# mahdi-slh/DeformContact

Hardware: AMD Instinct MI355X
Metric: M edges/sec fwd+bwd, everyday-deform batch=32 per GPU (encoder hot path) (higher is better)
Workload: dtype f32 (hops, storage, accumulate); wide dense blocks fp16x2-split operands (3 fp16 MFMA products, fp32 accumulate), narrow ones bf16x3-split (6 products); 1 GPU; everyday-deform synthetic, B=32 sample pairs per GPU: soft 32x(1024 v, 6132 e) + rigid 32x(762 v, 4560 e); TAGConv encoder 2 layers/branch, hidden 256, K=3 (configs[1]); edges_per_gpu_step=342144, global_batch=32, settle_steps=150, hipgraph=True, two_stream_branches=True, merged_branches=False, segmented_adjacency_build=True, parallelism=dp1

## Files before the change

deformcontact_amd/_lib.py:

```python
from __future__ import annotations

import ctypes
import os
from ctypes import POINTER, c_char_p, c_float, c_int, c_int32, c_int64, c_void_p

_HERE = os.path.dirname(os.path.abspath(__file__))
SO_PATH = os.path.join(_HERE, "libdeformcontact_hip.so")

_lib = None

_vp = c_void_p
_SIGNATURES = {
    "dc_version": (c_int, []),
    "dc_last_error": (c_char_p, []),
    "dc_stream_capture_id": (c_int64, [_vp]),
    "dc_csr_workspace_bytes": (c_int64, [c_int64, c_int64]),
    "dc_csr_build": (c_int, [_vp, c_int64, c_int64, c_int, c_int, _vp, _vp, _vp, _vp, _vp, _vp,
                             _vp, c_int64, _vp]),
    "dc_graph_workspace_bytes": (c_int64, [c_int64, c_int64]),
    "dc_graph_build": (c_int, [_vp, c_int64, c_int64, c_int, _vp, _vp, _vp, _vp, _vp, _vp, _vp, _vp,
                               _vp, _vp, c_int64, _vp]),
    "dc_graph_build_parts": (c_int, [POINTER(_vp), POINTER(c_int64), POINTER(c_int64), POINTER(c_int64), c_int,
                                     c_int64, c_int, _vp, _vp, _vp, _vp, _vp, _vp, _vp, _vp, _vp, _vp, c_int64,
                                     _vp]),
# ... 38 lines not shown
                                         _vp, _vp]),
    "dc_tag_grouped_bwd_dw_workspace_bytes": (c_int64, [POINTER(c_int64), c_int, c_int64, c_int64, c_int]),
    "dc_tag_grouped_bwd_dw_h2": (c_int, [_vp, c_int64, POINTER(_vp), POINTER(c_int64), c_int, c_int,
                                         POINTER(c_int64), POINTER(c_int64), c_int64, POINTER(_vp),
                                         POINTER(_vp), c_int, _vp, c_int64, c_int64, c_int64, _vp, _vp, _vp]),
    "dc_generic_dense_launches": (c_int64, [c_int]),
    "dc_kernel_trace": (None, [c_int]),
    "dc_kernel_trace_dump": (c_int64, [c_char_p, c_int64]),
    "dc_hash_i64": (c_int, [_vp, c_int64, _vp, _vp]),
    "dc_morton_codes": (c_int, [_vp, c_int64, c_int64, POINTER(c_float), POINTER(c_float), _vp, _vp]),
    "dc_morton_order_workspace_bytes": (c_int64, [c_int64]),
    "dc_morton_order": (c_int, [_vp, c_int64, c_int64, _vp, _vp, _vp, c_int64, _vp]),
    "dc_relabel_edges": (c_int, [_vp, c_int64, _vp, c_int64, _vp, _vp]),
    "dc_gather_rows": (c_int, [_vp, c_int64, _vp, _vp, c_int64, c_int64, c_int64, _vp]),
    "dc_invert_perm": (c_int, [_vp, _vp, _vp, c_int64, _vp]),
    "dc_neighbors_workspace_bytes": (c_int64, [c_int64, c_int64]),
    "dc_neighbors_fill": (c_int, [_vp, c_int64, c_int64, _vp, _vp, c_int64, c_int64, _vp, c_int, c_float, c_int, c_int,
                                  _vp, _vp, _vp, c_int64, _vp]),
    "dc_neighbors_compact_workspace_bytes": (c_int64, [c_int64]),
    "dc_neighbors_compact": (c_int, [_vp, c_int, _vp, c_int64, c_int, _vp, c_int64, _vp, c_int64, _vp]),
    "dc_spmm_f32": (c_int, [_vp, _vp, _vp, _vp, c_int64, _vp, c_int64, _vp, c_int64, c_int64,
                            c_int64, _vp]),
    "dc_spmm_bf16": (c_int, [_vp, _vp, _vp, _vp, c_int64, _vp, c_int64, _vp, c_int64, c_int64,
                             c_int64, c_int, _vp]),
    "dc_tag_linear_fwd_bf16": (c_int, [_vp, c_int64, _vp, _vp, c_int, _vp, c_int64, c_int, c_int64, c_int64,
                                       c_int64, _vp]),
    "dc_tag_mask_grad_bf16": (c_int, [_vp, c_int64, c_int, _vp, c_int64, c_int, _vp, c_int64, c_int64, c_int64, _vp]),
    "dc_tag_linear_bwd_dw_bf16_workspace_bytes": (c_int64, [c_int64, c_int64, c_int64, c_int]),
    "dc_tag_linear_bwd_dw_bf16": (c_int, [_vp, c_int64, _vp, c_int64, c_int, POINTER(_vp), _vp, c_int, _vp, c_int64,
                                          c_int64, c_int64, c_int64, _vp]),
    "dc_to_bf16": (c_int, [POINTER(_vp), c_int, c_int64, c_int64, c_int64, _vp, c_int64, _vp]),
    "dc_contact_loss_workspace_bytes": (c_int64, [c_int64]),
    "dc_contact_loss": (c_int, [_vp, _vp, _vp, _vp, _vp, c_int64, _vp, c_int64, c_int64, c_int64, _vp, _vp,
                                _vp, _vp, c_int64, _vp]),
    "dc_tag_linear_fwd": (c_int, [POINTER(_vp), POINTER(c_int64), POINTER(_vp), c_int, _vp, c_int,
                                  _vp, c_int64, c_int64, c_int64, c_int64, _vp]),
    "dc_tag_linear_bwd_dx": (c_int, [_vp, c_int64, _vp, c_int64, POINTER(_vp), c_int,
                                     POINTER(_vp), POINTER(c_int64), c_int64, c_int64, c_int64,
                                     _vp]),
    "dc_tag_linear_fwd_split": (c_int, [POINTER(_vp), POINTER(c_int64), POINTER(_vp), c_int, _vp,
                                        c_int, _vp, c_int64, c_int64, c_int64, c_int64, c_int, _vp]),
    "dc_tag_linear_bwd_dx_split_workspace_bytes": (c_int64, [c_int64, c_int64, c_int]),
    "dc_tag_linear_bwd_dx_split": (c_int, [_vp, c_int64, _vp, c_int64, POINTER(_vp), c_int,
                                           POINTER(_vp), POINTER(c_int64), _vp, c_int64, c_int64,
                                           c_int64, c_int64, c_int, _vp]),
    "dc_tag_linear_bwd_dw_workspace_bytes": (c_int64, [c_int64, c_int64, c_int64, c_int]),
    "dc_tag_linear_bwd_dw": (c_int, [_vp, c_int64, _vp, c_int64, POINTER(_vp), POINTER(c_int64),
                                     c_int, POINTER(_vp), c_int, c_int64, _vp, c_int, _vp, c_int64,
                                     c_int64, c_int64, c_int64, _vp]),
    "dc_tag_linear_bwd_dw_split": (c_int, [_vp, c_int64, _vp, c_int64, POINTER(_vp),
                                           POINTER(c_int64), c_int, POINTER(_vp), c_int, c_int64,
                                           _vp, c_int, _vp, c_int64, c_int64, c_int64, c_int64,
                                           c_int, _vp]),
    "dc_tag_linear_fwd_h2": (c_int, [POINTER(_vp), POINTER(c_int64), POINTER(_vp), c_int, _vp,
                                     c_int, _vp, c_int64, c_int64, c_int64, c_int64, _vp, _vp, _vp]),
    "dc_tag_linear_bwd_dx_h2": (c_int, [_vp, c_int64, _vp, c_int64, POINTER(_vp), c_int,
                                        POINTER(_vp), POINTER(c_int64), _vp, c_int64, c_int64,
                                        c_int64, c_int64, _vp, _vp, _vp]),
    "dc_tag_linear_bwd_dw_h2": (c_int, [_vp, c_int64, _vp, c_int64, POINTER(_vp),
                                        POINTER(c_int64), c_int, POINTER(_vp), c_int, c_int64,
                                        _vp, c_int, _vp, c_int64, c_int64, c_int64, c_int64,
                                        _vp, _vp, _vp]),
    "dc_tag_mask_grad": (c_int, [_vp, c_int64, _vp, c_int64, _vp, c_int64, c_int64, c_int64, _vp, _vp, _vp]),
    "dc_tag_transpose_weights": (c_int, [POINTER(_vp), c_int, c_int64, c_int64, _vp, _vp]),
    "dc_tag_linear_fwd_h2p_workspace_bytes": (c_int64, [c_int64, c_int64, c_int64]),
    "dc_tag_linear_fwd_h2p": (c_int, [_vp, c_int64, _vp, _vp, c_int, _vp, c_int64, c_int64, c_int64, c_int64,
                                      _vp, _vp, _vp, c_int64, _vp]),
    "dc_tag_linear_fwd_h2p_exp": (c_int, [_vp, c_int64, _vp, _vp, c_int64, c_int64, c_int64, c_int64, _vp, _vp, _vp,
                                          c_int64, _vp]),
    "dc_tag_weight_prep": (c_int, [POINTER(_vp), c_int, c_int64, c_int64, _vp, _vp, _vp, _vp, _vp]),
    "dc_tag_weight_prep_zero": (c_int, [POINTER(_vp), c_int, c_int64, c_int64, _vp, _vp, _vp, _vp, _vp, c_int64, _vp]),
    "dc_rowabsmax_f32": (c_int, [_vp, c_int64, c_int64, c_int64, _vp, _vp]),
    "dc_tag_weight_rowmax": (c_int, [POINTER(_vp), c_int, c_int64, c_int64, _vp, _vp]),
    "dc_spmm_f32_rowmax": (c_int, [_vp, _vp, _vp, _vp, c_int64, _vp, c_int64, _vp, c_int64, c_int64,
                                   c_int64, _vp, c_int, _vp]),
    "dc_tag_pack_input": (c_int, [_vp, c_int64, _vp, c_int64, c_int64, c_int64, c_int64, c_int64, _vp]),
    "dc_tag_pack_weights": (c_int, [POINTER(_vp), c_int, _vp, c_int64, c_int64, c_int64, _vp]),
    "dc_tag_linear_fwd_narrow_ok": (c_int, [c_int64, c_int, c_int64, c_int64]),
    "dc_tag_linear_fwd_narrow": (c_int, [_vp, c_int64, POINTER(_vp), c_int, c_int64, _vp, c_int, _vp, c_int64, c_int64,
                                         c_int64, c_int64, _vp]),
    "dc_attn_softmax_rows": (c_int, [_vp, c_int64, c_int64, c_int64, c_int64, _vp, _vp]),
    "dc_attn_exp_rows": (c_int, [_vp, c_int64, c_int64, c_int64, c_int64, _vp, _vp]),
    "dc_attn_ds_rows": (c_int, [_vp, _vp, c_int64, c_int64, c_int64, _vp, _vp, _vp]),
    "dc_adam_flat": (c_int, [_vp, _vp, _vp, _vp, c_int64, _vp, c_float, c_float, c_float, c_float,
                             c_int, _vp]),
    "dc_compose_perm": (c_int, [_vp, _vp, _vp, _vp, c_int64, _vp]),
    "dc_gat_edge_softmax_fwd": (c_int, [_vp, _vp, _vp, _vp, c_float, _vp, c_int64, _vp]),
    "dc_gat_edge_softmax_bwd": (c_int, [_vp, _vp, _vp, _vp, c_float, _vp, _vp, _vp, _vp, c_int64,
                                        _vp]),
    "dc_sddmm_f32": (c_int, [_vp, _vp, _vp, c_int64, _vp, c_int64, _vp, c_int64, c_int64, _vp]),
    "dc_segment_sum_f32": (c_int, [_vp, _vp, _vp, _vp, c_int64, _vp]),
    "dc_gather_f32": (c_int, [_vp, _vp, _vp, _vp, c_int64, _vp]),
    "dc_gat_alpha_heads_fwd": (c_int, [_vp, c_int64, _vp, _vp, _vp, _vp, c_int64, c_int64, c_int64, _vp]),
    "dc_gat_edge_softmax_heads_fwd": (c_int, [_vp, _vp, _vp, _vp, c_float, _vp, c_int64, c_int64, _vp]),
    "dc_spmm_f32_heads_bias_act": (c_int, [_vp, _vp, _vp, _vp, c_int64, _vp, c_int, c_int, _vp, c_int64, c_int64,
                                           c_int64, c_int64, _vp]),
    "dc_sddmm_f32_heads": (c_int, [_vp, _vp, _vp, c_int64, _vp, c_int64, _vp, c_int64, c_int64, c_int64, _vp]),
    "dc_gat_edge_softmax_heads_bwd": (c_int, [_vp, _vp, _vp, _vp, c_float, _vp, _vp, _vp, _vp, c_int64, c_int64,
                                              _vp]),
    "dc_segment_sum_f32_heads": (c_int, [_vp, _vp, _vp, _vp, c_int64, c_int64, _vp]),
    "dc_gather_f32_heads": (c_int, [_vp, _vp, _vp, _vp, c_int64, c_int64, _vp]),
    "dc_spread_heads_f32": (c_int, [_vp, c_int64, _vp, c_int64, c_int64, c_int64, c_int64, _vp]),
    "dc_gat_alpha_heads_bwd": (c_int, [_vp, c_int64, _vp, _vp, _vp, _vp, _vp, c_int64, c_int64, c_int64, c_int64, _vp,
                                       c_int64, _vp, _vp, c_int, _vp]),
    "dc_gat_edge_attr_fwd": (c_int, [_vp, _vp, _vp, c_int64, _vp, c_int, c_float, _vp, _vp, c_int64, c_int64, c_int64,
                                     c_int64, _vp]),
# ... 60 lines not shown
```

deformcontact_amd/csrc/dc_dense.h:

```cpp
#pragma once
#include "dc_common.h"

namespace dc {

constexpr int BK = 16;
constexpr int LDK = BK + 4;
constexpr int BN = 128;
constexpr int kMaxSeg = DC_MAX_SEG;

using f32x16 = __attribute__((ext_vector_type(16))) float;

struct Mat {
    const float *p;
    int64_t ld;
};

template <int MB>
struct Frag {
    float a[MB][4];
    float b[2][4];
};

template <int MB, bool A_KC, bool B_KC>
__device__ __forceinline__ void load_frag(Frag<MB> &f, const float *As, const float *Bs, int c,
// ... 38 lines not shown

template <int MB>
__device__ __forceinline__ void zero_acc(f32x16 (&acc)[MB][2]) {
#pragma unroll
    for (int mb = 0; mb < MB; ++mb)
#pragma unroll
        for (int i = 0; i < 16; ++i) acc[mb][0][i] = 0.f, acc[mb][1][i] = 0.f;
}

template <int MB> struct Tile {
    static constexpr int BM = 64 * MB;
    static constexpr int A_KC = BM * LDK, B_KC = BN * LDK, A_RC = BK * BM, B_RC = BK * BN;
};

template <int MB, typename F>
__device__ __forceinline__ void for_each_acc(const f32x16 (&acc)[MB][2], int wm, int wn, F &&f) {
    const int lane = threadIdx.x & 63, c = lane & 31, h = lane >> 5;
#pragma unroll
    for (int mb = 0; mb < MB; ++mb)
#pragma unroll
        for (int nb = 0; nb < 2; ++nb)
#pragma unroll
            for (int reg = 0; reg < 16; ++reg) {
                const int row = wm * 32 * MB + mb * 32 + (reg & 3) + 8 * (reg >> 2) + 4 * h;
                const int col = wn * 64 + nb * 32 + c;
                f(row, col, acc[mb][nb][reg]);
            }
}

struct H2Scales {
    const float *a_rowmax;
    const float *b_rowmax;
    int b_presplit;
};

__device__ __forceinline__ unsigned h2_exp(float m) {
    unsigned e = (__float_as_uint(m) >> 23) & 0xffu;
    e = e < 15u ? 15u : e;
    return e > 254u ? 254u : e;
}
__device__ __forceinline__ float h2_scale(float m) { return __uint_as_float((268u - h2_exp(m)) << 23); }
__device__ __forceinline__ float h2_unscale(float m) { return __uint_as_float((h2_exp(m) - 14u) << 23); }

__device__ __forceinline__ float h2_block_max(const float *v, int64_t beg, int64_t end, float *red) {
    float m = 0.f;
    for (int64_t i = beg + threadIdx.x; i < end; i += 256) m = fmaxf(m, v[i]);
#pragma unroll
    for (int o = 32; o >= 1; o >>= 1) m = fmaxf(m, __shfl_xor(m, o));
    if ((threadIdx.x & 63) == 0) red[threadIdx.x >> 6] = m;
    __syncthreads();
    m = fmaxf(fmaxf(red[0], red[1]), fmaxf(red[2], red[3]));
    __syncthreads();
    return m;
}

constexpr int kMaxGroups = DC_MAX_GROUPS;
constexpr int kGroupAlign = DC_GROUP_ALIGN;
struct FwdGroups {
    int n;
    int64_t row_beg[kMaxGroups];
    int64_t row_end[kMaxGroups];
    const float *w[kMaxGroups];
    const float *bias[kMaxGroups];
    const float *b_rowmax[kMaxGroups];
};
__device__ __forceinline__ int group_of_row(const int64_t (&row_beg)[kMaxGroups], int n, int64_t row) {
    int g = 0;
#pragma unroll
    for (int q = 1; q < kMaxGroups; ++q)
        if (q < n && row >= row_beg[q]) g = q;
    return g;
}

struct FwdParams {
    Mat x[kMaxSeg];
    Mat w[kMaxSeg];
    const float *bias;
    float *out;
    int64_t ldo, N, Fi, Fo;
    int nseg, relu;
    H2Scales h2;
    int ksplit;
    float *kpartial;
    const float *exp_lse;
    int64_t exp_ncols;
    FwdGroups grp;
    const float *x2, *x2_coef;
};

struct DxParams {
    Mat g, mask;
    int has_mask;
    Mat w[kMaxSeg];
    float *gx[kMaxSeg];
    int64_t ldgx[kMaxSeg];
    int64_t N, Fi, Fo;
    int nseg;
    H2Scales h2;
};

struct DwGroups {
    int n;
    int chunk_beg[kMaxGroups + 1];
    int64_t row_beg[kMaxGroups], row_end[kMaxGroups], chunk_rows[kMaxGroups];
};

struct DwParams {
    Mat g, mask;
    int has_mask;
    Mat x[kMaxSeg];
    float *partial;
    float *bias_partial;
    int64_t N, Fi, Fo, chunk_rows;
    int nseg, nchunks;
    H2Scales h2;
    DwGroups grp;
    const float *g2, *g2_coef;
};


struct DwBf16Params {
    const uint16_t *g, *x;
    int64_t ldg, ldx;
    float *partial;
    float *bias_partial;
    int64_t N, Fi, Fo, chunk_rows;
    int nseg, nchunks;
};
bool dw_bf16_launch(const DwBf16Params &p, hipStream_t hs);

bool fwd_fast_launch(const FwdParams &p, int mb, hipStream_t hs);
bool dx_fast_launch(const DxParams &p, int mb, hipStream_t hs);
bool dw_fast_launch(const DwParams &p, int mb, hipStream_t hs);
bool fwd_split_launch(const FwdParams &p, int mb, int products, hipStream_t hs);
bool dx_split_launch(DxParams p, float *wt, int mb, int products, hipStream_t hs);
bool dw_split_launch(const DwParams &p, int mb, int products, hipStream_t hs);
bool dw_h2w_launch(const DwParams &p, hipStream_t hs);
bool fwd_h2_launch(const FwdParams &p, int mb, hipStream_t hs);
bool fwd_h2w_launch(const FwdParams &p, hipStream_t hs);
bool fwd_h2d_launch(const FwdParams &p, hipStream_t hs);
void transpose_weights_launch(const float *const *ws, int nseg, int64_t Fo, int64_t Fi, float *wt,
                              hipStream_t hs);

}
```

deformcontact_amd/csrc/dc_dense.hip:

```cpp
#include <stdlib.h>

#include "dc_dense.h"

#include <atomic>
static std::atomic<long long> g_generic_dense_launches{0};

namespace dc {

template <bool VEC>
__device__ __forceinline__ float4 ld4(const float *row_ptr, int64_t k, int64_t kmax) {
    if (VEC) {
        const int64_t kc = (k + 4 <= kmax) ? k : 0;
        return *reinterpret_cast<const float4 *>(row_ptr + kc);
    } else {
        const int64_t last = kmax - 1;
        return make_float4(row_ptr[k + 0 <= last ? k + 0 : last], row_ptr[k + 1 <= last ? k + 1 : last],
                           row_ptr[k + 2 <= last ? k + 2 : last], row_ptr[k + 3 <= last ? k + 3 : last]);
    }
}

__device__ __forceinline__ float4 zero_invalid(float4 v, bool row_ok, int64_t k, int64_t kmax) {
    return make_float4((row_ok && k + 0 < kmax) ? v.x : 0.f, (row_ok && k + 1 < kmax) ? v.y : 0.f,
                       (row_ok && k + 2 < kmax) ? v.z : 0.f, (row_ok && k + 3 < kmax) ? v.w : 0.f);
}

__device__ __forceinline__ float4 relu_mask(float4 v, float4 m) {
    return make_float4(m.x > 0.f ? v.x : 0.f, m.y > 0.f ? v.y : 0.f, m.z > 0.f ? v.z : 0.f,
                       m.w > 0.f ? v.w : 0.f);
}

struct TileArgs {
    int64_t r0, rmax;
    int64_t c0, cmax;
};

template <int ROWS, bool VEC, bool MASK>
struct StageKC {
    float4 v[ROWS / 64];
    float4 m[MASK ? ROWS / 64 : 1];
    __device__ __forceinline__ void load(const Mat &mat, const Mat &mask, const TileArgs &t) {
        const int k4 = threadIdx.x & 3, r = threadIdx.x >> 2;
        const int64_t k = t.c0 + 4 * k4;
#pragma unroll
        for (int j = 0; j < ROWS / 64; ++j) {
            const int64_t row = t.r0 + r + 64 * j;
            const int64_t rc = row < t.rmax ? row : t.rmax - 1;
            v[j] = ld4<VEC>(mat.p + rc * mat.ld, k, t.cmax);
            if (MASK) m[j] = ld4<VEC>(mask.p + rc * mask.ld, k, t.cmax);
        }
    }
    __device__ __forceinline__ float4 value(int j, const TileArgs &t) const {
        const int k4 = threadIdx.x & 3, r = threadIdx.x >> 2;
        float4 x = zero_invalid(v[j], t.r0 + r + 64 * j < t.rmax, t.c0 + 4 * k4, t.cmax);
        if (MASK) x = relu_mask(x, m[j]);
        return x;
    }
    __device__ __forceinline__ void store(float *lds, const TileArgs &t) const {
        const int k4 = threadIdx.x & 3, r = threadIdx.x >> 2;
#pragma unroll
        for (int j = 0; j < ROWS / 64; ++j)
            *reinterpret_cast<float4 *>(lds + (r + 64 * j) * LDK + 4 * k4) = value(j, t);
    }
};

template <int COLS, bool VEC, bool MASK>
struct StageRC {
    static constexpr int PER = COLS / 4;
    static constexpr int KPER = 256 / PER;
    static constexpr int NLD = BK / KPER;
    float4 v[NLD];
    float4 m[MASK ? NLD : 1];
    __device__ __forceinline__ void load(const Mat &mat, const Mat &mask, const TileArgs &t) {
        const int c4 = threadIdx.x % PER, kr = threadIdx.x / PER;
        const int64_t col = t.c0 + 4 * c4;
#pragma unroll
        for (int j = 0; j < NLD; ++j) {
            const int64_t k = t.r0 + kr + KPER * j;
            const int64_t kc = k < t.rmax ? k : t.rmax - 1;
            v[j] = ld4<VEC>(mat.p + kc * mat.ld, col, t.cmax);
            if (MASK) m[j] = ld4<VEC>(mask.p + kc * mask.ld, col, t.cmax);
        }
    }
    __device__ __forceinline__ float4 value(int j, const TileArgs &t) const {
        const int c4 = threadIdx.x % PER, kr = threadIdx.x / PER;
        float4 x = zero_invalid(v[j], t.r0 + kr + KPER * j < t.rmax, t.c0 + 4 * c4, t.cmax);
        if (MASK) x = relu_mask(x, m[j]);
        return x;
    }
    __device__ __forceinline__ void store(float *lds, const TileArgs &t) const {
        const int c4 = threadIdx.x % PER, kr = threadIdx.x / PER;
#pragma unroll
        for (int j = 0; j < NLD; ++j)
            *reinterpret_cast<float4 *>(lds + (kr + KPER * j) * COLS + 4 * c4) = value(j, t);
    }
};

constexpr int kRing = 3;
static_assert(BK == 16, "the pipeline below is written for two 8-wide chunks per stage");

struct NoHook {
    template <typename S>
    __device__ __forceinline__ void operator()(const S &, const TileArgs &) const {}
};

template <int MB, bool A_KC, bool B_KC, int STAGE, int OFFB, typename SA, typename SB,
          typename TileFn, typename LdA, typename LdB, typename Hook = NoHook>
__device__ __forceinline__ void gemm_pipeline(float *lds, int nst, TileFn &&tile, LdA &&ldA,
                                              LdB &&ldB, f32x16 (&acc)[MB][2], int wm, int wn,
                                              Hook &&on_store_a = NoHook{}) {
    SA a0, a1;
    SB b0, b1;
    auto gload = [&](int st, SA &ra, SB &rb) {
        TileArgs ta, tb;
        tile(st, ta, tb);
        ldA(ra, ta);
        ldB(rb, tb);
    };
    auto lstore = [&](int st, const SA &ra, const SB &rb) {
        TileArgs ta, tb;
        tile(st, ta, tb);
        ra.store(lds + (st % kRing) * STAGE, ta);
        rb.store(lds + (st % kRing) * STAGE + OFFB, tb);
        on_store_a(ra, ta);
    };
    if (nst > 0) gload(0, a0, b0);
    if (nst > 1) gload(1, a1, b1);
    if (nst > 0) lstore(0, a0, b0);
    if (nst > 2) gload(2, a0, b0);
    if (nst > 1) lstore(1, a1, b1);
    if (nst > 3) gload(3, a1, b1);
    __syncthreads();
    Frag<MB> f0, f1;
    if (nst > 0) load_frag<MB, A_KC, B_KC>(f0, lds, lds + OFFB, 0, wm, wn);
// ... 76 lines not shown
    const int64_t col0 = (int64_t)(lb % ntn) * BN;
    const int wid = threadIdx.x >> 6, wm = wid >> 1, wn = wid & 1;

    f32x16 acc[MB][2];
    zero_acc<MB>(acc);

    const int nst = (int)((p.Fo + BK - 1) / BK);
    using SA = StageKC<BM, VEC, MASK>;
    using SB = StageRC<BN, VEC, false>;
    auto tile = [&](int st, TileArgs &ta, TileArgs &tb) {
        ta = TileArgs{row0, p.N, (int64_t)st * BK, p.Fo};
        tb = TileArgs{(int64_t)st * BK, p.Fo, col0, p.Fi};
    };
    auto ldA = [&](SA &ra, const TileArgs &t) { ra.load(p.g, p.mask, t); };
    auto ldB = [&](SB &rb, const TileArgs &t) { rb.load(p.w[s], p.w[s], t); };
    gemm_pipeline<MB, true, false, kStage, kOffB, SA, SB>(lds, nst, tile, ldA, ldB, acc, wm, wn);
    float *out = p.gx[s];
    const int64_t ldo = p.ldgx[s];
    for_each_acc<MB>(acc, wm, wn, [&](int r, int c, float v) {
        const int64_t row = row0 + r, col = col0 + c;
        if (row < p.N && col < p.Fi) out[row * ldo + col] = v;
    });
}


template <int MB, bool VEC, bool MASK>
__global__ void __launch_bounds__(256)
k_tag_linear_bwd_dw(DwParams p) {
    using T = Tile<MB>;
    constexpr int BM = T::BM, kStage = T::A_RC + T::B_RC, kOffB = T::A_RC;
    __shared__ __attribute__((aligned(16))) float lds[kRing * kStage];
    const unsigned ntm = (unsigned)((p.Fo + BM - 1) / BM), ntn = (unsigned)((p.Fi + BN - 1) / BN);
    const unsigned tiles = ntm * ntn, per_chunk = tiles * p.nseg;
    const unsigned lb = blockIdx.x;
    const unsigned chunk = lb / per_chunk, rem = lb % per_chunk;
    const int s = (int)(rem / tiles);
    const int64_t o0 = (int64_t)((rem % tiles) / ntn) * BM, f0 = (int64_t)((rem % tiles) % ntn) * BN;
    const int64_t n_beg = (int64_t)chunk * p.chunk_rows;
    const int64_t n_end = (n_beg + p.chunk_rows < p.N) ? n_beg + p.chunk_rows : p.N;
    const int wid = threadIdx.x >> 6, wm = wid >> 1, wn = wid & 1;
    const bool do_bias = p.bias_partial && s == 0 && f0 == 0;

    f32x16 acc[MB][2];
    zero_acc<MB>(acc);
    float4 bsum4 = make_float4(0.f, 0.f, 0.f, 0.f);

    const int nst = (int)((n_end - n_beg + BK - 1) / BK);
    using SA = StageRC<BM, VEC, MASK>;
    using SB = StageRC<BN, VEC, false>;
    auto tile = [&](int st, TileArgs &ta, TileArgs &tb) {
        ta = TileArgs{n_beg + (int64_t)st * BK, n_end, o0, p.Fo};
        tb = TileArgs{n_beg + (int64_t)st * BK, n_end, f0, p.Fi};
    };
    auto ldA = [&](SA &ra, const TileArgs &t) { ra.load(p.g, p.mask, t); };
    auto ldB = [&](SB &rb, const TileArgs &t) { rb.load(p.x[s], p.x[s], t); };
    auto bias_hook = [&](const SA &ra, const TileArgs &t) {
        if (do_bias) {
#pragma unroll
            for (int j = 0; j < SA::NLD; ++j) {
                const float4 x = ra.value(j, t);
                bsum4.x += x.x, bsum4.y += x.y, bsum4.z += x.z, bsum4.w += x.w;
            }
        }
    };
    gemm_pipeline<MB, false, false, kStage, kOffB, SA, SB>(lds, nst, tile, ldA, ldB, acc, wm, wn,
                                                          bias_hook);
    float *out = p.partial + ((int64_t)chunk * p.nseg + s) * p.Fo * p.Fi;
    for_each_acc<MB>(acc, wm, wn, [&](int r, int c, float v) {
        const int64_t o = o0 + r, f = f0 + c;
        if (o < p.Fo && f < p.Fi) out[o * p.Fi + f] = v;
    });
    if (do_bias) {
        __syncthreads();
        float4 *red = reinterpret_cast<float4 *>(lds);
        red[threadIdx.x] = bsum4;
        __syncthreads();
        if (threadIdx.x < SA::PER) {
            float4 t = make_float4(0.f, 0.f, 0.f, 0.f);
            for (int g = 0; g < 256 / SA::PER; ++g) {
                const float4 v = red[g * SA::PER + threadIdx.x];
                t.x += v.x, t.y += v.y, t.z += v.z, t.w += v.w;
            }
            float *bp = p.bias_partial + (int64_t)chunk * p.Fo;
            const int64_t o = o0 + 4 * threadIdx.x;
            if (o + 0 < p.Fo) bp[o + 0] = t.x;
            if (o + 1 < p.Fo) bp[o + 1] = t.y;
            if (o + 2 < p.Fo) bp[o + 2] = t.z;
            if (o + 3 < p.Fo) bp[o + 3] = t.w;
        }
    }
}

struct ReduceParams {
    const float *partial, *bias_partial;
    float *gw[2 * kMaxSeg];
    float *gbias;
    int64_t Fi, Fo, cols;
    int nseg, nchunks, ngw, bps, accumulate;
};

constexpr int kReduceOutputs = 64;
__device__ __forceinline__ void dw_reduce_body(const ReduceParams &p) {
    __shared__ float red[4][kReduceOutputs];
    const int64_t per_out = p.Fo * p.cols, total = per_out * p.ngw;
    const int64_t seg_elems = p.Fo * p.Fi, slab = seg_elems * p.nseg;
    const int el = threadIdx.x & 63, q = threadIdx.x >> 6;
    const int64_t i = (int64_t)blockIdx.x * kReduceOutputs + el;
// ... 93 lines not shown
static inline int env_int(const char *name, int dflt) {
    const char *v = getenv(name);
    return v ? atoi(v) : dflt;
}

static inline int pick_mb(int64_t rows, int64_t col_tiles) {
    return (((rows + 127) / 128) * col_tiles >= 512) ? 2 : 1;
}

static inline int split_mb(int64_t rows, int64_t col_tiles) {
    const int64_t nb2 = ((rows + 127) / 128) * col_tiles, nb1 = ((rows + 63) / 64) * col_tiles;
    const double t2 = (double)((nb2 + 255) / 256);
    const double t1 = (double)((nb1 + 255) / 256) * 0.5 * 1.12;
    return t1 < t2 ? 1 : 2;
}

static inline int dw_mb(int64_t Fo) {
    return Fo >= 128 ? 2 : 1;
}

static void dw_plan(int64_t N, int64_t Fi, int64_t Fo, int nseg, int64_t *chunk_rows,
                    int *nchunks) {
    const int64_t BM = 64 * dw_mb(Fo);
    const int64_t tiles = ((Fo + BM - 1) / BM) * ((Fi + BN - 1) / BN) * nseg;
    constexpr int target = 512, maxchunks = 128;
    int64_t want = target / (tiles > 0 ? tiles : 1);
    if (want < 1) want = 1;
    if (want > maxchunks) want = maxchunks;
    if (want == 1 && N >= 8192) {
        const int64_t t2 = ((Fo + 127) / 128) * ((Fi + 255) / 256) * nseg;
        double best = 0.0;
        for (int64_t c = 1; c <= 8 && N / c >= 2048; ++c) {
            const int64_t w = (t2 * c + 255) / 256;
            const double eff = (double)(t2 * c) / (double)(w * 256);
            if (eff > best + 0.02) best = eff, want = c;
        }
    }
    int64_t rows = (N + want - 1) / want;
    if (rows < 256) rows = 256;
    rows = (rows + 2 * BK - 1) / (2 * BK) * (2 * BK);
    *chunk_rows = rows;
    *nchunks = (int)((N + rows - 1) / rows);
    if (*nchunks < 1) *nchunks = 1;
}

}

using namespace dc;

static int fwd_impl(const float *const *xs, const int64_t *ldxs, const float *const *ws, int nseg,
                    const float *bias, int relu, float *out, int64_t ldo, int64_t N, int64_t Fi,
                    int64_t Fo, dc_stream_t stream, int products, H2Scales h2 = H2Scales{},
                    float *ksplit_ws = nullptr, int64_t ksplit_ws_bytes = 0, const float *exp_lse = nullptr,
                    int64_t exp_ncols = 0) {
    DC_REQUIRE(nseg >= 1 && nseg <= kMaxSeg, "dc_tag_linear_fwd: nseg must be 1..%d", kMaxSeg);
    DC_REQUIRE(N >= 0 && Fi >= 1 && Fo >= 1, "dc_tag_linear_fwd: bad sizes");
    if (N == 0) return DC_OK;
    DC_REQUIRE(xs && ldxs && ws && out && ldo >= Fo, "dc_tag_linear_fwd: null pointer / ldo < Fo");
    FwdParams p{};
    bool vec = (Fi % 4 == 0);
    for (int s = 0; s < nseg; ++s) {
        DC_REQUIRE(xs[s] && ws[s] && ldxs[s] >= Fi, "dc_tag_linear_fwd: bad segment %d", s);
        p.x[s] = make_mat(xs[s], ldxs[s], &vec);
        p.w[s] = make_mat(ws[s], Fi, &vec);
    }
    p.bias = bias, p.out = out, p.ldo = ldo, p.N = N, p.Fi = Fi, p.Fo = Fo;
    p.nseg = nseg, p.relu = relu;
    p.h2 = h2;
    p.exp_lse = exp_lse, p.exp_ncols = exp_ncols;
    DC_REQUIRE(!exp_lse || h2.b_presplit, "dc_tag_linear_fwd: the exp epilogue exists on the pre-split h2 kernels only");
    const int64_t ntn = (Fo + BN - 1) / BN;
    const int mb = pick_mb(N, ntn);
    const int64_t grid = ((N + 64 * mb - 1) / (64 * mb)) * ntn;
    DC_REQUIRE(grid < (int64_t)INT32_MAX, "dc_tag_linear_fwd: grid too large");
    const dim3 gd((unsigned)grid), bd(256);
    hipStream_t hs = (hipStream_t)stream;
    if (products == 2 && vec) {
        int smb = split_mb(N, ntn);
        const int64_t nst = Fi / BK;
        if (ksplit_ws && !bias && !relu && ldo == Fo && nseg == 1) {
            smb = 2;
            int64_t tiles = ((N + 127) / 128) * ntn;
            if (tiles < 128) smb = 1, tiles = ((N + 63) / 64) * ntn;
            int64_t ks = tiles < 256 ? (512 + tiles - 1) / tiles : 1;
            if (ks > nst / 8) ks = nst / 8;
            if (ks > 32) ks = 32;
            while (ks > 1 && ks * N * Fo * (int64_t)sizeof(float) > ksplit_ws_bytes) --ks;
            if (ks > 1) p.ksplit = (int)ks, p.kpartial = ksplit_ws;
        }
        if (fwd_h2_launch(p, smb, hs)) {
            if (p.ksplit > 1) {
                ReduceParams r{};
                r.partial = p.kpartial, r.gw[0] = out, r.Fi = Fo, r.Fo = N, r.cols = Fo;
                r.nseg = 1, r.nchunks = p.ksplit, r.ngw = 1, r.bps = 1, r.accumulate = 0;
                const int64_t total = N * Fo;
                launch_reduce(r, total, hs);
            }
            return check_launch("dc_tag_linear_fwd_h2");
        }
        p.ksplit = 0, p.kpartial = nullptr;
    }
    DC_REQUIRE(!h2.b_presplit, "dc_tag_linear_fwd_h2p: shape not eligible for the pre-split kernel");
    if (products && vec && fwd_split_launch(p, split_mb(N, ntn), products, hs))
        return check_launch("dc_tag_linear_fwd_split");
    DC_REQUIRE(products != 2, "dc_tag_linear_fwd_h2: needs Fi %% 16 == 0, 16-byte aligned operands, "
                              "equal leading dimensions (Fi=%lld)", (long long)Fi);
    if (vec && fwd_fast_launch(p, mb, hs)) return check_launch("dc_tag_linear_fwd");
    static const int trace = env_int("DC_DENSE_TRACE", 0);
    ++g_generic_dense_launches;
    if (trace)
        fprintf(stderr, "[dc] generic fwd dense kernel: N=%lld Fi=%lld Fo=%lld nseg=%d vec=%d ldx=%lld ldo=%lld products=%d\n",
                (long long)N, (long long)Fi, (long long)Fo, nseg, (int)vec, (long long)ldxs[0], (long long)ldo, products);
    if (mb == 2 && vec)
        DC_LAUNCH((k_tag_linear_fwd<2, true>), gd, bd, 0, hs, p);
    else if (mb == 2)
        DC_LAUNCH((k_tag_linear_fwd<2, false>), gd, bd, 0, hs, p);
    else if (vec)
        DC_LAUNCH((k_tag_linear_fwd<1, true>), gd, bd, 0, hs, p);
    else
        DC_LAUNCH((k_tag_linear_fwd<1, false>), gd, bd, 0, hs, p);
    return check_launch("dc_tag_linear_fwd");
}

static int dx_impl(const float *g, int64_t ldg, const float *out_for_mask, int64_t ldo,
                   const float *const *ws, int nseg, float *const *gxs, const int64_t *ldgxs,
                   int64_t N, int64_t Fi, int64_t Fo, dc_stream_t stream, float *split_ws,
                   int products, H2Scales h2 = H2Scales{}) {
    DC_REQUIRE(nseg >= 1 && nseg <= kMaxSeg, "dc_tag_linear_bwd_dx: nseg must be 1..%d", kMaxSeg);
    DC_REQUIRE(N >= 0 && Fi >= 1 && Fo >= 1, "dc_tag_linear_bwd_dx: bad sizes");
    if (N == 0) return DC_OK;
    DC_REQUIRE(g && ws && gxs && ldgxs && ldg >= Fo, "dc_tag_linear_bwd_dx: null pointer / ldg < Fo");
    DC_REQUIRE(!out_for_mask || ldo >= Fo, "dc_tag_linear_bwd_dx: ldo < Fo");
    DxParams p{};
    bool vec = (Fi % 4 == 0) && (Fo % 4 == 0);
    p.g = make_mat(g, ldg, &vec);
    p.has_mask = out_for_mask != nullptr;
    if (out_for_mask) p.mask = make_mat(out_for_mask, ldo, &vec);
    for (int s = 0; s < nseg; ++s) {
        DC_REQUIRE(ws[s] && gxs[s] && ldgxs[s] >= Fi, "dc_tag_linear_bwd_dx: bad segment %d", s);
        p.w[s] = make_mat(ws[s], Fi, &vec);
        p.gx[s] = gxs[s];
        p.ldgx[s] = ldgxs[s];
    }
// ... 47 lines not shown
extern "C" int dc_tag_linear_bwd_dx(const float *g, int64_t ldg, const float *out_for_mask,
                                    int64_t ldo, const float *const *ws, int nseg,
                                    float *const *gxs, const int64_t *ldgxs, int64_t N, int64_t Fi,
                                    int64_t Fo, dc_stream_t stream) {
    return dx_impl(g, ldg, out_for_mask, ldo, ws, nseg, gxs, ldgxs, N, Fi, Fo, stream, nullptr, 0);
}

extern "C" int dc_tag_linear_bwd_dw(const float *g, int64_t ldg, const float *out_for_mask,
                                    int64_t ldo, const float *const *xs, const int64_t *ldxs,
                                    int nseg, float *const *gws, int ngw, int64_t gw_cols,
                                    float *gbias, int accumulate, void *partials,
                                    int64_t partials_bytes, int64_t N, int64_t Fi, int64_t Fo,
                                    dc_stream_t stream);
extern "C" int dc_tag_linear_bwd_dw_split(const float *g, int64_t ldg, const float *out_for_mask,
                                          int64_t ldo, const float *const *xs, const int64_t *ldxs,
                                          int nseg, float *const *gws, int ngw, int64_t gw_cols,
                                          float *gbias, int accumulate, void *partials,
                                          int64_t partials_bytes, int64_t N, int64_t Fi, int64_t Fo,
                                          int products, dc_stream_t stream);

extern "C" int64_t dc_tag_linear_bwd_dx_split_workspace_bytes(int64_t Fi, int64_t Fo, int nseg) {
    if (Fi < 1 || Fo < 1 || nseg < 1 || nseg > kMaxSeg) return DC_EINVAL;
    return (int64_t)sizeof(float) * nseg * Fi * Fo + 16;
}

extern "C" int dc_tag_linear_bwd_dx_split(const float *g, int64_t ldg, const float *out_for_mask,
                                          int64_t ldo, const float *const *ws, int nseg,
                                          float *const *gxs, const int64_t *ldgxs, void *workspace,
                                          int64_t workspace_bytes, int64_t N, int64_t Fi,
                                          int64_t Fo, int products, dc_stream_t stream) {
    DC_REQUIRE(products == 6 || products == 3 || products == 1,
               "dc_tag_linear_bwd_dx_split: products must be 6, 3 or 1");
    DC_REQUIRE(workspace && ((uintptr_t)workspace & 15) == 0 &&
                   workspace_bytes >= dc_tag_linear_bwd_dx_split_workspace_bytes(Fi, Fo, nseg),
               "dc_tag_linear_bwd_dx_split: workspace missing, misaligned or too small");
    return dx_impl(g, ldg, out_for_mask, ldo, ws, nseg, gxs, ldgxs, N, Fi, Fo, stream,
                   (float *)workspace, products);
}

extern "C" int64_t dc_tag_linear_bwd_dw_workspace_bytes(int64_t N, int64_t Fi, int64_t Fo,
                                                        int nseg) {
    if (N < 0 || Fi < 1 || Fo < 1 || nseg < 1 || nseg > kMaxSeg) return DC_EINVAL;
    int64_t rows;
    int nchunks;
    dw_plan(N, Fi, Fo, nseg, &rows, &nchunks);
    return (int64_t)sizeof(float) * (nchunks + 1) * (nseg * Fo * Fi + Fo) + 16;
}

static int dw_impl(const float *g, int64_t ldg, const float *out_for_mask, int64_t ldo,
                   const float *const *xs, const int64_t *ldxs, int nseg, float *const *gws, int ngw,
                   int64_t gw_cols, float *gbias, int accumulate, void *partials,
                   int64_t partials_bytes, int64_t N, int64_t Fi, int64_t Fo, dc_stream_t stream,
                   int products, H2Scales h2 = H2Scales{}, const float *g2 = nullptr,
                   const float *g2_coef = nullptr) {
    DC_REQUIRE(nseg >= 1 && nseg <= kMaxSeg, "dc_tag_linear_bwd_dw: nseg must be 1..%d", kMaxSeg);
    DC_REQUIRE(N >= 0 && Fi >= 1 && Fo >= 1, "dc_tag_linear_bwd_dw: bad sizes");
    DC_REQUIRE(g && xs && ldxs && gws && partials && ldg >= Fo,
               "dc_tag_linear_bwd_dw: null pointer / ldg < Fo");
    DC_REQUIRE(!out_for_mask || ldo >= Fo, "dc_tag_linear_bwd_dw: ldo < Fo");
    DC_REQUIRE(partials_bytes >= dc_tag_linear_bwd_dw_workspace_bytes(N, Fi, Fo, nseg),
               "dc_tag_linear_bwd_dw: workspace too small");
    DC_REQUIRE(((uintptr_t)partials & 15) == 0, "dc_tag_linear_bwd_dw: workspace not 16-byte aligned");
    DwParams p{};
    bool vec = (Fi % 4 == 0) && (Fo % 4 == 0);
    p.g = make_mat(g, ldg, &vec);
    p.has_mask = out_for_mask != nullptr;
    if (out_for_mask) p.mask = make_mat(out_for_mask, ldo, &vec);
    ReduceParams r{};
    for (int s = 0; s < nseg; ++s) {
        DC_REQUIRE(xs[s] && ldxs[s] >= Fi, "dc_tag_linear_bwd_dw: bad segment %d", s);
        p.x[s] = make_mat(xs[s], ldxs[s], &vec);
    }
    DC_REQUIRE(ngw >= nseg && ngw <= 2 * kMaxSeg && ngw % nseg == 0 && gw_cols >= 1 &&
                   (ngw / nseg) * gw_cols <= Fi,
               "dc_tag_linear_bwd_dw: %d output blocks of %lld columns do not tile %d segments of %lld",
               ngw, (long long)gw_cols, nseg, (long long)Fi);
    for (int j = 0; j < ngw; ++j) {
        DC_REQUIRE(gws[j], "dc_tag_linear_bwd_dw: null output block %d", j);
        r.gw[j] = gws[j];
    }
    dw_plan(N, Fi, Fo, nseg, &p.chunk_rows, &p.nchunks);
    p.N = N, p.Fi = Fi, p.Fo = Fo, p.nseg = nseg;
    p.h2 = h2;
    p.partial = (float *)partials;
    const int64_t tail = vec ? N % BK : 0;
    const bool ragged = tail != 0 && N > tail;
    const int nslots = p.nchunks + (ragged ? 1 : 0);
    p.bias_partial = gbias ? p.partial + (int64_t)nslots * nseg * Fo * Fi : nullptr;
    const int mb = dw_mb(Fo);
    const int64_t tiles = ((Fo + 64 * mb - 1) / (64 * mb)) * ((Fi + BN - 1) / BN);
    const int64_t grid = tiles * nseg * p.nchunks;
    if (!p.has_mask) p.mask = p.g;
    const dim3 gd((unsigned)grid), bd(256);
    hipStream_t hs = (hipStream_t)stream;
    if (g2) {
        DC_REQUIRE(g2_coef && products == 2 && vec && !ragged && (((uintptr_t)g2) & 15) == 0,
                   "dc_tag_linear_bwd_dw_h2_corr: needs the coefficient vector, aligned operands and N %% 16 == 0");
        p.g2 = g2, p.g2_coef = g2_coef;
        DC_REQUIRE(dw_h2w_launch(p, hs), "dc_tag_linear_bwd_dw_h2_corr: shape not eligible for the 128 x 256 tile kernel "
                   "(needs Fo %% 128 == 0, Fi == 256, N %% 32 == 0; N=%lld Fi=%lld Fo=%lld)", (long long)N,
                   (long long)Fi, (long long)Fo);
        r.partial = p.partial, r.bias_partial = p.bias_partial, r.gbias = gbias;
        r.Fi = Fi, r.Fo = Fo, r.nseg = nseg, r.nchunks = nslots;
        r.cols = gw_cols, r.ngw = ngw, r.bps = ngw / nseg, r.accumulate = accumulate;
        const int64_t total_c = (int64_t)ngw * Fo * gw_cols + (gbias ? Fo : 0);
        launch_reduce(r, total_c, hs);
        return check_launch("dc_tag_linear_bwd_dw_h2_corr");
    }
    if (ragged) {
        DwParams t = p;
        const int64_t n0 = N - tail;
        t.g.p += n0 * t.g.ld;
        t.mask.p += n0 * t.mask.ld;
        for (int s = 0; s < nseg; ++s) t.x[s].p += n0 * t.x[s].ld;
        t.N = tail, t.chunk_rows = BK, t.nchunks = 1;
        t.partial = p.partial + (int64_t)p.nchunks * nseg * Fo * Fi;
        t.bias_partial = p.bias_partial ? p.bias_partial + (int64_t)p.nchunks * Fo : nullptr;
        t.h2 = H2Scales{};
        const dim3 gt((unsigned)(tiles * nseg));
        if (mb == 2) {
            if (p.has_mask) DC_LAUNCH((k_tag_linear_bwd_dw<2, true, true>), gt, bd, 0, hs, t);
            else DC_LAUNCH((k_tag_linear_bwd_dw<2, true, false>), gt, bd, 0, hs, t);
        } else {
            if (p.has_mask) DC_LAUNCH((k_tag_linear_bwd_dw<1, true, true>), gt, bd, 0, hs, t);
            else DC_LAUNCH((k_tag_linear_bwd_dw<1, true, false>), gt, bd, 0, hs, t);
        }
        p.N = n0;
    }
    bool fast_done = products && vec && dw_split_launch(p, mb, products, hs);
    DC_REQUIRE(fast_done || products != 2, "dc_tag_linear_bwd_dw_h2: needs N %% 16 == 0, Fi %% 4 == 0, "
               "Fo %% 4 == 0 and 16-byte aligned operands (N=%lld)", (long long)N);
    fast_done = fast_done || (vec && dw_fast_launch(p, mb, hs));
#define DC_DW(MB_, V_, M_) DC_LAUNCH((k_tag_linear_bwd_dw<MB_, V_, M_>), gd, bd, 0, hs, p)
    if (!fast_done) ++g_generic_dense_launches;
    if (fast_done) {
    } else
    if (mb == 2) {
        if (vec && p.has_mask) DC_DW(2, true, true);
        else if (vec) DC_DW(2, true, false);
        else if (p.has_mask) DC_DW(2, false, true);
        else DC_DW(2, false, false);
    } else {
        if (vec && p.has_mask) DC_DW(1, true, true);
        else if (vec) DC_DW(1, true, false);
        else if (p.has_mask) DC_DW(1, false, true);
        else DC_DW(1, false, false);
    }
#undef DC_DW
    r.partial = p.partial, r.bias_partial = p.bias_partial, r.gbias = gbias;
    r.Fi = Fi, r.Fo = Fo, r.nseg = nseg, r.nchunks = nslots;
    r.cols = gw_cols, r.ngw = ngw, r.bps = ngw / nseg, r.accumulate = accumulate;
    const int64_t total = (int64_t)ngw * Fo * gw_cols + (gbias ? Fo : 0);
    launch_reduce(r, total, (hipStream_t)stream);
    return check_launch("dc_tag_linear_bwd_dw");
}

extern "C" int dc_tag_linear_bwd_dw(const float *g, int64_t ldg, const float *out_for_mask,
                                    int64_t ldo, const float *const *xs, const int64_t *ldxs,
                                    int nseg, float *const *gws, int ngw, int64_t gw_cols,
                                    float *gbias, int accumulate, void *partials,
                                    int64_t partials_bytes, int64_t N, int64_t Fi, int64_t Fo,
                                    dc_stream_t stream) {
    return dw_impl(g, ldg, out_for_mask, ldo, xs, ldxs, nseg, gws, ngw, gw_cols, gbias, accumulate,
                   partials, partials_bytes, N, Fi, Fo, stream, 0);
}

extern "C" int dc_tag_linear_bwd_dw_split(const float *g, int64_t ldg, const float *out_for_mask,
                                          int64_t ldo, const float *const *xs, const int64_t *ldxs,
                                          int nseg, float *const *gws, int ngw, int64_t gw_cols,
                                          float *gbias, int accumulate, void *partials,
                                          int64_t partials_bytes, int64_t N, int64_t Fi, int64_t Fo,
                                          int products, dc_stream_t stream) {
    DC_REQUIRE(products == 6 || products == 3 || products == 1,
               "dc_tag_linear_bwd_dw_split: products must be 6, 3 or 1");
    return dw_impl(g, ldg, out_for_mask, ldo, xs, ldxs, nseg, gws, ngw, gw_cols, gbias, accumulate,
                   partials, partials_bytes, N, Fi, Fo, stream, products);
}


extern "C" int dc_tag_linear_fwd_h2(const float *const *xs, const int64_t *ldxs,
                                    const float *const *ws, int nseg, const float *bias, int relu,
                                    float *out, int64_t ldo, int64_t N, int64_t Fi, int64_t Fo,
                                    const float *x_rowmax, const float *w_rowmax,
                                    dc_stream_t stream) {
    DC_REQUIRE(x_rowmax && w_rowmax, "dc_tag_linear_fwd_h2: x_rowmax / w_rowmax missing");
    H2Scales h{};
    h.a_rowmax = x_rowmax, h.b_rowmax = w_rowmax;
    return fwd_impl(xs, ldxs, ws, nseg, bias, relu, out, ldo, N, Fi, Fo, stream, 2, h);
}

extern "C" int64_t dc_tag_linear_fwd_h2p_workspace_bytes(int64_t N, int64_t K, int64_t Fo) {
    if (N < 0 || K < 1 || Fo < 1) return DC_EINVAL;
    const int64_t tiles = ((N + 63) / 64) * ((Fo + BN - 1) / BN);
    if (tiles >= 256 || K / BK < 16) return 0;
    return 32 * N * Fo * (int64_t)sizeof(float);
}

extern "C" int dc_tag_linear_fwd_h2p(const float *x, int64_t ldx, const void *w_image,
                                     const float *bias, int relu, float *out, int64_t ldo, int64_t N,
                                     int64_t K, int64_t Fo, const float *x_rowmax,
                                     const float *w_rowmax, void *workspace,
                                     int64_t workspace_bytes, dc_stream_t stream) {
    DC_REQUIRE(x && w_image && x_rowmax && w_rowmax, "dc_tag_linear_fwd_h2p: null pointer");
    DC_REQUIRE(K >= 16 && K % 16 == 0 && ldx >= K && ldx % 4 == 0 && (((uintptr_t)x) & 15) == 0 &&
                   (((uintptr_t)w_image) & 15) == 0,
               "dc_tag_linear_fwd_h2p: K %% 16 == 0 and 16-byte aligned operands required (K=%lld)",
               (long long)K);
    H2Scales h{};
    h.a_rowmax = x_rowmax, h.b_rowmax = w_rowmax, h.b_presplit = 1;
    const float *xs[1] = {x};
    const float *ws[1] = {(const float *)w_image};
    const int64_t ld[1] = {ldx};
    DC_REQUIRE(!workspace || (((uintptr_t)workspace) & 15) == 0, "dc_tag_linear_fwd_h2p: workspace misaligned");
    return fwd_impl(xs, ld, ws, 1, bias, relu, out, ldo, N, K, Fo, stream, 2, h, (float *)workspace,
                    workspace ? workspace_bytes : 0);
}

extern "C" int dc_tag_linear_fwd_h2p_corr(const float *x, int64_t ldx, const float *x2, const float *x2_coef,
                                          const void *w_image, float *out, int64_t ldo, int64_t N, int64_t K,
                                          int64_t Fo, const float *x_rowmax, const float *w_rowmax,
                                          dc_stream_t stream) {
    DC_REQUIRE(N >= 0 && K >= 32 && K % 32 == 0 && Fo >= 1, "dc_tag_linear_fwd_h2p_corr: K must be a multiple of 32");
    if (N == 0) return DC_OK;
    DC_REQUIRE(x && x2 && x2_coef && w_image && out && x_rowmax && w_rowmax && ldx >= K && ldo >= Fo &&
                   (((uintptr_t)x2) & 15) == 0, "dc_tag_linear_fwd_h2p_corr: null / short / misaligned operand");
    FwdParams p{};
    bool vec = true;
    p.x[0] = make_mat(x, ldx, &vec);
    p.w[0] = make_mat((const float *)w_image, K, &vec);
    p.out = out, p.ldo = ldo, p.N = N, p.Fi = K, p.Fo = Fo, p.nseg = 1;
    p.h2.a_rowmax = x_rowmax, p.h2.b_rowmax = w_rowmax, p.h2.b_presplit = 1;
    p.x2 = x2, p.x2_coef = x2_coef;
    DC_REQUIRE(vec && fwd_h2w_launch(p, (hipStream_t)stream),
               "dc_tag_linear_fwd_h2p_corr: shape not eligible for the 128 x 256 tile kernel (N=%lld K=%lld Fo=%lld: "
               "needs 16-byte aligned rows)", (long long)N, (long long)K, (long long)Fo);
    return check_launch("dc_tag_linear_fwd_h2p_corr");
}

extern "C" int dc_tag_linear_fwd_h2p_exp(const float *x, int64_t ldx, const void *w_image, float *out,
                                         int64_t ldo, int64_t N, int64_t K, int64_t Fo, const float *x_rowmax,
                                         const float *w_rowmax, const float *row_lse, int64_t ncols_valid,
                                         dc_stream_t stream) {
    DC_REQUIRE(x && w_image && x_rowmax && w_rowmax && row_lse, "dc_tag_linear_fwd_h2p_exp: null pointer");
    DC_REQUIRE(K >= 16 && K % 16 == 0 && ldx >= K && ldx % 4 == 0 && (((uintptr_t)x) & 15) == 0 &&
                   (((uintptr_t)w_image) & 15) == 0 && ncols_valid >= 0 && ncols_valid <= Fo,
               "dc_tag_linear_fwd_h2p_exp: K %% 16 == 0, 16-byte aligned operands, 0 <= ncols_valid <= Fo required");
    H2Scales h{};
    h.a_rowmax = x_rowmax, h.b_rowmax = w_rowmax, h.b_presplit = 1;
    const float *xs[1] = {x};
    const float *ws[1] = {(const float *)w_image};
    const int64_t ld[1] = {ldx};
    return fwd_impl(xs, ld, ws, 1, nullptr, 0, out, ldo, N, K, Fo, stream, 2, h, nullptr, 0, row_lse, ncols_valid);
}

extern "C" int dc_tag_linear_bwd_dx_h2(const float *g, int64_t ldg, const float *out_for_mask,
                                       int64_t ldo, const float *const *ws, int nseg,
                                       float *const *gxs, const int64_t *ldgxs, void *workspace,
                                       int64_t workspace_bytes, int64_t N, int64_t Fi, int64_t Fo,
                                       const float *g_rowmax, const float *w_rowmax,
                                       dc_stream_t stream) {
    DC_REQUIRE(w_rowmax && g_rowmax, "dc_tag_linear_bwd_dx_h2: g_rowmax / w_rowmax missing");
    DC_REQUIRE(workspace && ((uintptr_t)workspace & 15) == 0 &&
                   workspace_bytes >= dc_tag_linear_bwd_dx_split_workspace_bytes(Fi, Fo, nseg),
               "dc_tag_linear_bwd_dx_h2: workspace missing, misaligned or too small");
    H2Scales h{};
    h.a_rowmax = g_rowmax, h.b_rowmax = w_rowmax;
    return dx_impl(g, ldg, out_for_mask, ldo, ws, nseg, gxs, ldgxs, N, Fi, Fo, stream,
                   (float *)workspace, 2, h);
// ... 23 lines not shown
    H2Scales h2{};
    h2.a_rowmax = g_rowmax, h2.b_rowmax = x_rowmax;
    return dw_impl(g, ldg, nullptr, 0, xs, ldxs, nseg, gws, ngw, gw_cols, nullptr, accumulate, partials,
                   partials_bytes, N, Fi, Fo, stream, 2, h2, g2, g2_coef);
}

namespace dc {
__global__ void __launch_bounds__(256)
k_rowabsmax(const float *__restrict__ x, int64_t ld, int64_t N, int F, float *__restrict__ rowmax,
            bool vec4) {
    const int64_t row = (int64_t)blockIdx.x * 4 + (threadIdx.x >> 6);
    if (row >= N) return;
    const int lane = threadIdx.x & 63;
    const float *xr = x + row * ld;
    float m = 0.f;
    if (vec4) {
        for (int c = lane * 4; c < F; c += 256) {
            const float4 v = *reinterpret_cast<const float4 *>(xr + c);
            m = fmaxf(m, fmaxf(fmaxf(fabsf(v.x), fabsf(v.y)), fmaxf(fabsf(v.z), fabsf(v.w))));
        }
    } else {
        for (int c = lane; c < F; c += 64) m = fmaxf(m, fabsf(xr[c]));
    }
#pragma unroll
    for (int o = 32; o >= 1; o >>= 1) m = fmaxf(m, __shfl_xor(m, o));
    if (lane == 0) rowmax[row] = m;
}

struct WRowmaxParams {
    const float *w[kMaxSeg];
    int nseg;
    int64_t Fo, Fi;
    float *out;
};
__global__ void __launch_bounds__(256) k_w_rowmax(WRowmaxParams p) {
    const int64_t o = (int64_t)blockIdx.x * 4 + (threadIdx.x >> 6);
    if (o >= p.Fo) return;
    const int lane = threadIdx.x & 63;
    float m = 0.f;
    for (int s = 0; s < p.nseg; ++s) {
        const float *wr = p.w[s] + o * p.Fi;
        for (int64_t c = lane; c < p.Fi; c += 64) m = fmaxf(m, fabsf(wr[c]));
    }
#pragma unroll
    for (int q = 32; q >= 1; q >>= 1) m = fmaxf(m, __shfl_xor(m, q));
    if (lane == 0) p.out[o] = m;
}
}

namespace dc {
__global__ void __launch_bounds__(256)
k_mask_grad(const float *__restrict__ g, int64_t ldg, const float *__restrict__ mask, int64_t ldm,
            float *__restrict__ gm, int64_t ldgm, int64_t N, int F, float *__restrict__ rowmax_a,
            float *__restrict__ rowmax_b, bool vec4) {
    const int64_t row = (int64_t)blockIdx.x * 4 + (threadIdx.x >> 6);
    if (row >= N) return;
    const int lane = threadIdx.x & 63;
    const float *gr = g + row * ldg, *mr = mask ? mask + row * ldm : nullptr;
    float *o = gm + row * ldgm;
    float m = 0.f;
    if (vec4) {
        for (int c = lane * 4; c < F; c += 256) {
            float4 v = *reinterpret_cast<const float4 *>(gr + c);
            if (mr) {
                const float4 k = *reinterpret_cast<const float4 *>(mr + c);
                v = make_float4(k.x > 0.f ? v.x : 0.f, k.y > 0.f ? v.y : 0.f, k.z > 0.f ? v.z : 0.f,
                                k.w > 0.f ? v.w : 0.f);
            }
            *reinterpret_cast<float4 *>(o + c) = v;
            m = fmaxf(m, fmaxf(fmaxf(fabsf(v.x), fabsf(v.y)), fmaxf(fabsf(v.z), fabsf(v.w))));
        }
    } else {
        for (int c = lane; c < F; c += 64) {
            float v = gr[c];
            if (mr && !(mr[c] > 0.f)) v = 0.f;
            o[c] = v;
            m = fmaxf(m, fabsf(v));
        }
    }
#pragma unroll
    for (int q = 32; q >= 1; q >>= 1) m = fmaxf(m, __shfl_xor(m, q));
    if (lane == 0) {
        rowmax_a[row] = m;
        if (rowmax_b) rowmax_b[row] = m;
    }
}
}

extern "C" int dc_tag_mask_grad(const float *g, int64_t ldg, const float *out_for_mask, int64_t ldo,
                                float *gm, int64_t ldgm, int64_t N, int64_t F, float *rowmax_a,
                                float *rowmax_b, dc_stream_t stream) {
    DC_REQUIRE(N >= 0 && F >= 1 && F < (1 << 24) && ldg >= F && ldgm >= F && (!out_for_mask || ldo >= F),
               "dc_tag_mask_grad: bad sizes");
    if (N == 0) return DC_OK;
    DC_REQUIRE(g && gm && rowmax_a, "dc_tag_mask_grad: null pointer");
    const bool vec4 = (F % 4 == 0) && (ldg % 4 == 0) && (ldgm % 4 == 0) && (((uintptr_t)g) & 15) == 0 &&
                      (((uintptr_t)gm) & 15) == 0 &&
                      (!out_for_mask || ((ldo % 4 == 0) && (((uintptr_t)out_for_mask) & 15) == 0));
    DC_LAUNCH(k_mask_grad, dim3((unsigned)((N + 3) / 4)), dim3(256), 0, (hipStream_t)stream, g,
                       ldg, out_for_mask, ldo, gm, ldgm, N, (int)F, rowmax_a, rowmax_b, vec4);
    return check_launch("dc_tag_mask_grad");
}

namespace dc {
struct WPrepParams {
    const float *w[kMaxSeg];
    int nseg;
    int64_t Fo, Fi;
    float *w_rowmax, *wt_rowmax;
    _Float16 *wimg, *wtimg;
    float *zero;
    int64_t zero_n;
    int tall;
};
__device__ __forceinline__ void wprep_put(_Float16 *img_row, int64_t k, float v, float scale) {
    const float x = v * scale;
    const _Float16 h = (_Float16)x;
    _Float16 *rec = img_row + (k >> 4) * 32 + (k & 15);
    rec[0] = h;
    rec[16] = (_Float16)(x - (float)h);
}
__device__ __forceinline__ void weight_prep_body(const WPrepParams &p) {
    const int lane = threadIdx.x & 63;
    for (int64_t i = (int64_t)blockIdx.x * blockDim.x + threadIdx.x; i < p.zero_n; i += (int64_t)gridDim.x * blockDim.x)
        p.zero[i] = 0.f;
    if (p.tall)
        for (int64_t i = (int64_t)blockIdx.x * blockDim.x + threadIdx.x; i < p.Fi; i += (int64_t)gridDim.x * blockDim.x)
            p.wt_rowmax[i] = 0.f;
    const int64_t rb = (p.Fo + 3) / 4;
    float m = 0.f;
    const bool small = p.Fi <= 256 && p.Fo <= 256;
    if ((int64_t)blockIdx.x < rb) {
        const int64_t o = (int64_t)blockIdx.x * 4 + (threadIdx.x >> 6);
        if (o >= p.Fo) return;
        float v[kMaxSeg][4];
        if (small) {
#pragma unroll
            for (int s = 0; s < kMaxSeg; ++s)
#pragma unroll
                for (int j = 0; j < 4; ++j) {
                    const int64_t c = lane + 64 * j;
                    v[s][j] = (s < p.nseg && c < p.Fi) ? p.w[s][o * p.Fi + c] : 0.f;
                    m = fmaxf(m, fabsf(v[s][j]));
                }
        } else {
            for (int s = 0; s < p.nseg; ++s) {
                const float *wr = p.w[s] + o * p.Fi;
                for (int64_t c = lane; c < p.Fi; c += 64) m = fmaxf(m, fabsf(wr[c]));
            }
        }
#pragma unroll
        for (int q = 32; q >= 1; q >>= 1) m = fmaxf(m, __shfl_xor(m, q));
        if (lane == 0) p.w_rowmax[o] = m;
        if (p.wimg) {
// ... 472 lines not shown
```

deformcontact_amd/csrc/dc_dense_fast.hip:

```cpp
#include "dc_dense.h"

namespace dc {

template <int ROWS, bool KC, bool MASK>
struct FastOp {
    static constexpr int NV = ROWS / 64;
    static constexpr int PER = ROWS / 4;
    static constexpr int KPER = 256 / PER;
    const float *p[NV];
    const float *pm[MASK ? NV : 1];
    float4 v[NV];
    float4 m[MASK ? NV : 1];
    int off[NV];
    int64_t step;

    __device__ __forceinline__ void init_kc(const float *base, const float *mbase, int64_t ld,
                                            int64_t row0, int64_t nrows, int64_t k0) {
        const int k4 = threadIdx.x & 3, r = threadIdx.x >> 2;
#pragma unroll
        for (int j = 0; j < NV; ++j) {
            int64_t row = row0 + r + 64 * j;
            row = row < nrows ? row : nrows - 1;
            p[j] = base + row * ld + k0 + 4 * k4;
            if (MASK) pm[j] = mbase + row * ld + k0 + 4 * k4;
// ... 204 lines not shown
        __syncthreads();
        float4 *red = reinterpret_cast<float4 *>(lds);
        red[threadIdx.x] = bsum4;
        __syncthreads();
        if (threadIdx.x < OA::PER) {
            float4 t = make_float4(0.f, 0.f, 0.f, 0.f);
            for (int g = 0; g < 256 / OA::PER; ++g) {
                const float4 v = red[g * OA::PER + threadIdx.x];
                t.x += v.x, t.y += v.y, t.z += v.z, t.w += v.w;
            }
            float *bp = p.bias_partial + (int64_t)chunk * p.Fo;
            const int64_t o = o0 + 4 * threadIdx.x;
            if (o + 4 <= p.Fo) {
                bp[o + 0] = t.x, bp[o + 1] = t.y, bp[o + 2] = t.z, bp[o + 3] = t.w;
            }
        }
    }
}

static inline bool al16(const void *q) { return ((uintptr_t)q & 15) == 0; }

bool fwd_fast_launch(const FwdParams &p, int mb, hipStream_t hs) {
    if (p.Fi % BK != 0 || p.Fi < BK) return false;
    for (int s = 0; s < p.nseg; ++s)
        if (!al16(p.x[s].p) || !al16(p.w[s].p) || p.x[s].ld % 4 != 0 || p.x[s].ld != p.x[0].ld)
            return false;
    const int64_t grid = ((p.N + 64 * mb - 1) / (64 * mb)) * ((p.Fo + BN - 1) / BN);
    const dim3 gd((unsigned)grid), bd(256);
    if (mb == 2)
        DC_LAUNCH((k_fwd_fast<2>), gd, bd, 0, hs, p);
    else
        DC_LAUNCH((k_fwd_fast<1>), gd, bd, 0, hs, p);
    return true;
}

bool dx_fast_launch(const DxParams &p, int mb, hipStream_t hs) {
    if (p.Fo % BK != 0 || p.Fi % 4 != 0 || p.Fi < 4 || !al16(p.g.p) || p.g.ld % 4 != 0) return false;
    if (p.has_mask && (!al16(p.mask.p) || p.mask.ld != p.g.ld)) return false;
    for (int s = 0; s < p.nseg; ++s)
        if (!al16(p.w[s].p)) return false;
    const int64_t grid = ((p.N + 64 * mb - 1) / (64 * mb)) * ((p.Fi + BN - 1) / BN) * p.nseg;
    const dim3 gd((unsigned)grid), bd(256);
#define DC_L(MB_, M_) DC_LAUNCH((k_dx_fast<MB_, M_>), gd, bd, 0, hs, p)
    if (mb == 2) { if (p.has_mask) DC_L(2, true); else DC_L(2, false); }
    else { if (p.has_mask) DC_L(1, true); else DC_L(1, false); }
#undef DC_L
    return true;
}

bool dw_fast_launch(const DwParams &p, int mb, hipStream_t hs) {
    if (p.N % BK != 0 || p.chunk_rows % BK != 0 || p.Fi % 4 != 0 || p.Fo % 4 != 0 || p.Fi < 4 ||
        p.Fo < 4 || !al16(p.g.p) || p.g.ld % 4 != 0)
        return false;
    if (p.has_mask && (!al16(p.mask.p) || p.mask.ld != p.g.ld)) return false;
    for (int s = 0; s < p.nseg; ++s)
        if (!al16(p.x[s].p) || p.x[s].ld % 4 != 0) return false;
    const int64_t tiles = ((p.Fo + 64 * mb - 1) / (64 * mb)) * ((p.Fi + BN - 1) / BN);
    const dim3 gd((unsigned)(tiles * p.nseg * p.nchunks)), bd(256);
#define DC_L(MB_, M_) DC_LAUNCH((k_dw_fast<MB_, M_>), gd, bd, 0, hs, p)
    if (mb == 2) { if (p.has_mask) DC_L(2, true); else DC_L(2, false); }
    else { if (p.has_mask) DC_L(1, true); else DC_L(1, false); }
#undef DC_L
    return true;
}

}
```

deformcontact_amd/csrc/dc_dense_h2.hip:

```cpp
#include "dc_dense.h"

namespace dc {

using h2_f16x4 = __attribute__((ext_vector_type(4))) _Float16;
using h2_f16x8 = __attribute__((ext_vector_type(8))) _Float16;

constexpr int kH2Plane = 32;
constexpr int kH2Row = 2 * kH2Plane + 16;

__device__ __forceinline__ void h2_split_store(char *dst, float4 x, float s) {
    x = make_float4(x.x * s, x.y * s, x.z * s, x.w * s);
    h2_f16x4 h, l;
    const float v[4] = {x.x, x.y, x.z, x.w};
#pragma unroll
    for (int i = 0; i < 4; ++i) {
        const _Float16 a = (_Float16)v[i];
        h[i] = a;
        l[i] = (_Float16)(v[i] - (float)a);
    }
    *reinterpret_cast<h2_f16x4 *>(dst) = h;
    *reinterpret_cast<h2_f16x4 *>(dst + kH2Plane) = l;
}

template <int MB, bool BDMA>
// ... 133 lines not shown
            frags(cur);
            if (BDMA) dma_b(nxt);
            store(nxt);
            load();
            mma();
            if (BDMA) __builtin_amdgcn_s_waitcnt(0xF70 | 0);
            __syncthreads();
        }
        for (; it < nst; ++it) {
            const int cur = it & 1, nxt = cur ^ 1;
            frags(cur);
            if (it + 1 < nst) {
                if (BDMA) dma_b(nxt);
                store(nxt);
            }
            mma();
            if (BDMA) __builtin_amdgcn_s_waitcnt(0xF70 | 0);
            __syncthreads();
        }
    }

    float bcol[2], icol[2];
#pragma unroll
    for (int nb = 0; nb < 2; ++nb) {
        const int64_t col = col0 + wn * 64 + nb * 32 + (threadIdx.x & 31);
        bcol[nb] = (p.bias && col < p.Fo) ? p.bias[col] : 0.f;
        icol[nb] = h2_unscale(p.h2.b_rowmax[col < p.Fo ? col : p.Fo - 1]);
    }
    const bool relu = p.relu != 0;
    if (ks > 1) {
        float *part = p.kpartial + (int64_t)kz * p.N * p.Fo;
        for_each_acc<MB>(acc, wm, wn, [&](int rr, int c, float v) {
            const int64_t row = row0 + rr, col = col0 + c;
            if (row < p.N && col < p.Fo) part[row * p.Fo + col] = (v * s_inv[rr]) * icol[(c >> 5) & 1];
        });
        return;
    }
    for_each_acc<MB>(acc, wm, wn, [&](int rr, int c, float v) {
        const int64_t row = row0 + rr, col = col0 + c;
        if (row < p.N && col < p.Fo) {
            v = (v * s_inv[rr]) * icol[(c >> 5) & 1];
            v += bcol[(c >> 5) & 1];
            if (relu) v = fmaxf(v, 0.f);
            if (p.exp_lse) v = col < p.exp_ncols ? expf(v - p.exp_lse[row]) : 0.f;
            p.out[row * p.ldo + col] = v;
        }
    });
}



static inline bool h2_al16(const void *q) { return ((uintptr_t)q & 15) == 0; }

bool fwd_h2_launch(const FwdParams &p, int mb, hipStream_t hs) {
    if (!p.h2.a_rowmax || !p.h2.b_rowmax || p.nseg != 1) return false;
    if (fwd_h2w_launch(p, hs)) return true;
    if (p.Fi % BK != 0 || p.Fi < BK) return false;
    if (p.x[0].ld * 128 >= ((int64_t)1 << 30) || p.Fi * 128 >= ((int64_t)1 << 30)) return false;
    for (int s = 0; s < p.nseg; ++s)
        if (!h2_al16(p.x[s].p) || !h2_al16(p.w[s].p) || p.x[s].ld % 4 != 0 || p.x[s].ld != p.x[0].ld)
            return false;
    const int64_t grid = ((p.N + 64 * mb - 1) / (64 * mb)) * ((p.Fo + BN - 1) / BN) *
                         (p.ksplit > 1 ? p.ksplit : 1);
    const dim3 gd((unsigned)grid), bd(256);
    if (p.h2.b_presplit) {
        if (mb == 2) DC_LAUNCH((k_fwd_h2<2, true>), gd, bd, 0, hs, p);
        else DC_LAUNCH((k_fwd_h2<1, true>), gd, bd, 0, hs, p);
    } else {
        if (mb == 2) DC_LAUNCH((k_fwd_h2<2, false>), gd, bd, 0, hs, p);
        else DC_LAUNCH((k_fwd_h2<1, false>), gd, bd, 0, hs, p);
    }
    return true;
}

}
```

deformcontact_amd/csrc/dc_dense_h2d.hip:

```cpp
#include "dc_dense.h"

namespace dc {

using hd_f16x8 = __attribute__((ext_vector_type(8))) _Float16;
using hd_f32x4 = __attribute__((ext_vector_type(4))) float;

constexpr int kDBM = 128, kDBN = 256, kDBK = 32;
constexpr int kDRow = 128;
constexpr int kDSzA = kDBM * kDRow, kDSzB = kDBN * kDRow;
constexpr int kDRX = 4, kDRW = 3;
constexpr int kDLds = kDRW * kDSzB + kDRX * kDSzA;
constexpr int kDOffRowF = kDBM * 1024, kDOffColF = kDOffRowF + kDBM * 4, kDOffBias = kDOffColF + kDBN * 4;
static_assert(kDLds <= 160 * 1024 && kDOffBias + kDBN * 4 <= kDLds, "LDS budget");

__device__ __forceinline__ int hd_swz(int row) { return ((row >> 1) & 7) ^ ((row & 1) << 1); }
#define DC_HD_WAITVM(n) __builtin_amdgcn_s_waitcnt(0x0F70 | ((n) & 15) | (((n) >> 4) << 14))

template <bool FULL>
__global__ void __launch_bounds__(512)
k_fwd_h2d(FwdParams p) {
    __shared__ __attribute__((aligned(1024))) char lds[kDLds];
    char *const sB = lds, *const sA = lds + kDRW * kDSzB;
    const unsigned ntn = (unsigned)((p.Fo + kDBN - 1) / kDBN);
    const unsigned lb = xcd_remap(blockIdx.x, gridDim.x);
    const int64_t row0 = (int64_t)(lb / ntn) * kDBM, col0 = (int64_t)(lb % ntn) * kDBN;
    const int wid = __builtin_amdgcn_readfirstlane((int)(threadIdx.x >> 6)), lane = threadIdx.x & 63;
    const int nst = (int)(p.Fi / kDBK);
    const int64_t lda = p.x[0].ld;
    const float *wimg = p.w[0].p, *bias = p.bias, *brm = p.h2.b_rowmax;
    int64_t data_end = p.N;
    if (p.grp.n >= 1) {
        const int g = group_of_row(p.grp.row_beg, p.grp.n, row0);
        wimg = p.grp.w[g], bias = p.grp.bias[g], brm = p.grp.b_rowmax[g];
        data_end = p.grp.row_end[g];
    }

    auto store_rows = [&]() {
        __syncthreads();
        const bool relu = p.relu != 0;
        const hd_f32x4 icol = *reinterpret_cast<const hd_f32x4 *>(lds + kDOffColF + 16 * lane);
        const hd_f32x4 bcol = *reinterpret_cast<const hd_f32x4 *>(lds + kDOffBias + 16 * lane);
        const int64_t col = col0 + 4 * lane;
#pragma unroll 4
        for (int j = 0; j < 16; ++j) {
            const int rl = wid * 16 + j;
            const int64_t row = row0 + rl;
            const float sv = *reinterpret_cast<const float *>(lds + kDOffRowF + 4 * rl);
            hd_f32x4 v = *reinterpret_cast<const hd_f32x4 *>(lds + rl * 1024 + 16 * lane);
#pragma unroll
            for (int i = 0; i < 4; ++i) {
                float t = (v[i] * sv) * icol[i];
                t += bcol[i];
                if (relu) t = fmaxf(t, 0.f);
                v[i] = row >= data_end ? 0.f : t;
            }
            if (FULL || (row < p.N && col < p.Fo)) *reinterpret_cast<hd_f32x4 *>(p.out + row * p.ldo + col) = v;
        }
    };

    if (wid >= 4) {
        const bool isx = wid >= 6;
        const int w = wid & 1;
        const int64_t ld = isx ? lda : p.Fi;
        const int64_t trows = isx ? (p.N - row0 < kDBM ? p.N - row0 : kDBM) : (p.Fo - col0 < kDBN ? p.Fo - col0 : kDBN);
        const float *base = isx ? p.x[0].p + row0 * lda : wimg + col0 * p.Fi;
        const __amdgpu_buffer_rsrc_t rs = __builtin_amdgcn_make_buffer_rsrc(
            const_cast<float *>(base), 0, (int)(((trows - 1) * ld + p.Fi) * 4), 0x00020000);
        int voff[2];
#pragma unroll
        for (int e = 0; e < 2; ++e)
            voff[e] = (int)(((int64_t)(lane >> 3) * ld) * 4 + 16 * ((lane & 7) ^ hd_swz(8 * e + (lane >> 3))));
        const int cstep = (int)(8 * ld * 4);
        if (isx) {
            float rowf[2] = {0.f, 0.f};
            hd_f32x4 colf = {0.f, 0.f, 0.f, 0.f}, biasv = {0.f, 0.f, 0.f, 0.f};
            if (w == 0) {
#pragma unroll
                for (int i = 0; i < 2; ++i) {
                    const int64_t row = row0 + 2 * lane + i;
                    rowf[i] = h2_unscale(p.h2.a_rowmax[(FULL || row < p.N) ? row : p.N - 1]);
                }
#pragma unroll
                for (int i = 0; i < 4; ++i) {
                    const int64_t col = col0 + 4 * lane + i;
                    const int64_t colc = (FULL || col < p.Fo) ? col : p.Fo - 1;
                    colf[i] = h2_unscale(brm[colc]);
                    biasv[i] = bias ? bias[colc] : 0.f;
                }
            }
            auto stage = [&](int s) {
                char *dst = sA + (s % kDRX) * kDSzA;
#pragma unroll
                for (int j = 0; j < 8; ++j) {
                    const int c = 8 * w + j;
                    __builtin_amdgcn_raw_ptr_buffer_load_lds(rs, (void __attribute__((address_space(3))) *)(dst + c * 1024), 16,
                                                             voff[j & 1], c * cstep + s * (kDBK * 4), 0, 0);
                }
            };
#pragma unroll
            for (int s = 0; s < kDRX - 1; ++s)
                if (s < nst) stage(s);
            if (nst > kDRX - 1) DC_HD_WAITVM(8 * (kDRX - 3)); else DC_HD_WAITVM(0);
            __builtin_amdgcn_s_barrier();
            int it = 0;
            for (; it + kDRX - 1 < nst; ++it) {
                stage(it + kDRX - 1);
                DC_HD_WAITVM(8 * (kDRX - 3));
                __builtin_amdgcn_s_barrier();
            }
// ... 124 lines not shown
        mma_nb(FA_CUR, 0);                                                                            \
        fragB(0, SW_NEXT, KS_NEXT);                                                                   \
        __builtin_amdgcn_sched_group_barrier(0x100, 4, 0);                                            \
        __builtin_amdgcn_sched_group_barrier(0x008, 6, 0);                                            \
        __builtin_amdgcn_sched_group_barrier(0x100, 2, 0);                                            \
        __builtin_amdgcn_sched_barrier(0);                                                            \
        mma_nb(FA_CUR, 1);                                                                            \
        fragB(1, SW_NEXT, KS_NEXT);                                                                   \
        __builtin_amdgcn_sched_group_barrier(0x008, 6, 0);                                            \
        __builtin_amdgcn_sched_group_barrier(0x100, 2, 0);                                            \
        __builtin_amdgcn_sched_barrier(0);                                                            \
        mma_nb(FA_CUR, 2);                                                                            \
        split(FA_NEXT, 0);                                                                            \
        fragB(2, SW_NEXT, KS_NEXT);                                                                   \
        sgb_mfma_valu();                                                                              \
        __builtin_amdgcn_sched_barrier(0);                                                            \
        mma_nb(FA_CUR, 3);                                                                            \
        split(FA_NEXT, 1);                                                                            \
        fragB(3, SW_NEXT, KS_NEXT);                                                                   \
        sgb_mfma_valu();                                                                              \
        __builtin_amdgcn_sched_barrier(0);                                                            \
    }
    for (int it = 0; it + 1 < nst; ++it) {
        const int sx1 = sx + 1 == kDRX ? 0 : sx + 1, sw1 = sw + 1 == kDRW ? 0 : sw + 1;
        DC_H2D_KSTEP(fa0, fa1, sx, sw, 1)
        DC_H2D_KSTEP(fa1, fa0, sx1, sw1, 0)
        __syncthreads();
        sx = sx1, sw = sw1;
    }
    DC_H2D_KSTEP(fa0, fa1, sx, sw, 1)
#pragma unroll
    for (int nb = 0; nb < 4; ++nb) mma_nb(fa1, nb);
    __syncthreads();
#undef DC_H2D_KSTEP

    const int c = lane & 31, h = lane >> 5;
    float *const so = reinterpret_cast<float *>(lds);
#pragma unroll
    for (int mb = 0; mb < 2; ++mb)
#pragma unroll
        for (int nb = 0; nb < 4; ++nb)
#pragma unroll
            for (int r = 0; r < 16; ++r)
#ifdef DC_H2D_ABL_MFMA16
                so[(wm * 64 + mb * 32 + (r & 3) + 8 * (r >> 2) + 4 * h) * 256 + wn * 128 + nb * 32 + c] = acc4[mb][nb][r >> 2][r & 3];
#else
                so[(wm * 64 + mb * 32 + (r & 3) + 8 * (r >> 2) + 4 * h) * 256 + wn * 128 + nb * 32 + c] = acc[mb][nb][r];
#endif
    store_rows();
}

static inline bool hd_al16(const void *q) { return ((uintptr_t)q & 15) == 0; }

bool fwd_h2d_launch(const FwdParams &p, hipStream_t hs) {
    static const int on = [] {
        const char *v = getenv("DC_H2_DMA");
        return (v && *v) ? atoi(v) : 1;
    }();
    if (!on || p.ksplit > 1 || p.exp_lse || p.x2) return false;
    if (!p.h2.a_rowmax || !p.h2.b_rowmax || !p.h2.b_presplit || p.nseg != 1) return false;
    static const int min_k = [] {
        const char *v = getenv("DC_H2_DMA_MIN_K");
        return (v && *v) ? atoi(v) : 8 * kDBK;
    }();
    if (p.Fi % kDBK != 0 || p.Fi < kDBK || p.Fi < min_k || p.Fo % 4 != 0 || p.ldo % 4 != 0 || p.x[0].ld % 4 != 0) return false;
    if (!hd_al16(p.x[0].p) || !hd_al16(p.w[0].p) || !hd_al16(p.out)) return false;
    for (int g = 0; g < p.grp.n; ++g)
        if (!hd_al16(p.grp.w[g])) return false;
    if (p.x[0].ld * kDBM >= ((int64_t)1 << 28) || p.Fi * kDBN >= ((int64_t)1 << 28)) return false;
    const int64_t tiles = ((p.N + kDBM - 1) / kDBM) * ((p.Fo + kDBN - 1) / kDBN);
    if (tiles >= (int64_t)INT32_MAX) return false;
    const dim3 gd((unsigned)tiles), bd(512);
    if (p.N % kDBM == 0 && p.Fo % kDBN == 0)
        DC_LAUNCH((k_fwd_h2d<true>), gd, bd, 0, hs, p);
    else
        DC_LAUNCH((k_fwd_h2d<false>), gd, bd, 0, hs, p);
    return true;
}

}
```

deformcontact_amd/csrc/dc_dense_h2w.hip:

```cpp
#include "dc_dense.h"

namespace dc {

using hw_f16x4 = __attribute__((ext_vector_type(4))) _Float16;
using hw_f16x8 = __attribute__((ext_vector_type(8))) _Float16;
using hw_f32x4 = __attribute__((ext_vector_type(4))) float;
using hw_u32x4 = __attribute__((ext_vector_type(4))) unsigned;

constexpr int kWBM = 128, kWBN = 256, kWBK = 32;
constexpr int kWRow = 128;
constexpr int kWSzA = kWBM * kWRow, kWSzB = kWBN * kWRow;

__device__ __forceinline__ int hw_swz(int row) { return ((row >> 1) & 7) ^ ((row & 1) << 1); }

template <bool FULL, bool CORR = false>
__global__ void __launch_bounds__(512)
k_fwd_h2w(FwdParams p) {
    __shared__ __attribute__((aligned(16))) char sA[3 * kWSzA];
    __shared__ __attribute__((aligned(16))) char sB[3 * kWSzB];
    __shared__ __attribute__((aligned(16))) float s_inv[kWBM];
    const unsigned ntn = (unsigned)((p.Fo + kWBN - 1) / kWBN);
    const unsigned ks = p.ksplit > 1 ? (unsigned)p.ksplit : 1u, ntiles = gridDim.x / ks;
    const unsigned lbb = xcd_remap(blockIdx.x, gridDim.x);
    const unsigned lb = lbb % ntiles, kz = lbb / ntiles;
// ... 179 lines not shown
            const int64_t col = col0 + wn * 64 + nb * 32 + c;
            const bool cok = FULL || col < p.Fo;
            const float icol = h2_unscale(brm[cok ? col : p.Fo - 1]);
#pragma unroll
            for (int mb = 0; mb < 2; ++mb)
#pragma unroll
                for (int g = 0; g < 4; ++g) {
                    const int rl = wm * 64 + mb * 32 + 8 * g + 4 * h;
#pragma unroll
                    for (int i = 0; i < 4; ++i) {
                        const int64_t row = row0 + rl + i;
                        if (FULL || (cok && row < p.N))
                            part[row * p.Fo + col] = (acc[mb][nb][4 * g + i] * s_inv[rl + i]) * icol;
                    }
                }
        }
        return;
    }
#pragma unroll
    for (int nb = 0; nb < 2; ++nb) {
        const int64_t col = col0 + wn * 64 + nb * 32 + c;
        const bool cok = FULL || col < p.Fo;
        const int64_t colc = cok ? col : p.Fo - 1;
        const float bcol = bias ? bias[colc] : 0.f;
        const float icol = h2_unscale(brm[colc]);
#pragma unroll
        for (int mb = 0; mb < 2; ++mb)
#pragma unroll
            for (int g = 0; g < 4; ++g) {
                const int rl = wm * 64 + mb * 32 + 8 * g + 4 * h;
                const float4 si = *reinterpret_cast<const float4 *>(&s_inv[rl]);
                const float sv[4] = {si.x, si.y, si.z, si.w};
#pragma unroll
                for (int i = 0; i < 4; ++i) {
                    const int64_t row = row0 + rl + i;
                    float v = (acc[mb][nb][4 * g + i] * sv[i]) * icol;
                    v += bcol;
                    if (relu) v = fmaxf(v, 0.f);
                    if (p.exp_lse)
                        v = col < p.exp_ncols ? expf(v - p.exp_lse[(FULL || row < p.N) ? row : p.N - 1]) : 0.f;
                    if (row >= data_end) v = 0.f;
                    if (FULL || (cok && row < p.N)) p.out[row * p.ldo + col] = v;
                }
            }
    }
}

static inline bool hw_al16(const void *q) { return ((uintptr_t)q & 15) == 0; }
static inline int hw_env_int(const char *name, int dflt) {
    const char *v = getenv(name);
    return (v && *v) ? atoi(v) : dflt;
}

bool fwd_h2w_launch(const FwdParams &p, hipStream_t hs) {
    static const int wide = hw_env_int("DC_H2_WIDE", 1);
    if (!p.h2.a_rowmax || !p.h2.b_rowmax || !p.h2.b_presplit || p.nseg != 1) return false;
    if (!wide && p.grp.n < 1 && !p.x2) return false;
    const int64_t ks = p.ksplit > 1 ? p.ksplit : 1;
    if (ks > 1 && (!p.kpartial || p.bias || p.relu || p.exp_lse)) return false;
    if (p.Fi % kWBK != 0 || p.Fi < kWBK) return false;
    if (p.x[0].ld * kWBM >= ((int64_t)1 << 30) || p.Fi * kWBN >= ((int64_t)1 << 30)) return false;
    if (!hw_al16(p.x[0].p) || !hw_al16(p.w[0].p) || p.x[0].ld % 4 != 0) return false;
    const int64_t tiles = ((p.N + kWBM - 1) / kWBM) * ((p.Fo + kWBN - 1) / kWBN);
    static const int min_tiles = hw_env_int("DC_H2_WIDE_MIN_TILES", 128);
    if ((tiles * ks < min_tiles && p.grp.n < 1 && !p.x2) || tiles * ks >= (int64_t)INT32_MAX) return false;
    if (fwd_h2d_launch(p, hs)) return true;
    const dim3 gd((unsigned)(tiles * ks)), bd(512);
    if (p.x2) {
        if (!p.x2_coef || ks > 1 || !hw_al16(p.x2)) return false;
        if (p.N % kWBM == 0 && p.Fo % kWBN == 0)
            DC_LAUNCH((k_fwd_h2w<true, true>), gd, bd, 0, hs, p);
        else
            DC_LAUNCH((k_fwd_h2w<false, true>), gd, bd, 0, hs, p);
        return true;
    }
    if (p.N % kWBM == 0 && p.Fo % kWBN == 0)
        DC_LAUNCH((k_fwd_h2w<true>), gd, bd, 0, hs, p);
    else
        DC_LAUNCH((k_fwd_h2w<false>), gd, bd, 0, hs, p);
    return true;
}

}
```

deformcontact_amd/csrc/dc_dense_narrow.hip:

```cpp
#include "dc_dense.h"

#ifndef DC_NARROW_ABL
#define DC_NARROW_ABL 0
#endif

namespace dc {

using nb_bf16x4 = __attribute__((ext_vector_type(4))) __bf16;
using nb_bf16x8 = __attribute__((ext_vector_type(8))) __bf16;
using nb_f32x4 = __attribute__((ext_vector_type(4))) float;

struct NarrowParams {
    const float *x;
    int64_t ld;
    const float *w[kMaxSeg];
    int nseg, fi;
    const float *bias;
    float *out;
    int64_t ldo, N;
    int relu, ntiles;
};

constexpr int kNarrowFo = 256;

__device__ __forceinline__ void nb_lds_barrier() {
    asm volatile("s_waitcnt lgkmcnt(0)\n\ts_barrier" ::: "memory");
}

__device__ __forceinline__ void nb_split1(float x, __bf16 &hi, __bf16 &mid, __bf16 &lo) {
    hi = (__bf16)x;
    const float r = x - (float)hi;
    mid = (__bf16)r;
    const float r2 = r - (float)mid;
    lo = (__bf16)r2;
}

template <int KS, int MB>
__global__ void __launch_bounds__(256)
k_fwd_narrow(NarrowParams p) {
    constexpr int TR = 32 * MB;
    constexpr int SROWA = KS * 96 + 16;
    constexpr int PPR = 4 * KS;
    constexpr int TP = TR * PPR, NV = (TP + 255) / 256;
    constexpr int KP = 16 * KS;
    constexpr int kOffStage = ((TR * SROWA + 1023) / 1024) * 1024;
    constexpr int kLdsTiles = kOffStage + TR * 1024, kLdsW = kNarrowFo * (KP + 4) * 4;
    __shared__ __attribute__((aligned(1024))) char lds[kLdsTiles > kLdsW ? kLdsTiles : kLdsW];
    char *const sA = lds;
    float *const so = reinterpret_cast<float *>(lds + kOffStage);
    const int wid = __builtin_amdgcn_readfirstlane((int)(threadIdx.x >> 6)), lane = threadIdx.x & 63;
    const int c = lane & 31, h = lane >> 5;

    nb_f32x4 xv[NV];
    auto load_tile = [&](int t) {
        const int64_t row0 = (int64_t)t * TR;
#pragma unroll
        for (int j = 0; j < NV; ++j) {
            const int q = (int)threadIdx.x + 256 * j;
            if (TP % 256 != 0 && q >= TP) continue;
            const int r = q / PPR, c4 = q - r * PPR;
            int64_t row = row0 + r;
            row = row < p.N ? row : p.N - 1;
            if (DC_NARROW_ABL & 8) xv[j] = nb_f32x4{(float)row, 1.f, 2.f, 3.f};
            else xv[j] = *reinterpret_cast<const nb_f32x4 *>(p.x + row * p.ld + 4 * c4);
        }
    };
    int t = blockIdx.x;
    if (t < p.ntiles) load_tile(t);

    constexpr int WROW = KP + 4;
    {
        float *wi = reinterpret_cast<float *>(lds);
        const int width = p.nseg * p.fi, per4 = kNarrowFo * p.fi / 4;
// ... 21 lines not shown
                }
            }
        const int padw = KP - width;
        for (int e = threadIdx.x; e < kNarrowFo * padw; e += 256) {
            const int o = e / padw, f = e - o * padw;
            wi[o * WROW + width + f] = 0.f;
        }
    }
    __syncthreads();
    nb_bf16x8 fb[2][KS][3];
#pragma unroll
    for (int nb = 0; nb < 2; ++nb) {
        const float *wr = reinterpret_cast<const float *>(lds) + (64 * wid + 32 * nb + c) * WROW + 8 * h;
#pragma unroll
        for (int ks = 0; ks < KS; ++ks) {
            const nb_f32x4 v0 = *reinterpret_cast<const nb_f32x4 *>(wr + 16 * ks);
            const nb_f32x4 v1 = *reinterpret_cast<const nb_f32x4 *>(wr + 16 * ks + 4);
#pragma unroll
            for (int j = 0; j < 8; ++j) {
                __bf16 hi, mid, lo;
                nb_split1(j < 4 ? v0[j] : v1[j - 4], hi, mid, lo);
                fb[nb][ks][0][j] = hi, fb[nb][ks][1][j] = mid, fb[nb][ks][2][j] = lo;
            }
        }
    }
    __syncthreads();
    float bcol[2];
#pragma unroll
    for (int nb = 0; nb < 2; ++nb) bcol[nb] = p.bias ? p.bias[64 * wid + 32 * nb + c] : 0.f;
    const bool relu = p.relu != 0;

    auto store_tile = [&]() {
#pragma unroll
        for (int j = 0; j < NV; ++j) {
            const int q = (int)threadIdx.x + 256 * j;
            if (TP % 256 != 0 && q >= TP) continue;
            const int r = q / PPR, c4 = q - r * PPR;
            nb_bf16x4 hi, mid, lo;
#pragma unroll
            for (int i = 0; i < 4; ++i) {
                __bf16 a, b, d;
                nb_split1(xv[j][i], a, b, d);
                hi[i] = a, mid[i] = b, lo[i] = d;
            }
            char *dst = sA + r * SROWA + (c4 >> 2) * 96 + ((c4 >> 1) & 1) * 16 + (c4 & 1) * 8;
            *reinterpret_cast<nb_bf16x4 *>(dst) = hi;
            *reinterpret_cast<nb_bf16x4 *>(dst + 32) = mid;
            *reinterpret_cast<nb_bf16x4 *>(dst + 64) = lo;
        }
    };

    auto store_rows = [&](int64_t row0) {
#pragma unroll 4
        for (int r = wid; r < TR; r += 4) {
            const int64_t row = row0 + r;
            const nb_f32x4 v = *reinterpret_cast<const nb_f32x4 *>(so + r * 256 + 4 * lane);
            if (row < p.N && (!(DC_NARROW_ABL & 4) || v[0] == 12345.678f)) *reinterpret_cast<nb_f32x4 *>(p.out + row * p.ldo + 4 * lane) = v;
        }
    };
    int64_t prev_row0 = -1;
    for (; t < p.ntiles; t += gridDim.x) {
        const int64_t row0 = (int64_t)t * TR;
        if (!(DC_NARROW_ABL & 8)) store_tile();
        if (prev_row0 >= 0) store_rows(prev_row0);
        if (t + (int)gridDim.x < p.ntiles) load_tile(t + gridDim.x);
        nb_lds_barrier();
        f32x16 acc[MB][2];
#pragma unroll
        for (int mb = 0; mb < MB; ++mb)
#pragma unroll
            for (int nb = 0; nb < 2; ++nb)
#pragma unroll
                for (int i = 0; i < 16; ++i) acc[mb][nb][i] = 0.f;
        constexpr int HI = 0, MID = 1, LO = 2;
        constexpr int pa6[6] = {LO, HI, MID, MID, HI, HI}, pb6[6] = {HI, LO, MID, HI, MID, HI};
#pragma unroll
        for (int ks = 0; ks < KS; ++ks) {
            nb_bf16x8 fa[MB][3];
#pragma unroll
            for (int mb = 0; mb < MB; ++mb)
#pragma unroll
                for (int pl = 0; pl < 3; ++pl)
                    fa[mb][pl] = *reinterpret_cast<const nb_bf16x8 *>(sA + (mb * 32 + c) * SROWA + ks * 96 + pl * 32 + h * 16);
#pragma unroll
            for (int tt = 0; tt < 6; ++tt)
#pragma unroll
                for (int mb = 0; mb < MB; ++mb)
#pragma unroll
                    for (int nb = 0; nb < 2; ++nb)
                        if (!(DC_NARROW_ABL & 1))
                            acc[mb][nb] = __builtin_amdgcn_mfma_f32_32x32x16_bf16(fa[mb][pa6[tt]], fb[nb][ks][pb6[tt]], acc[mb][nb], 0, 0, 0);
                        else
                            acc[mb][nb][tt] += (float)fa[mb][pa6[tt]][0] * (float)fb[nb][ks][pb6[tt]][0];
        }
#pragma unroll
        for (int mb = 0; mb < MB; ++mb)
#pragma unroll
            for (int nb = 0; nb < 2; ++nb)
#pragma unroll
                for (int r = 0; r < 16; ++r) {
                    float v = acc[mb][nb][r] + bcol[nb];
                    if (relu) v = fmaxf(v, 0.f);
                    if (!(DC_NARROW_ABL & 16) || r == 0)
                        so[(mb * 32 + (r & 3) + 8 * (r >> 2) + 4 * h) * 256 + 64 * wid + 32 * nb + c] = v;
                }
        nb_lds_barrier();
        prev_row0 = row0;
    }
    if (prev_row0 >= 0) store_rows(prev_row0);
}

template <int KS>
static void narrow_launch(const NarrowParams &p0, hipStream_t hs) {
    NarrowParams p = p0;
    p.ntiles = (int)((p.N + 31) / 32);
    const unsigned grid = (unsigned)(p.ntiles < 256 ? p.ntiles : 256);
    DC_LAUNCH((k_fwd_narrow<KS, 1>), dim3(grid), dim3(256), 0, hs, p);
}

}

using namespace dc;

extern "C" int dc_tag_linear_fwd_narrow_ok(int64_t fi, int nseg, int64_t wpad, int64_t Fo) {
    return (Fo == kNarrowFo && nseg >= 1 && nseg <= kMaxSeg && fi >= 1 && fi <= 32 && nseg * fi <= wpad &&
            (wpad == 96 || wpad == 112 || wpad == 128)) ? 1 : 0;
}

extern "C" int dc_tag_linear_fwd_narrow(const float *slab, int64_t ld, const float *const *ws, int nseg, int64_t fi,
                                        const float *bias, int relu, float *out, int64_t ldo, int64_t N, int64_t wpad,
                                        int64_t Fo, dc_stream_t stream) {
    DC_REQUIRE(dc_tag_linear_fwd_narrow_ok(fi, nseg, wpad, Fo),
               "dc_tag_linear_fwd_narrow: needs Fo = 256, a padded reduction of 96 / 112 / 128 >= nseg * fi (got Fo=%lld wpad=%lld "
               "nseg=%d fi=%lld)", (long long)Fo, (long long)wpad, nseg, (long long)fi);
    DC_REQUIRE(N >= 0, "dc_tag_linear_fwd_narrow: negative N");
    if (N == 0) return DC_OK;
    DC_REQUIRE(slab && ws && out && ld >= wpad && ldo >= Fo, "dc_tag_linear_fwd_narrow: null pointer / short leading dimension");
    DC_REQUIRE(ld % 4 == 0 && ldo % 4 == 0 && ((uintptr_t)slab & 15) == 0 && ((uintptr_t)out & 15) == 0,
               "dc_tag_linear_fwd_narrow: rows of the slab and of the output must be 16-byte aligned");
    DC_REQUIRE(N < ((int64_t)1 << 31) - 64, "dc_tag_linear_fwd_narrow: too many rows");
    NarrowParams p{};
    p.x = slab, p.ld = ld, p.nseg = nseg, p.fi = (int)fi, p.bias = bias, p.out = out, p.ldo = ldo, p.N = N, p.relu = relu;
    for (int s = 0; s < nseg; ++s) {
        DC_REQUIRE(ws[s], "dc_tag_linear_fwd_narrow: null weight segment %d", s);
        p.w[s] = ws[s];
    }
    hipStream_t hs = (hipStream_t)stream;
    switch (wpad) {
    case 96: narrow_launch<6>(p, hs); break;
    case 112: narrow_launch<7>(p, hs); break;
    default: narrow_launch<8>(p, hs); break;
    }
    return check_launch("dc_tag_linear_fwd_narrow");
}
```

deformcontact_amd/csrc/dc_dense_split.hip:

```cpp
#include "dc_dense.h"

#ifndef DC_DWS_ABL
#define DC_DWS_ABL 0
#endif

namespace dc {

using bf16x4 = __attribute__((ext_vector_type(4))) __bf16;
using bf16x8 = __attribute__((ext_vector_type(8))) __bf16;

constexpr int kPlane = 32;

template <int NP> struct Planes {
    static_assert(NP == 6 || NP == 3 || NP == 1 || NP == 2, "products per tile: 6, 3, 1 or 2 (= fp16x2)");
    static constexpr bool F16 = NP == 2;
    static constexpr int P = NP == 6 ? 3 : ((NP == 3 || NP == 2) ? 2 : 1);
    static constexpr int NPROD = NP == 2 ? 3 : NP;
    static constexpr int SROW = P * kPlane + 16;
};

using f16x4 = __attribute__((ext_vector_type(4))) _Float16;
using f16x8 = __attribute__((ext_vector_type(8))) _Float16;

__device__ __forceinline__ void split4_h2(const float4 &v, f16x4 &h, f16x4 &l) {
// ... 240 lines not shown
}

template <int MB, bool MASK, int NP>
__global__ void __launch_bounds__(256)
k_dx_split(DxParams p) {
    constexpr int BM = 64 * MB, SROW = Planes<NP>::SROW;
    __shared__ __attribute__((aligned(16))) char lds[2 * (BM + BN) * SROW];
    const unsigned ntn = (unsigned)((p.Fi + BN - 1) / BN), per_row = ntn * p.nseg;
    const unsigned lb = xcd_remap(blockIdx.x, gridDim.x);
    const int64_t row0 = (int64_t)(lb / per_row) * BM;
    const int s = (int)((lb % per_row) / ntn);
    const int64_t col0 = (int64_t)(lb % ntn) * BN;
    const int wid = threadIdx.x >> 6, wm = wid >> 1, wn = wid & 1;

    f32x16 acc[MB][2];
    zero_acc<MB>(acc);
    SplitOp<BM, MASK, NP> A;
    SplitOp<BN, false, NP> B;
    A.init(p.g.p, p.mask.p, p.g.ld, row0, p.N, p.mask.ld);
    B.init(p.w[s].p, nullptr, p.Fo, col0, p.Fi);
    constexpr bool F16 = Planes<NP>::F16;
    __shared__ float s_inv[F16 ? BM : 1];
    float invb = 1.f;
    if (F16) {
        const int r = threadIdx.x >> 2;
#pragma unroll
        for (int j = 0; j < BM / 64; ++j) {
            int64_t row = row0 + r + 64 * j;
            row = row < p.N ? row : p.N - 1;
            const float m = p.h2.a_rowmax[row];
            A.sc[j] = h2_scale(m);
            if ((threadIdx.x & 3) == 0) s_inv[r + 64 * j] = h2_unscale(m);
        }
        const float bm = h2_block_max(p.h2.b_rowmax, 0, p.Fo, reinterpret_cast<float *>(lds));
        B.set_scale(h2_scale(bm));
        invb = h2_unscale(bm);
    }
    split_loop<MB, NP>(lds, (int)(p.Fo / BK), A, B, []() {}, acc, wm, wn);
    float *out = p.gx[s];
    const int64_t ldo = p.ldgx[s];
    for_each_acc<MB>(acc, wm, wn, [&](int r, int c, float v) {
        const int64_t row = row0 + r, col = col0 + c;
        if (F16) v = (v * s_inv[r]) * invb;
        if (row < p.N && col < p.Fi) out[row * ldo + col] = v;
    });
}

template <int COLS, int NP> struct TrImage {
    static constexpr int ROWB = COLS * 2 + 64;
    static constexpr int PLANE = BK * ROWB;
    static constexpr int BYTES = Planes<NP>::P * PLANE;
};

template <int COLS, bool MASK, int NP>
struct SplitOpRC {
    static constexpr int P = Planes<NP>::P;
    static constexpr int NV = COLS / 64;
    static constexpr int PER = COLS / 4, KPER = 256 / PER;
    using Img = TrImage<COLS, NP>;
    const float *p[NV];
    const float *pm[MASK ? NV : 1];
    float4 v[NV];
    float4 m[MASK ? NV : 1];
    int off[NV];
    int64_t step, mstep;
    float sc;

    __device__ __forceinline__ void init(const float *base, const float *mbase, int64_t ld,
                                         int64_t k0, int64_t col0, int64_t ncols, int64_t mld = 0) {
        const int c4 = threadIdx.x % PER, kr = threadIdx.x / PER;
        int64_t col = col0 + 4 * c4;
        col = col + 4 <= ncols ? col : ncols - 4;
        mld = mld ? mld : ld;
#pragma unroll
        for (int j = 0; j < NV; ++j) {
            const int64_t k = k0 + kr + KPER * j;
            p[j] = base + k * ld + col;
            if (MASK) pm[j] = mbase + k * mld + col;
            off[j] = (kr + KPER * j) * Img::ROWB + 8 * c4;
        }
        step = BK * ld;
        mstep = BK * mld;
    }
    __device__ __forceinline__ void load() {
#pragma unroll
        for (int j = 0; j < NV; ++j) {
            if ((DC_DWS_ABL & 8) && MASK) v[j] = make_float4(1.f, 2.f, 3.f, (float)j);
            else if ((DC_DWS_ABL & 16) && !MASK) v[j] = make_float4(1.f, 2.f, 3.f, (float)j);
            else v[j] = *reinterpret_cast<const float4 *>(p[j]);
            p[j] += step;
            if (MASK) {
                if (DC_DWS_ABL & 2) m[j] = make_float4(1.f, -1.f, 1.f, 1.f);
                else m[j] = *reinterpret_cast<const float4 *>(pm[j]);
                pm[j] += mstep;
            }
        }
    }
    __device__ __forceinline__ float4 value(int j) const {
        if (!MASK) return v[j];
        return make_float4(m[j].x > 0.f ? v[j].x : 0.f, m[j].y > 0.f ? v[j].y : 0.f,
                           m[j].z > 0.f ? v[j].z : 0.f, m[j].w > 0.f ? v[j].w : 0.f);
    }
    __device__ __forceinline__ void store(char *lds) const {
#pragma unroll
        for (int j = 0; j < NV; ++j) {
            if (Planes<NP>::F16) {
                float4 x = value(j);
                x = make_float4(x.x * sc, x.y * sc, x.z * sc, x.w * sc);
                f16x4 h, l;
                split4_h2(x, h, l);
                *reinterpret_cast<f16x4 *>(lds + off[j]) = h;
                *reinterpret_cast<f16x4 *>(lds + off[j] + Img::PLANE) = l;
                continue;
            }
            bf16x4 hi, mid, lo;
            split4(value(j), hi, mid, lo);
            *reinterpret_cast<bf16x4 *>(lds + off[j]) = hi;
            if (P > 1) *reinterpret_cast<bf16x4 *>(lds + off[j] + Img::PLANE) = mid;
            if (P > 2) *reinterpret_cast<bf16x4 *>(lds + off[j] + 2 * Img::PLANE) = lo;
        }
    }
};

using s16x4 = __attribute__((ext_vector_type(4))) short;
typedef __attribute__((address_space(3))) s16x4 lds_s16x4;

template <int ROWB>
__device__ __forceinline__ bf16x8 tr_operand(const char *plane, int m0) {
    const int lane = threadIdx.x & 63, g = lane >> 4, q = (lane >> 2) & 3, pp = lane & 3;
    const int h = g >> 1;
    const char *a = plane + (8 * h + q) * ROWB + (m0 + 16 * (g & 1) + 4 * pp) * 2;
    const s16x4 lo4 = __builtin_amdgcn_ds_read_tr16_b64_v4i16((lds_s16x4 *)(uintptr_t)(a));
    const s16x4 hi4 = __builtin_amdgcn_ds_read_tr16_b64_v4i16(
        (lds_s16x4 *)(uintptr_t)(a + 4 * ROWB));
    union { s16x4 s[2]; bf16x8 b; } u;
    u.s[0] = lo4, u.s[1] = hi4;
    return u.b;
}

template <int MB, bool MASK, int NP>
__global__ void __launch_bounds__(256)
k_dw_split(DwParams p) {
    constexpr int BM = 64 * MB, P = Planes<NP>::P;
    using IA = TrImage<BM, NP>;
    using IB = TrImage<BN, NP>;
    constexpr int kStage = IA::BYTES + IB::BYTES, kOffB = IA::BYTES;
    __shared__ __attribute__((aligned(16))) char lds[2 * kStage];
    const unsigned ntm = (unsigned)((p.Fo + BM - 1) / BM), ntn = (unsigned)((p.Fi + BN - 1) / BN);
    const unsigned tiles = ntm * ntn, per_chunk = tiles * p.nseg;
    const unsigned lb = xcd_remap(blockIdx.x, gridDim.x);
    const unsigned chunk = lb / per_chunk, rem = lb % per_chunk;
    const int s = (int)(rem / tiles);
    const int64_t o0 = (int64_t)((rem % tiles) / ntn) * BM, f0 = (int64_t)((rem % tiles) % ntn) * BN;
    const int64_t n_beg = (int64_t)chunk * p.chunk_rows;
    const int64_t n_end = (n_beg + p.chunk_rows < p.N) ? n_beg + p.chunk_rows : p.N;
    const int wid = threadIdx.x >> 6, wm = wid >> 1, wn = wid & 1;
    const bool do_bias = p.bias_partial && s == 0 && f0 == 0;

    f32x16 acc[MB][2];
    zero_acc<MB>(acc);
    float4 bsum4 = make_float4(0.f, 0.f, 0.f, 0.f);
    using OA = SplitOpRC<BM, MASK, NP>;
    OA A;
    SplitOpRC<BN, false, NP> B;
    A.init(p.g.p, p.mask.p, p.g.ld, n_beg, o0, p.Fo, p.mask.ld);
    B.init(p.x[s].p, nullptr, p.x[s].ld, n_beg, f0, p.Fi);
    float inva = 1.f, invb = 1.f;
    if (Planes<NP>::F16) {
        const float am = h2_block_max(p.h2.a_rowmax, n_beg, n_end, reinterpret_cast<float *>(lds));
        const float bm = h2_block_max(p.h2.b_rowmax, n_beg, n_end, reinterpret_cast<float *>(lds));
        A.sc = h2_scale(am), B.sc = h2_scale(bm);
        inva = h2_unscale(am), invb = h2_unscale(bm);
    }
    auto bias_acc = [&]() {
        if (do_bias) {
#pragma unroll
            for (int j = 0; j < OA::NV; ++j) {
                const float4 x = A.value(j);
                bsum4.x += x.x, bsum4.y += x.y, bsum4.z += x.z, bsum4.w += x.w;
            }
        }
    };
    const int nst = (int)((n_end - n_beg) / BK);
    if (nst > 0) {
        A.load();
        B.load();
        A.store(lds);
        B.store(lds + kOffB);
        bias_acc();
        if (nst > 1) {
            A.load();
            B.load();
        }
    }
    __syncthreads();
    for (int it = 0; it < nst; ++it) {
        const char *cur = lds + (it & 1) * kStage;
        char *nxt = lds + ((it + 1) & 1) * kStage;
        SplitFrag<MB, NP> f;
#pragma unroll
        for (int pl = 0; pl < P; ++pl) {
#pragma unroll
            for (int mb = 0; mb < MB; ++mb)
                f.a[mb][pl] = tr_operand<IA::ROWB>(cur + pl * IA::PLANE, wm * 32 * MB + mb * 32);
#pragma unroll
            for (int nb = 0; nb < 2; ++nb)
                f.b[nb][pl] = tr_operand<IB::ROWB>(cur + kOffB + pl * IB::PLANE, wn * 64 + nb * 32);
        }
        if (it + 1 < nst) {
            A.store(nxt);
            B.store(nxt + kOffB);
            bias_acc();
        }
        if (it + 2 < nst) {
            A.load();
            B.load();
        }
        if (!(DC_DWS_ABL & 1)) mma_split<MB, NP>(f, acc);
// ... 275 lines not shown

bool fwd_split_launch(const FwdParams &p, int mb, int np, hipStream_t hs) {
    if (np != 6 && np != 3 && np != 1 && np != 2) return false;
    if (np == 2 && (!p.h2.a_rowmax || !p.h2.b_rowmax)) return false;
    if (p.Fi % BK != 0 || p.Fi < BK) return false;
    for (int s = 0; s < p.nseg; ++s)
        if (!al16(p.x[s].p) || !al16(p.w[s].p) || p.x[s].ld % 4 != 0 || p.x[s].ld != p.x[0].ld)
            return false;
    const int64_t grid = ((p.N + 64 * mb - 1) / (64 * mb)) * ((p.Fo + BN - 1) / BN);
    const dim3 gd((unsigned)grid), bd(256);
#define DC_L(MB_, NP_) DC_LAUNCH((k_fwd_split<MB_, NP_>), gd, bd, 0, hs, p)
    if (mb == 2) { if (np == 6) DC_L(2, 6); else if (np == 3) DC_L(2, 3); else if (np == 2) DC_L(2, 2); else DC_L(2, 1); }
    else { if (np == 6) DC_L(1, 6); else if (np == 3) DC_L(1, 3); else if (np == 2) DC_L(1, 2); else DC_L(1, 1); }
#undef DC_L
    return true;
}

bool dx_split_eligible(const DxParams &p) {
    if (p.Fo % BK != 0 || p.Fo < BK || p.Fi % 4 != 0 || !al16(p.g.p) || p.g.ld % 4 != 0) return false;
    if (p.has_mask && (!al16(p.mask.p) || p.mask.ld % 4 != 0)) return false;
    return true;
}

bool dx_split_launch(DxParams p, float *wt, int mb, int np, hipStream_t hs) {
    if (!dx_split_eligible(p) || !al16(wt) || (np != 6 && np != 3 && np != 1 && np != 2)) return false;
    if (np == 2 && (!p.h2.b_rowmax || !p.h2.a_rowmax)) return false;
    TransposeParams t{};
    for (int s = 0; s < p.nseg; ++s) t.w[s] = p.w[s].p;
    t.wt = wt, t.Fi = p.Fi, t.Fo = p.Fo, t.nseg = p.nseg;
    const int64_t tiles = ((p.Fi + 31) / 32) * ((p.Fo + 31) / 32) * p.nseg;
    DC_LAUNCH(k_transpose_w, dim3((unsigned)tiles), dim3(256), 0, hs, t);
    for (int s = 0; s < p.nseg; ++s) p.w[s] = Mat{wt + (int64_t)s * p.Fi * p.Fo, p.Fo};
    const int64_t grid = ((p.N + 64 * mb - 1) / (64 * mb)) * ((p.Fi + BN - 1) / BN) * p.nseg;
    const dim3 gd((unsigned)grid), bd(256);
#define DC_L(MB_, M_)                                                                 \
    do {                                                                              \
        if (np == 6) DC_LAUNCH((k_dx_split<MB_, M_, 6>), gd, bd, 0, hs, p);       \
        else if (np == 3) DC_LAUNCH((k_dx_split<MB_, M_, 3>), gd, bd, 0, hs, p);  \
        else if (np == 2) DC_LAUNCH((k_dx_split<MB_, M_, 2>), gd, bd, 0, hs, p);  \
        else DC_LAUNCH((k_dx_split<MB_, M_, 1>), gd, bd, 0, hs, p);               \
    } while (0)
    if (mb == 2) { if (p.has_mask) DC_L(2, true); else DC_L(2, false); }
    else { if (p.has_mask) DC_L(1, true); else DC_L(1, false); }
#undef DC_L
    return true;
}

bool dw_split_launch(const DwParams &p, int mb, int np, hipStream_t hs) {
    if (np != 6 && np != 3 && np != 1 && np != 2) return false;
    if (np == 2 && (!p.h2.a_rowmax || !p.h2.b_rowmax)) return false;
    if (p.N % BK != 0 || p.chunk_rows % BK != 0 || p.Fi % 4 != 0 || p.Fo % 4 != 0 || p.Fi < 4 ||
        p.Fo < 4 || !al16(p.g.p) || p.g.ld % 4 != 0)
        return false;
    if (p.has_mask && (!al16(p.mask.p) || p.mask.ld % 4 != 0)) return false;
    for (int s = 0; s < p.nseg; ++s)
        if (!al16(p.x[s].p) || p.x[s].ld % 4 != 0) return false;
    if (np == 2 && dw_h2w_launch(p, hs)) return true;
    const int64_t tiles = ((p.Fo + 64 * mb - 1) / (64 * mb)) * ((p.Fi + BN - 1) / BN);
    const dim3 gd((unsigned)(tiles * p.nseg * p.nchunks)), bd(256);
#define DC_L(MB_, M_)                                                                 \
    do {                                                                              \
        if (np == 6) DC_LAUNCH((k_dw_split<MB_, M_, 6>), gd, bd, 0, hs, p);       \
        else if (np == 3) DC_LAUNCH((k_dw_split<MB_, M_, 3>), gd, bd, 0, hs, p);  \
        else if (np == 2) DC_LAUNCH((k_dw_split<MB_, M_, 2>), gd, bd, 0, hs, p);  \
        else DC_LAUNCH((k_dw_split<MB_, M_, 1>), gd, bd, 0, hs, p);               \
    } while (0)
    if (mb == 2) { if (p.has_mask) DC_L(2, true); else DC_L(2, false); }
    else { if (p.has_mask) DC_L(1, true); else DC_L(1, false); }
#undef DC_L
    return true;
}

}
```

deformcontact_amd/ops.py:

```python
from __future__ import annotations

import ctypes
import os
from typing import List, Optional

import torch

from . import _lib
from .deferred import resolve
from .graph import GraphIndex, SortedAdjacency, _require_cuda, capture_id, current_stream_ptr


def _rowmajor(t: torch.Tensor, what: str, dtypes=(torch.float32,)) -> int:
    if t.dim() != 2 or t.dtype not in dtypes:
        raise ValueError(f"{what}: expected a 2-D tensor of {dtypes}, got {tuple(t.shape)} {t.dtype}")
    if t.size(1) > 1 and t.stride(1) != 1:
        raise ValueError(f"{what}: innermost dimension must be contiguous")
    return t.stride(0) if t.size(0) > 1 else max(t.stride(0), t.size(1))


def _vp_array(ptrs):
    return (ctypes.c_void_p * len(ptrs))(*ptrs)


# ... 73 lines not shown
    n, f = x.shape
    if adj.ptr.numel() != n + 1:
        raise ValueError(f"hop_bf16: x has {n} rows but the graph has {adj.ptr.numel() - 1} nodes")
    if out is None:
        out = torch.empty((n, f), dtype=out_dtype, device=x.device)
    if out.shape != x.shape:
        raise ValueError("hop_bf16: out shape mismatch")
    ldy = _rowmajor(out, "out", (out_dtype,))
    lda = 0
    if addend is not None:
        if addend.shape != x.shape:
            raise ValueError("hop_bf16: addend shape mismatch")
        lda = _rowmajor(addend, "addend", (out_dtype,))
    rc = _lib.lib().dc_spmm_bf16(
        adj.ptr.data_ptr(), adj.other.data_ptr(), _ptr(adj.w if weighted else None), x.data_ptr(), ldx,
        _ptr(addend), lda, out.data_ptr(), ldy, n, f, 1 if out_dtype == torch.float32 else 0,
        current_stream_ptr(x.device))
    _lib.check(rc, "dc_spmm_bf16")
    return out


class _HopFn(torch.autograd.Function):

    @staticmethod
    def forward(ctx, g: GraphIndex, x: torch.Tensor, weighted: bool):
        ctx.g, ctx.weighted = g, weighted
        return hop(g.fwd, x.contiguous(), weighted=weighted)

    @staticmethod
    def backward(ctx, gy):
        return None, hop(ctx.g.bwd, _grad_layout(gy, 0), weighted=ctx.weighted), None


def propagate(g: GraphIndex, x: torch.Tensor, weighted: bool = True) -> torch.Tensor:
    return _HopFn.apply(g, resolve(x), weighted)


def _grad_layout(g: torch.Tensor, row_align: int) -> torch.Tensor:
    ok = row_align == 1 or (row_align == 4 and g.stride(0) % 4 == 0 and g.data_ptr() % 16 == 0)
    return g if (ok and g.stride(1) == 1) else g.contiguous()


MAX_SEG = 4

DIRECT_PARAM_GRAD = True


DENSE_SPLIT_BF16 = os.environ.get("DC_DENSE_SPLIT", "1") != "0"

DENSE_PRODUCTS = 6


NARROW_FWD = os.environ.get("DC_NARROW_FWD", "1") != "0"

DENSE_F16X2 = os.environ.get("DC_DENSE_F16X2", "1") != "0"


HOP_CHAIN = os.environ.get("DC_HOP_CHAIN", "1") != "0"
_CHAIN_MAX_NODES = None


def hop_chain_eligible(g, adj: SortedAdjacency, slab: torch.Tensor, f: int, k: int) -> bool:
    global _CHAIN_MAX_NODES
    seg = getattr(g, "_layout", None)
    if not HOP_CHAIN or seg is None or k < 1 or f % 32 != 0 or adj.row_offset:
        return False
    if _CHAIN_MAX_NODES is None:
        _CHAIN_MAX_NODES = int(_lib.lib().dc_hop_chain_max_nodes())
    return (0 < g._seg_max_nodes <= _CHAIN_MAX_NODES and slab.dtype == torch.float32 and slab.dim() == 2
            and slab.stride(1) == 1 and slab.stride(0) % 4 == 0 and slab.data_ptr() % 16 == 0
            and adj.ptr.numel() == slab.size(0) + 1)


HOP_CHAIN_GCN = True


def hop_chain(g, adj: SortedAdjacency, slab: torch.Tensor, f: int, k: int, weighted: bool = True,
              rowmax: Optional[torch.Tensor] = None, rowmax_mode: int = 0, src_block: int = 0, direction: int = 1) -> None:
    nptr, nseg = g._layout
    w = adj.w if weighted else None
    deg = g.fwd.ptr if (HOP_CHAIN_GCN and w is not None and g.normalize and not g.self_loops) else None
    rc = _lib.lib().dc_hop_chain_f32(
        adj.ptr.data_ptr(), adj.other.data_ptr(), _ptr(w), _ptr(deg), adj.other.numel(),
        nptr, nseg, slab.data_ptr(), slab.stride(0), slab.size(0), f, k, int(src_block), int(direction),
        _ptr(rowmax), int(rowmax_mode), current_stream_ptr(slab.device))
    _lib.check(rc, "dc_hop_chain_f32")


DEBUG_TAP = None
DEBUG_CHAIN = None
DEBUG_CHAIN_PRE = None


def chained_hops(g: GraphIndex, slab: torch.Tensor, f: int, k: int, backward: bool,
                 rowmax: Optional[torch.Tensor] = None, transposed: bool = False,
                 rowmax_has_block0: bool = False, rowmax_zeroed: bool = False) -> None:
    if k == 0:
        return
    adj = g.bwd if (backward or transposed) else g.fwd
    blocks = [slab[:, j * f:(j + 1) * f] for j in range(k + 1)]
    if backward:
        for j in range(k, 0, -1):
            hop(adj, blocks[j], out=blocks[j - 1], addend=blocks[j - 1], weighted=g.normalize)
    elif hop_chain_eligible(g, adj, slab, f, k):
        if DEBUG_CHAIN_PRE is not None:
            DEBUG_CHAIN_PRE(g, adj, slab, f, k, transposed)
# ... 181 lines not shown
        return [slab], [ld], slab.size(1), 1
    return [slab[:, j * fi:(j + 1) * fi] for j in range(k + 1)], [ld] * (k + 1), fi, k + 1


def _tag_slab(g, x: torch.Tensor, weights, h2: bool, need_x: bool):
    n, fi = x.shape
    k = len(weights) - 1
    dev = x.device
    wpad = tag_slab_geometry(fi, k)[2]
    slab = _as_slab_block0(x, n, fi, wpad)
    if slab is None and k == 0 and wpad == fi and x.is_contiguous() and x.data_ptr() % 16 == 0:
        slab = x
    rowmax = prepped = None
    if slab is None:
        key = None
        if HOP_CACHE and g is not None and k >= 1 and not need_x:
            key = _hop_cache_key(x, k, wpad, h2)
            hit = _hop_cache_get(g, key, x, dev)
            if hit is not None:
                slab, rowmax = hit
        if slab is None:
            slab, rowmax = _build_input_slab(g, x, k, h2)
            if key is not None:
                _hop_cache_put(g, key, x, slab, rowmax, dev)
    else:
        rowmax = torch.empty(n, dtype=torch.float32, device=dev) if h2 else None
        zeroed = False
        if h2 and g is not None and hop_chain_eligible(g, g.fwd, slab, fi, k):
            fo = weights[0].size(0)
            prepped = _h2_weight_prep(_lib.lib(), [w.contiguous() for w in weights], k, fo, fi,
                                      need_x and fo % 16 == 0, dev, current_stream_ptr(dev), zero=rowmax)
            zeroed = True
        chained_hops(g, slab, fi, k, backward=False, rowmax=rowmax, rowmax_zeroed=zeroed)
    if h2 and k == 0:
        rowmax = rowabsmax(slab)
    return slab, rowmax, prepped


def _tag_out_buffer(next_geom, n: int, fo: int, dev) -> torch.Tensor:
    if isinstance(next_geom, OutInto):
        out = next_geom.view
        if out.shape != (n, fo) or out.stride(1) != 1 or out.dtype != torch.float32 or out.device != dev:
            raise ValueError("tag_conv: out_into view has the wrong shape / layout")
        return out
    if next_geom is None:
        return torch.empty((n, fo), dtype=torch.float32, device=dev)
    next_width, next_wpad = next_geom
    nxt = _alloc_slab(n, next_wpad, dev, tag=(n, fo, next_wpad))
    if next_wpad > next_width:
        nxt[:, next_width:].zero_()
    return nxt[:, :fo]


def _tag_weight_gradients(ctx, slab, g: torch.Tensor, mask_ptr, ldm: int, g_rowmax=None, xrowmax=None):
    k, fi, fo = ctx.k, ctx.fi, ctx.fo
    need_ws, need_b = ctx.needs_input_grad[5:], ctx.has_bias and ctx.needs_input_grad[2]
    gws: List[Optional[torch.Tensor]] = [None] * (k + 1)
    if not (any(need_ws) or need_b):
        return gws, None
    L = _lib.lib()
    n, dev = slab.size(0), slab.device
    st = current_stream_ptr(dev)
    bucket = _direct_sink(list(ctx.params) + ([ctx.bias_param] if ctx.has_bias else []),
                          list(need_ws) + [need_b or not ctx.has_bias])
    if bucket is not None:
        outs = [p.grad for p in ctx.params]
        gb_out = ctx.bias_param.grad if ctx.has_bias else None
    else:
        outs = [torch.empty((fo, fi), dtype=torch.float32, device=dev) for _ in range(k + 1)]
        gb_out = torch.empty(fo, dtype=torch.float32, device=dev) if need_b else None
    xs, ldxs, fi_eff, nseg = _dense_operands(slab, fi, k, ctx.concat)
    nbytes = L.dc_tag_linear_bwd_dw_workspace_bytes(n, fi_eff, fo, nseg)
    scratch = torch.empty(nbytes, dtype=torch.uint8, device=dev)
    args = (g.data_ptr(), g.stride(0), mask_ptr, ldm, _ptr_array(xs), _i64_array(ldxs), nseg,
            _ptr_array(outs), k + 1, fi, _ptr(gb_out), int(bucket is not None), scratch.data_ptr(), nbytes,
            n, fi_eff, fo)
    if g_rowmax is not None and n % 16 == 0:
        rc = L.dc_tag_linear_bwd_dw_h2(*args, g_rowmax.data_ptr(), xrowmax.data_ptr(), st)
    elif ctx.path != "fp32":
        rc = L.dc_tag_linear_bwd_dw_split(*args, DENSE_PRODUCTS, st)
    else:
        rc = L.dc_tag_linear_bwd_dw(*args, st)
    _lib.check(rc, "dc_tag_linear_bwd_dw")
    if bucket is not None:
        bucket.note_direct_write(torch.cuda.current_stream(dev))
        return gws, None
    return [outs[j] if need_ws[j] else None for j in range(k + 1)], gb_out


def _tap_h2_backward(g, fi: int, fo: int, hop_rowmax, g_rowmax, gx, gslab) -> None:
    DEBUG_TAP(f"bwd{fi}x{fo}.hop_rowmax", hop_rowmax)
    DEBUG_TAP(f"bwd{fi}x{fo}.g_rowmax", g_rowmax)
    if os.environ.get("HUNT_TAP_ADJ") == "1":
        for nm, t in (("bwd.ptr", g.bwd.ptr), ("bwd.other", g.bwd.other), ("bwd.w", g.bwd.w), ("fwd.ptr", g.fwd.ptr)):
            DEBUG_TAP(f"bwd{fi}x{fo}.adj.{nm}", t)
    if os.environ.get("HUNT_TAP_BIG") == "1":
        DEBUG_TAP(f"bwd{fi}x{fo}.gx", gx)
        DEBUG_TAP(f"bwd{fi}x{fo}.gslab", gslab)


def _tag_backward_h2(ctx, gout: torch.Tensor):
    slab, out, xrowmax, wt, wt_rowmax, *ws = ctx.saved_tensors
    g, k, fi, fo = ctx.g, ctx.k, ctx.fi, ctx.fo
    L = _lib.lib()
    n, dev = slab.size(0), slab.device
    st = current_stream_ptr(dev)
    need_x = ctx.needs_input_grad[1]
    ldm = out.stride(0) if out is not None else fo
    gwid = (k + 1) * fo
    gslab = _alloc_slab(n, gwid, dev)
    gld = gslab.stride(0)
    g_rowmax = torch.empty(n, dtype=torch.float32, device=dev)
    hop_rowmax = torch.empty(n, dtype=torch.float32, device=dev) if need_x else None
    _lib.check(L.dc_tag_mask_grad(gout.data_ptr(), gout.stride(0), _ptr(out), ldm, gslab.data_ptr(), gld, n, fo,
                                  g_rowmax.data_ptr(), _ptr(hop_rowmax), st), "dc_tag_mask_grad")

    def weight_gradients():
        return _tag_weight_gradients(ctx, slab, gslab, None, ldm, g_rowmax, xrowmax)

    dw_pos = _dw_position(dev)
    if not need_x:
        return (None, *weight_gradients())
    grads = weight_gradients() if dw_pos == "first" else None
    chained_hops(g, gslab, fo, k, backward=False, rowmax=hop_rowmax, transposed=True, rowmax_has_block0=True)
    if dw_pos == "mid":
        grads = weight_gradients()
    if wt is None:
        wt = torch.empty((fi, gwid), dtype=torch.float32, device=dev)
        wt_rowmax = torch.empty(fi, dtype=torch.float32, device=dev)
        _lib.check(L.dc_tag_weight_prep(_ptr_array(ws), k + 1, fo, fi, torch.empty(fo, device=dev).data_ptr(), None,
                                        wt.data_ptr(), wt_rowmax.data_ptr(), st), "dc_tag_weight_prep")
    gx = torch.empty((n, fi), dtype=torch.float32, device=dev)
    rc = L.dc_tag_linear_fwd_h2p(gslab.data_ptr(), gld, wt.data_ptr(), None, 0, gx.data_ptr(), fi, n, gwid, fi,
                                 hop_rowmax.data_ptr(), wt_rowmax.data_ptr(), None, 0, st)
    _lib.check(rc, "dc_tag_linear_fwd_h2 (dX)")
    if DEBUG_TAP is not None:
        _tap_h2_backward(g, fi, fo, hop_rowmax, g_rowmax, gx, gslab)
    if grads is None:
        grads = weight_gradients()
    return (gx, *grads)


def _tag_backward_generic(ctx, gout: torch.Tensor):
    slab, out, _, _, _, *ws = ctx.saved_tensors
    k, fi, fo = ctx.k, ctx.fi, ctx.fo
    L = _lib.lib()
    n, dev = slab.size(0), slab.device
    st = current_stream_ptr(dev)
    mask_ptr, ldm = _ptr(out), (out.stride(0) if out is not None else fo)
    gws, gb = _tag_weight_gradients(ctx, slab, gout, mask_ptr, ldm)
    if not ctx.needs_input_grad[1]:
        return None, gws, gb
    wpad = slab.size(1)
    if ctx.path == "narrow":
        ws = [_pack_weights(ws, fo, fi, wpad, st)]
    gslab = _alloc_slab(n, wpad, dev)
    gxs, ldgs, fi_eff, nseg = _dense_operands(gslab, fi, k, ctx.concat)
    if ctx.path != "fp32":
        wsb = L.dc_tag_linear_bwd_dx_split_workspace_bytes(fi_eff, fo, nseg)
        wsx = torch.empty(wsb, dtype=torch.uint8, device=dev)
        rc = L.dc_tag_linear_bwd_dx_split(gout.data_ptr(), gout.stride(0), mask_ptr, ldm, _ptr_array(ws), nseg,
                                          _ptr_array(gxs), _i64_array(ldgs), wsx.data_ptr(), wsb, n, fi_eff, fo,
                                          DENSE_PRODUCTS, st)
    else:
        rc = L.dc_tag_linear_bwd_dx(gout.data_ptr(), gout.stride(0), mask_ptr, ldm, _ptr_array(ws), nseg,
                                    _ptr_array(gxs), _i64_array(ldgs), n, fi_eff, fo, st)
    _lib.check(rc, "dc_tag_linear_bwd_dx")
    chained_hops(ctx.g, gslab, fi, k, backward=True)
    return gslab[:, :fi], gws, gb


class _TagConvFn(torch.autograd.Function):

    @staticmethod
    def forward(ctx, g: GraphIndex, x: torch.Tensor, bias: Optional[torch.Tensor], relu: bool,
                next_geom, *weights):
        n, fi = x.shape
        k = len(weights) - 1
        fo = weights[0].size(0)
        if k + 1 > MAX_SEG:
            raise NotImplementedError(f"TAGConv K={k} > {MAX_SEG - 1} is not supported by the fused dense block")
        dev = x.device
        L = _lib.lib()
        st = current_stream_ptr(dev)
        six = next_geom is SIX_PRODUCTS
        if six:
            next_geom = None
        ctx.empty = n == 0
        if ctx.empty:
            ctx.fi, ctx.has_bias = fi, bias is not None
            ctx.save_for_backward(*weights)
            return _tag_out_buffer(next_geom, n, fo, dev)
        concat, width, wpad = tag_slab_geometry(fi, k)
        path = _dense_path(fi, k, fo, six, concat and bool(L.dc_tag_linear_fwd_narrow_ok(fi, k + 1, wpad, fo)))
        need_x = ctx.needs_input_grad[1]
        slab, rowmax, prepped = _tag_slab(g, x, weights, path == "h2", need_x)
        ws = [w.contiguous() for w in weights]
        if concat and path != "narrow":
            ws = [_pack_weights(ws, fo, fi, wpad, st)]
        out = _tag_out_buffer(next_geom, n, fo, dev)
        ldo = out.stride(0)
        b = bias.contiguous() if bias is not None else None
        wt = wt_rowmax = None
        if path == "h2":
            if prepped is None:
                prepped = _h2_weight_prep(L, ws, k, fo, fi, need_x and fo % 16 == 0, dev, st)
            wmax, wimg, wt, wt_rowmax = prepped
            rc = L.dc_tag_linear_fwd_h2p(slab.data_ptr(), slab.stride(0), wimg.data_ptr(), _ptr(b), int(relu),
                                         out.data_ptr(), ldo, n, width, fo, rowmax.data_ptr(), wmax.data_ptr(),
                                         None, 0, st)
        elif path == "narrow":
            rc = L.dc_tag_linear_fwd_narrow(slab.data_ptr(), slab.stride(0), _ptr_array(ws), k + 1, fi, _ptr(b),
                                            int(relu), out.data_ptr(), ldo, n, wpad, fo, st)
        else:
            xs, ldxs, fi_eff, nseg = _dense_operands(slab, fi, k, concat)
            args = (_ptr_array(xs), _i64_array(ldxs), _ptr_array(ws), nseg, _ptr(b), int(relu), out.data_ptr(), ldo,
                    n, fi_eff, fo)
            rc = L.dc_tag_linear_fwd(*args, st) if path == "fp32" else L.dc_tag_linear_fwd_split(*args, DENSE_PRODUCTS, st)
        _lib.check(rc, "dc_tag_linear_fwd")
        ctx.g, ctx.k, ctx.fi, ctx.fo, ctx.has_bias, ctx.relu, ctx.concat, ctx.path = \
            g, k, fi, fo, bias is not None, relu, concat, path
        ctx.params, ctx.bias_param = weights, bias
        ctx.save_for_backward(slab, out if relu else None, rowmax, wt, wt_rowmax, *ws)
        return out

    @staticmethod
    def backward(ctx, gout):
        if ctx.empty:
            need = ctx.needs_input_grad
            ws = ctx.saved_tensors
            gx = gout.new_zeros((0, ctx.fi)) if need[1] else None
            gb = gout.new_zeros(gout.size(1)) if (ctx.has_bias and need[2]) else None
            return (None, gx, gb, None, None, *[torch.zeros_like(w) if need[5 + j] else None for j, w in enumerate(ws)])
        gout = _grad_layout(gout, 4)
        if ctx.path == "h2" and ctx.fo % 16 == 0:
            gx, gws, gb = _tag_backward_h2(ctx, gout)
        else:
            gx, gws, gb = _tag_backward_generic(ctx, gout)
        return (None, gx, gb, None, None, *gws)


class OutInto:

    def __init__(self, view: torch.Tensor):
        self.view = view


_MERGED_TAG = "_dc_merged_slab"


def alloc_merged_slab(mg: GraphIndex, fi: int, k: int, dev) -> torch.Tensor:
    concat, width, wpad = tag_slab_geometry(fi, k)
    if concat:
        raise ValueError("alloc_merged_slab: wide layers only (Fi a multiple of 16, (K+1)*Fi > 128)")
    n = mg.num_nodes
    slab = _alloc_slab(n, wpad, dev, tag=("merged", n, fi, wpad, tuple(mg.row_beg), tuple(mg.rows)))
    ends = list(mg.row_beg[1:]) + [n]
    for r0, rows, r1 in zip(mg.row_beg, mg.rows, ends):
        if r0 + rows < r1:
            slab[r0 + rows:r1, :fi].zero_()
    return slab


def merged_slab_part(slab: torch.Tensor, mg: GraphIndex, g: int, fi: int) -> torch.Tensor:
    r0 = mg.row_beg[g]
    return slab[r0:r0 + mg.rows[g], :fi]


def _as_merged_slab(xs, mg: GraphIndex, fi: int, wpad: int):
    base = xs[0]._base
    tag = ("merged", mg.num_nodes, fi, wpad, tuple(mg.row_beg), tuple(mg.rows))
    if base is None or getattr(base, _SLAB_TAG, None) != tag or base.dim() != 2 or not base.is_contiguous():
        return None
    ld = base.size(1)
    for g, x in enumerate(xs):
        if (x._base is not base or x.shape != (mg.rows[g], fi) or x.stride() != (ld, 1)
# ... 870 lines not shown
```

include/deformcontact.h:

```cpp
#ifndef DEFORMCONTACT_H
#define DEFORMCONTACT_H

#include <stdint.h>

#ifdef __cplusplus
extern "C" {
#endif

#define DC_OK 0
#define DC_EINVAL (-1)
#define DC_ELAUNCH (-2)
#define DC_EWORKSPACE (-3)

typedef void *dc_stream_t;

#define DC_MAX_PARTS 4
#define DC_MAX_GROUPS 4
#define DC_GROUP_ALIGN 256

int dc_version(void);
const char *dc_last_error(void);
int64_t dc_stream_capture_id(dc_stream_t stream);

int64_t dc_csr_workspace_bytes(int64_t E, int64_t N);
// ... 73 lines not shown

int dc_spmm_bf16(const int32_t *ptr, const int32_t *other, const float *w, const uint16_t *x,
                 int64_t ldx, const void *addend, int64_t ldadd, void *y, int64_t ldy, int64_t N,
                 int64_t F, int y_is_f32, dc_stream_t stream);

int dc_spmm_f32_rowmax(const int32_t *ptr, const int32_t *other, const float *w, const float *x,
                       int64_t ldx, const float *addend, int64_t ldadd, float *y, int64_t ldy,
                       int64_t N, int64_t F, float *rowmax, int mode, dc_stream_t stream);

int64_t dc_hop_chain_max_nodes(void);
int64_t dc_hop_chain_lds_request(void);
int dc_hop_chain_f32(const int32_t *ptr, const int32_t *other, const float *w, const int32_t *deg_ptr,
                     int64_t cap, const int64_t *node_ptr_host, int nseg, float *slab, int64_t ld, int64_t N,
                     int64_t F, int K, int src_block, int dir, float *rowmax, int mode,
                     dc_stream_t stream);

int dc_tag_linear_fwd_bf16(const uint16_t *a, int64_t lda, const uint16_t *w, const float *bias,
                           int relu, void *out, int64_t ldo, int out_is_bf16, int64_t N, int64_t K,
                           int64_t Fo, dc_stream_t stream);
int dc_tag_mask_grad_bf16(const void *g, int64_t ldg, int g_is_bf16, const void *out_for_mask, int64_t ldo,
                          int mask_is_bf16, uint16_t *gm, int64_t ldgm, int64_t N, int64_t F,
                          dc_stream_t stream);
int64_t dc_tag_linear_bwd_dw_bf16_workspace_bytes(int64_t N, int64_t Fi, int64_t Fo, int nseg);
int dc_tag_linear_bwd_dw_bf16(const uint16_t *g, int64_t ldg, const uint16_t *x, int64_t ldx, int nseg,
                              float *const *gws, float *gbias, int accumulate, void *partials,
                              int64_t partials_bytes, int64_t N, int64_t Fi, int64_t Fo, dc_stream_t stream);
int dc_to_bf16(const float *const *srcs, int nseg, int64_t rows, int64_t cols, int64_t ld_src,
               uint16_t *dst, int64_t ld_dst, dc_stream_t stream);

int64_t dc_contact_loss_workspace_bytes(int64_t N);
int dc_contact_loss(const int32_t *ptr_f, const int32_t *other_f, const int32_t *ptr_b,
                    const int32_t *other_b, const float *pred, int64_t ld_pred, const float *target,
                    int64_t ld_target, int64_t N, int64_t E, float *grad_l1, float *grad_gcl,
                    float *losses , void *workspace, int64_t workspace_bytes,
                    dc_stream_t stream);

#define DC_MAX_SEG 4
int dc_tag_linear_fwd(const float *const *xs, const int64_t *ldxs, const float *const *ws,
                      int nseg, const float *bias, int relu, float *out, int64_t ldo,
                      int64_t N, int64_t Fi, int64_t Fo, dc_stream_t stream);

int dc_tag_linear_bwd_dx(const float *g, int64_t ldg, const float *out_for_mask, int64_t ldo,
                         const float *const *ws, int nseg, float *const *gxs,
                         const int64_t *ldgxs, int64_t N, int64_t Fi, int64_t Fo,
                         dc_stream_t stream);

int dc_tag_linear_fwd_split(const float *const *xs, const int64_t *ldxs, const float *const *ws,
                            int nseg, const float *bias, int relu, float *out, int64_t ldo,
                            int64_t N, int64_t Fi, int64_t Fo, int products, dc_stream_t stream);
int dc_tag_linear_fwd_narrow_ok(int64_t fi, int nseg, int64_t wpad, int64_t Fo);
int dc_tag_linear_fwd_narrow(const float *slab, int64_t ld, const float *const *ws, int nseg, int64_t fi,
                             const float *bias, int relu, float *out, int64_t ldo, int64_t N, int64_t wpad,
                             int64_t Fo, dc_stream_t stream);
int64_t dc_tag_linear_bwd_dx_split_workspace_bytes(int64_t Fi, int64_t Fo, int nseg);
int dc_tag_linear_bwd_dx_split(const float *g, int64_t ldg, const float *out_for_mask,
                               int64_t ldo, const float *const *ws, int nseg, float *const *gxs,
                               const int64_t *ldgxs, void *workspace, int64_t workspace_bytes,
                               int64_t N, int64_t Fi, int64_t Fo, int products, dc_stream_t stream);

int64_t dc_tag_linear_bwd_dw_workspace_bytes(int64_t N, int64_t Fi, int64_t Fo, int nseg);
int dc_tag_linear_bwd_dw(const float *g, int64_t ldg, const float *out_for_mask, int64_t ldo,
                         const float *const *xs, const int64_t *ldxs, int nseg,
                         float *const *gws, int ngw, int64_t gw_cols, float *gbias,
                         int accumulate, void *partials, int64_t partials_bytes, int64_t N,
                         int64_t Fi, int64_t Fo, dc_stream_t stream);
int dc_tag_linear_bwd_dw_split(const float *g, int64_t ldg, const float *out_for_mask,
                               int64_t ldo, const float *const *xs, const int64_t *ldxs, int nseg,
                               float *const *gws, int ngw, int64_t gw_cols, float *gbias,
                               int accumulate, void *partials, int64_t partials_bytes, int64_t N,
                               int64_t Fi, int64_t Fo, int products, dc_stream_t stream);

int dc_tag_linear_fwd_h2(const float *const *xs, const int64_t *ldxs, const float *const *ws,
                         int nseg, const float *bias, int relu, float *out, int64_t ldo, int64_t N,
                         int64_t Fi, int64_t Fo, const float *x_rowmax, const float *w_rowmax,
                         dc_stream_t stream);
int dc_tag_linear_bwd_dx_h2(const float *g, int64_t ldg, const float *out_for_mask, int64_t ldo,
                            const float *const *ws, int nseg, float *const *gxs,
                            const int64_t *ldgxs, void *workspace, int64_t workspace_bytes,
                            int64_t N, int64_t Fi, int64_t Fo, const float *g_rowmax,
                            const float *w_rowmax, dc_stream_t stream);
int dc_tag_linear_bwd_dw_h2(const float *g, int64_t ldg, const float *out_for_mask, int64_t ldo,
                            const float *const *xs, const int64_t *ldxs, int nseg,
                            float *const *gws, int ngw, int64_t gw_cols, float *gbias,
                            int accumulate, void *partials, int64_t partials_bytes, int64_t N,
                            int64_t Fi, int64_t Fo, const float *g_rowmax, const float *x_rowmax,
                            dc_stream_t stream);
int dc_tag_linear_bwd_dw_h2_corr(const float *g, int64_t ldg, const float *g2, const float *g2_coef,
                                 const float *const *xs, const int64_t *ldxs, int nseg, float *const *gws, int ngw,
                                 int64_t gw_cols, int accumulate, void *partials, int64_t partials_bytes, int64_t N,
                                 int64_t Fi, int64_t Fo, const float *g_rowmax, const float *x_rowmax,
                                 dc_stream_t stream);
int dc_tag_mask_grad(const float *g, int64_t ldg, const float *out_for_mask, int64_t ldo, float *gm,
                     int64_t ldgm, int64_t N, int64_t F, float *rowmax_a, float *rowmax_b,
                     dc_stream_t stream);
int dc_tag_transpose_weights(const float *const *ws, int nseg, int64_t Fo, int64_t Fi, float *wt,
                             dc_stream_t stream);
int dc_tag_weight_prep(const float *const *ws, int nseg, int64_t Fo, int64_t Fi, float *w_rowmax,
                       void *w_image, void *wt_image, float *wt_rowmax, dc_stream_t stream);
int dc_tag_weight_prep_zero(const float *const *ws, int nseg, int64_t Fo, int64_t Fi, float *w_rowmax,
                            void *w_image, void *wt_image, float *wt_rowmax, float *zero, int64_t zero_n,
                            dc_stream_t stream);
int64_t dc_tag_linear_fwd_h2p_workspace_bytes(int64_t N, int64_t K, int64_t Fo);
int dc_tag_linear_fwd_h2p(const float *x, int64_t ldx, const void *w_image, const float *bias, int relu,
                          float *out, int64_t ldo, int64_t N, int64_t K, int64_t Fo,
                          const float *x_rowmax, const float *w_rowmax, void *workspace,
                          int64_t workspace_bytes, dc_stream_t stream);
int dc_tag_linear_fwd_h2p_exp(const float *x, int64_t ldx, const void *w_image, float *out, int64_t ldo,
                              int64_t N, int64_t K, int64_t Fo, const float *x_rowmax, const float *w_rowmax,
                              const float *row_lse, int64_t ncols_valid, dc_stream_t stream);
int dc_tag_linear_fwd_h2p_corr(const float *x, int64_t ldx, const float *x2, const float *x2_coef, const void *w_image,
                               float *out, int64_t ldo, int64_t N, int64_t K, int64_t Fo, const float *x_rowmax,
                               const float *w_rowmax, dc_stream_t stream);
int dc_tag_grouped_weight_prep(const float *const *ws, int ngroups, int nseg, int64_t Fo, int64_t Fi,
                               float *const *w_rowmax, void *const *w_image, void *const *wt_image,
                               float *const *wt_rowmax, dc_stream_t stream);
int dc_tag_grouped_fwd_h2p(const float *x, int64_t ldx, int ngroups, const int64_t *row_beg,
                           const int64_t *rows, int64_t N_total, const void *const *w_images,
                           const float *const *biases, int relu, float *out, int64_t ldo, int64_t K,
                           int64_t Fo, const float *x_rowmax, const float *const *w_rowmaxes,
                           dc_stream_t stream);
int dc_tag_grouped_mask_grad(const float *const *g, const int64_t *ldg, int ngroups, const int64_t *row_beg,
                             const int64_t *rows, int64_t N_total, const float *out_for_mask, int64_t ldo,
                             float *gm, int64_t ldgm, int64_t F, float *rowmax_a, float *rowmax_b,
// ... 126 lines not shown
```

Baseline: 541.6 M edges/s.

## Pack ReLU activation mask into bits in forward and read bits in backward

The forward dense kernels (h2 pre-split and narrow paths) now also write a 1-bit-per-element ReLU mask image, built with wave ballots in the epilogue or by a separate pack kernel. The backward mask-grad and split dW kernels read this bit image instead of re-reading the full fp32 output to decide which gradients to zero. This cuts backward memory traffic for the mask by about 32x. The cost is an extra allocation and write in forward, plus a possible extra pack launch when the fused epilogue does not emit bits.

```diff
diff --git a/deformcontact_amd/_lib.py b/deformcontact_amd/_lib.py
--- a/deformcontact_amd/_lib.py
+++ b/deformcontact_amd/_lib.py
@@ -114,6 +114,15 @@
                                            POINTER(c_int64), c_int, POINTER(_vp), c_int, c_int64,
                                            _vp, c_int, _vp, c_int64, c_int64, c_int64, c_int64,
                                            c_int, _vp]),
+    "dc_tag_linear_bwd_dw_split_bits": (c_int, [_vp, c_int64, _vp, c_int64, POINTER(_vp),
+                                                POINTER(c_int64), c_int, POINTER(_vp), c_int, c_int64,
+                                                _vp, c_int, _vp, c_int64, c_int64, c_int64, c_int64,
+                                                c_int, _vp]),
+    "dc_tag_mask_grad_bits": (c_int, [_vp, c_int64, _vp, c_int64, _vp, c_int64, c_int64, c_int64, _vp, _vp, _vp]),
+    "dc_tag_linear_fwd_h2p_bits": (c_int, [_vp, c_int64, _vp, _vp, c_int, _vp, c_int64, c_int64, c_int64, c_int64,
+                                           _vp, _vp, _vp, c_int64, _vp, c_int64, _vp]),
+    "dc_tag_linear_fwd_narrow_bits": (c_int, [_vp, c_int64, POINTER(_vp), c_int, c_int64, _vp, c_int, _vp, c_int64,
+                                              c_int64, c_int64, c_int64, _vp, c_int64, _vp]),
     "dc_tag_linear_fwd_h2": (c_int, [POINTER(_vp), POINTER(c_int64), POINTER(_vp), c_int, _vp,
                                      c_int, _vp, c_int64, c_int64, c_int64, c_int64, _vp, _vp, _vp]),
     "dc_tag_linear_bwd_dx_h2": (c_int, [_vp, c_int64, _vp, c_int64, POINTER(_vp), c_int,
diff --git a/deformcontact_amd/csrc/dc_dense.h b/deformcontact_amd/csrc/dc_dense.h
--- a/deformcontact_amd/csrc/dc_dense.h
+++ b/deformcontact_amd/csrc/dc_dense.h
@@ -114,6 +114,40 @@
     m = fmaxf(fmaxf(red[0], red[1]), fmaxf(red[2], red[3]));
     __syncthreads();
     return m;
+}
+
+constexpr int kReluBitsGroup = 256;
+
+__host__ __device__ __forceinline__ int64_t relu_bits_word(int64_t col) { return ((col >> 7) << 2) + (col & 3); }
+__host__ __device__ __forceinline__ int relu_bits_shift(int64_t col) { return (int)((col >> 2) & 31); }
+
+__device__ __forceinline__ bool relu_bit(const uint32_t *bits, int64_t ldb, int64_t row, int64_t col) {
+    return (bits[row * ldb + relu_bits_word(col)] >> relu_bits_shift(col)) & 1u;
+}
+__device__ __forceinline__ uint4 relu_bits_load4(const uint32_t *bits, int64_t ldb, int64_t row, int64_t col) {
+    return *reinterpret_cast<const uint4 *>(bits + row * ldb + ((col >> 7) << 2));
+}
+__device__ __forceinline__ unsigned relu_bits_pick4(const uint4 &w, int shift) {
+    return ((w.x >> shift) & 1u) | (((w.y >> shift) & 1u) << 1) | (((w.z >> shift) & 1u) << 2) |
+           (((w.w >> shift) & 1u) << 3);
+}
+__device__ __forceinline__ unsigned relu_bits4(const uint32_t *bits, int64_t ldb, int64_t row, int64_t col) {
+    return relu_bits_pick4(relu_bits_load4(bits, ldb, row, col), relu_bits_shift(col));
+}
+__device__ __forceinline__ float4 relu_bits_apply(const float4 &v, unsigned flags) {
+    return make_float4((flags & 1u) ? v.x : 0.f, (flags & 2u) ? v.y : 0.f, (flags & 4u) ? v.z : 0.f,
+                       (flags & 8u) ? v.w : 0.f);
+}
+template <typename V4>
+__device__ __forceinline__ void relu_bits_store_group(uint32_t *group_words, const V4 &v) {
+    const unsigned long long b0 = __ballot(v[0] > 0.f), b1 = __ballot(v[1] > 0.f), b2 = __ballot(v[2] > 0.f),
+                             b3 = __ballot(v[3] > 0.f);
+    const int lane = threadIdx.x & 63;
+    if ((lane & 31) == 0) {
+        const int sh = lane;
+        *reinterpret_cast<uint4 *>(group_words + (lane >> 3)) =
+            make_uint4((unsigned)(b0 >> sh), (unsigned)(b1 >> sh), (unsigned)(b2 >> sh), (unsigned)(b3 >> sh));
+    }
 }
 
 constexpr int kMaxGroups = DC_MAX_GROUPS;
@@ -148,6 +182,8 @@
     int64_t exp_ncols;
     FwdGroups grp;
     const float *x2, *x2_coef;
+    uint32_t *bits;
+    int64_t ldbits;
 };
 
 struct DxParams {
@@ -178,6 +214,8 @@
     H2Scales h2;
     DwGroups grp;
     const float *g2, *g2_coef;
+    const uint32_t *mbits;
+    int64_t ldmb;
 };
 
 
@@ -198,9 +236,10 @@
 bool dx_split_launch(DxParams p, float *wt, int mb, int products, hipStream_t hs);
 bool dw_split_launch(const DwParams &p, int mb, int products, hipStream_t hs);
 bool dw_h2w_launch(const DwParams &p, hipStream_t hs);
-bool fwd_h2_launch(const FwdParams &p, int mb, hipStream_t hs);
-bool fwd_h2w_launch(const FwdParams &p, hipStream_t hs);
-bool fwd_h2d_launch(const FwdParams &p, hipStream_t hs);
+bool fwd_h2_launch(const FwdParams &p, int mb, hipStream_t hs, bool *wrote_bits = nullptr);
+bool fwd_h2w_launch(const FwdParams &p, hipStream_t hs, bool *wrote_bits = nullptr);
+bool fwd_h2d_launch(const FwdParams &p, hipStream_t hs, bool *wrote_bits = nullptr);
+void relu_bits_pack_launch(const float *out, int64_t ldo, uint32_t *bits, int64_t ldb, int64_t N, int64_t F, hipStream_t hs);
 void transpose_weights_launch(const float *const *ws, int nseg, int64_t Fo, int64_t Fi, float *wt,
                               hipStream_t hs);
 
diff --git a/deformcontact_amd/csrc/dc_dense.hip b/deformcontact_amd/csrc/dc_dense.hip
--- a/deformcontact_amd/csrc/dc_dense.hip
+++ b/deformcontact_amd/csrc/dc_dense.hip
@@ -22,6 +22,20 @@
 __device__ __forceinline__ float4 zero_invalid(float4 v, bool row_ok, int64_t k, int64_t kmax) {
     return make_float4((row_ok && k + 0 < kmax) ? v.x : 0.f, (row_ok && k + 1 < kmax) ? v.y : 0.f,
                        (row_ok && k + 2 < kmax) ? v.z : 0.f, (row_ok && k + 3 < kmax) ? v.w : 0.f);
+}
+
+template <bool VEC>
+__device__ __forceinline__ float4 ld4_bits(const uint32_t *bits, int64_t ldb, int64_t row, int64_t k, int64_t kmax) {
+    if (VEC) {
+        const unsigned f = relu_bits4(bits, ldb, row, (k + 4 <= kmax) ? k : 0);
+        return make_float4((f & 1u) ? 1.f : 0.f, (f & 2u) ? 1.f : 0.f, (f & 4u) ? 1.f : 0.f, (f & 8u) ? 1.f : 0.f);
+    } else {
+        const int64_t last = kmax - 1;
+        return make_float4(relu_bit(bits, ldb, row, k + 0 <= last ? k + 0 : last) ? 1.f : 0.f,
+                           relu_bit(bits, ldb, row, k + 1 <= last ? k + 1 : last) ? 1.f : 0.f,
+                           relu_bit(bits, ldb, row, k + 2 <= last ? k + 2 : last) ? 1.f : 0.f,
+                           relu_bit(bits, ldb, row, k + 3 <= last ? k + 3 : last) ? 1.f : 0.f);
+    }
 }
 
 __device__ __forceinline__ float4 relu_mask(float4 v, float4 m) {
@@ -79,6 +93,17 @@
             const int64_t kc = k < t.rmax ? k : t.rmax - 1;
             v[j] = ld4<VEC>(mat.p + kc * mat.ld, col, t.cmax);
             if (MASK) m[j] = ld4<VEC>(mask.p + kc * mask.ld, col, t.cmax);
+        }
+    }
+    __device__ __forceinline__ void load_bits(const Mat &mat, const uint32_t *bits, int64_t ldb, const TileArgs &t) {
+        const int c4 = threadIdx.x % PER, kr = threadIdx.x / PER;
+        const int64_t col = t.c0 + 4 * c4;
+#pragma unroll
+        for (int j = 0; j < NLD; ++j) {
+            const int64_t k = t.r0 + kr + KPER * j;
+            const int64_t kc = k < t.rmax ? k : t.rmax - 1;
+            v[j] = ld4<VEC>(mat.p + kc * mat.ld, col, t.cmax);
+            if (MASK) m[j] = ld4_bits<VEC>(bits, ldb, kc, col, t.cmax);
         }
     }
     __device__ __forceinline__ float4 value(int j, const TileArgs &t) const {
@@ -261,7 +286,10 @@
         ta = TileArgs{n_beg + (int64_t)st * BK, n_end, o0, p.Fo};
         tb = TileArgs{n_beg + (int64_t)st * BK, n_end, f0, p.Fi};
     };
-    auto ldA = [&](SA &ra, const TileArgs &t) { ra.load(p.g, p.mask, t); };
+    auto ldA = [&](SA &ra, const TileArgs &t) {
+        if (MASK && p.mbits) ra.load_bits(p.g, p.mbits, p.ldmb, t);
+        else ra.load(p.g, p.mask, t);
+    };
     auto ldB = [&](SB &rb, const TileArgs &t) { rb.load(p.x[s], p.x[s], t); };
     auto bias_hook = [&](const SA &ra, const TileArgs &t) {
         if (do_bias) {
@@ -461,7 +489,7 @@
                     const float *bias, int relu, float *out, int64_t ldo, int64_t N, int64_t Fi,
                     int64_t Fo, dc_stream_t stream, int products, H2Scales h2 = H2Scales{},
                     float *ksplit_ws = nullptr, int64_t ksplit_ws_bytes = 0, const float *exp_lse = nullptr,
-                    int64_t exp_ncols = 0) {
+                    int64_t exp_ncols = 0, uint32_t *bits = nullptr, int64_t ldbits = 0, bool *wrote_bits = nullptr) {
     DC_REQUIRE(nseg >= 1 && nseg <= kMaxSeg, "dc_tag_linear_fwd: nseg must be 1..%d", kMaxSeg);
     DC_REQUIRE(N >= 0 && Fi >= 1 && Fo >= 1, "dc_tag_linear_fwd: bad sizes");
     if (N == 0) return DC_OK;
@@ -477,6 +505,7 @@
     p.nseg = nseg, p.relu = relu;
     p.h2 = h2;
     p.exp_lse = exp_lse, p.exp_ncols = exp_ncols;
+    p.bits = bits, p.ldbits = ldbits;
     DC_REQUIRE(!exp_lse || h2.b_presplit, "dc_tag_linear_fwd: the exp epilogue exists on the pre-split h2 kernels only");
     const int64_t ntn = (Fo + BN - 1) / BN;
     const int mb = pick_mb(N, ntn);
@@ -497,7 +526,7 @@
             while (ks > 1 && ks * N * Fo * (int64_t)sizeof(float) > ksplit_ws_bytes) --ks;
             if (ks > 1) p.ksplit = (int)ks, p.kpartial = ksplit_ws;
         }
-        if (fwd_h2_launch(p, smb, hs)) {
+        if (fwd_h2_launch(p, smb, hs, wrote_bits)) {
             if (p.ksplit > 1) {
                 ReduceParams r{};
                 r.partial = p.kpartial, r.gw[0] = out, r.Fi = Fo, r.Fo = N, r.cols = Fo;
@@ -651,8 +680,12 @@
                    int64_t gw_cols, float *gbias, int accumulate, void *partials,
                    int64_t partials_bytes, int64_t N, int64_t Fi, int64_t Fo, dc_stream_t stream,
                    int products, H2Scales h2 = H2Scales{}, const float *g2 = nullptr,
-                   const float *g2_coef = nullptr) {
+                   const float *g2_coef = nullptr, const uint32_t *mbits = nullptr, int64_t ldmb = 0) {
     DC_REQUIRE(nseg >= 1 && nseg <= kMaxSeg, "dc_tag_linear_bwd_dw: nseg must be 1..%d", kMaxSeg);
+    DC_REQUIRE(!mbits || (!out_for_mask && Fo % kReluBitsGroup == 0 && ldmb >= Fo / 32 && ldmb % 4 == 0 &&
+                          ((uintptr_t)mbits & 15) == 0),
+               "dc_tag_linear_bwd_dw_split_bits: the bit image needs Fo %% 256 == 0, ldb >= Fo / 32, ldb %% 4 == 0 and a "
+               "16-byte aligned base (Fo=%lld ldb=%lld)", (long long)Fo, (long long)ldmb);
     DC_REQUIRE(N >= 0 && Fi >= 1 && Fo >= 1, "dc_tag_linear_bwd_dw: bad sizes");
     DC_REQUIRE(g && xs && ldxs && gws && partials && ldg >= Fo,
                "dc_tag_linear_bwd_dw: null pointer / ldg < Fo");
@@ -665,6 +698,7 @@
     p.g = make_mat(g, ldg, &vec);
     p.has_mask = out_for_mask != nullptr;
     if (out_for_mask) p.mask = make_mat(out_for_mask, ldo, &vec);
+    if (mbits) p.has_mask = 1, p.mbits = mbits, p.ldmb = ldmb;
     ReduceParams r{};
     for (int s = 0; s < nseg; ++s) {
         DC_REQUIRE(xs[s] && ldxs[s] >= Fi, "dc_tag_linear_bwd_dw: bad segment %d", s);
@@ -689,7 +723,7 @@
     const int mb = dw_mb(Fo);
     const int64_t tiles = ((Fo + 64 * mb - 1) / (64 * mb)) * ((Fi + BN - 1) / BN);
     const int64_t grid = tiles * nseg * p.nchunks;
-    if (!p.has_mask) p.mask = p.g;
+    if (!p.has_mask || p.mbits) p.mask = p.g;
     const dim3 gd((unsigned)grid), bd(256);
     hipStream_t hs = (hipStream_t)stream;
     if (g2) {
@@ -711,6 +745,7 @@
         const int64_t n0 = N - tail;
         t.g.p += n0 * t.g.ld;
         t.mask.p += n0 * t.mask.ld;
+        if (t.mbits) t.mbits += n0 * t.ldmb;
         for (int s = 0; s < nseg; ++s) t.x[s].p += n0 * t.x[s].ld;
         t.N = tail, t.chunk_rows = BK, t.nchunks = 1;
         t.partial = p.partial + (int64_t)p.nchunks * nseg * Fo * Fi;
@@ -776,6 +811,17 @@
                    partials, partials_bytes, N, Fi, Fo, stream, products);
 }
 
+extern "C" int dc_tag_linear_bwd_dw_split_bits(const float *g, int64_t ldg, const uint32_t *mask_bits, int64_t ldb,
+                                               const float *const *xs, const int64_t *ldxs, int nseg,
+                                               float *const *gws, int ngw, int64_t gw_cols, float *gbias,
+                                               int accumulate, void *partials, int64_t partials_bytes, int64_t N,
+                                               int64_t Fi, int64_t Fo, int products, dc_stream_t stream) {
+    DC_REQUIRE(products == 6, "dc_tag_linear_bwd_dw_split_bits: products must be 6");
+    DC_REQUIRE(mask_bits, "dc_tag_linear_bwd_dw_split_bits: null bit image");
+    return dw_impl(g, ldg, nullptr, 0, xs, ldxs, nseg, gws, ngw, gw_cols, gbias, accumulate, partials,
+                   partials_bytes, N, Fi, Fo, stream, products, H2Scales{}, nullptr, nullptr, mask_bits, ldb);
+}
+
 
 extern "C" int dc_tag_linear_fwd_h2(const float *const *xs, const int64_t *ldxs,
                                     const float *const *ws, int nseg, const float *bias, int relu,
@@ -813,6 +859,34 @@
     DC_REQUIRE(!workspace || (((uintptr_t)workspace) & 15) == 0, "dc_tag_linear_fwd_h2p: workspace misaligned");
     return fwd_impl(xs, ld, ws, 1, bias, relu, out, ldo, N, K, Fo, stream, 2, h, (float *)workspace,
                     workspace ? workspace_bytes : 0);
+}
+
+extern "C" int dc_tag_linear_fwd_h2p_bits(const float *x, int64_t ldx, const void *w_image, const float *bias,
+                                          int relu, float *out, int64_t ldo, int64_t N, int64_t K, int64_t Fo,
+                                          const float *x_rowmax, const float *w_rowmax, void *workspace,
+                                          int64_t workspace_bytes, uint32_t *bits, int64_t ldb,
+                                          dc_stream_t stream) {
+    DC_REQUIRE(x && w_image && x_rowmax && w_rowmax && bits, "dc_tag_linear_fwd_h2p_bits: null pointer");
+    DC_REQUIRE(K >= 16 && K % 16 == 0 && ldx >= K && ldx % 4 == 0 && (((uintptr_t)x) & 15) == 0 &&
+                   (((uintptr_t)w_image) & 15) == 0,
+               "dc_tag_linear_fwd_h2p_bits: K %% 16 == 0 and 16-byte aligned operands required (K=%lld)",
+               (long long)K);
+    DC_REQUIRE(Fo % kReluBitsGroup == 0 && ldb >= Fo / 32 && ldb % 4 == 0 && ((uintptr_t)bits & 15) == 0 && ldo % 4 == 0 &&
+                   (((uintptr_t)out) & 15) == 0,
+               "dc_tag_linear_fwd_h2p_bits: the bit image needs Fo %% 256 == 0, ldb >= Fo / 32, ldb %% 4 == 0 and 16-byte "
+               "aligned rows of the image and of the output (Fo=%lld ldb=%lld)", (long long)Fo, (long long)ldb);
+    H2Scales h{};
+    h.a_rowmax = x_rowmax, h.b_rowmax = w_rowmax, h.b_presplit = 1;
+    const float *xs[1] = {x};
+    const float *ws[1] = {(const float *)w_image};
+    const int64_t ld[1] = {ldx};
+    DC_REQUIRE(!workspace || (((uintptr_t)workspace) & 15) == 0, "dc_tag_linear_fwd_h2p_bits: workspace misaligned");
+    bool wrote = false;
+    const int rc = fwd_impl(xs, ld, ws, 1, bias, relu, out, ldo, N, K, Fo, stream, 2, h, (float *)workspace,
+                            workspace ? workspace_bytes : 0, nullptr, 0, bits, ldb, &wrote);
+    if (rc != DC_OK || wrote || N == 0) return rc;
+    relu_bits_pack_launch(out, ldo, bits, ldb, N, Fo, (hipStream_t)stream);
+    return check_launch("dc_tag_linear_fwd_h2p_bits");
 }
 
 extern "C" int dc_tag_linear_fwd_h2p_corr(const float *x, int64_t ldx, const float *x2, const float *x2_coef,
@@ -942,7 +1016,7 @@
 __global__ void __launch_bounds__(256)
 k_mask_grad(const float *__restrict__ g, int64_t ldg, const float *__restrict__ mask, int64_t ldm,
             float *__restrict__ gm, int64_t ldgm, int64_t N, int F, float *__restrict__ rowmax_a,
-            float *__restrict__ rowmax_b, bool vec4) {
+            float *__restrict__ rowmax_b, bool vec4, const uint32_t *__restrict__ bits, int64_t ldb) {
     const int64_t row = (int64_t)blockIdx.x * 4 + (threadIdx.x >> 6);
     if (row >= N) return;
     const int lane = threadIdx.x & 63;
@@ -952,7 +1026,9 @@
     if (vec4) {
         for (int c = lane * 4; c < F; c += 256) {
             float4 v = *reinterpret_cast<const float4 *>(gr + c);
-            if (mr) {
+            if (bits) {
+                v = relu_bits_apply(v, relu_bits4(bits, ldb, row, c));
+            } else if (mr) {
                 const float4 k = *reinterpret_cast<const float4 *>(mr + c);
                 v = make_float4(k.x > 0.f ? v.x : 0.f, k.y > 0.f ? v.y : 0.f, k.z > 0.f ? v.z : 0.f,
                                 k.w > 0.f ? v.w : 0.f);
@@ -963,7 +1039,7 @@
     } else {
         for (int c = lane; c < F; c += 64) {
             float v = gr[c];
-            if (mr && !(mr[c] > 0.f)) v = 0.f;
+            if (bits ? !relu_bit(bits, ldb, row, c) : (mr && !(mr[c] > 0.f))) v = 0.f;
             o[c] = v;
             m = fmaxf(m, fabsf(v));
         }
@@ -977,19 +1053,52 @@
 }
 }
 
-extern "C" int dc_tag_mask_grad(const float *g, int64_t ldg, const float *out_for_mask, int64_t ldo,
-                                float *gm, int64_t ldgm, int64_t N, int64_t F, float *rowmax_a,
-                                float *rowmax_b, dc_stream_t stream) {
+static int mask_grad_impl(const float *g, int64_t ldg, const float *out_for_mask, int64_t ldo, const uint32_t *bits,
+                          int64_t ldb, float *gm, int64_t ldgm, int64_t N, int64_t F, float *rowmax_a, float *rowmax_b,
+                          dc_stream_t stream) {
     DC_REQUIRE(N >= 0 && F >= 1 && F < (1 << 24) && ldg >= F && ldgm >= F && (!out_for_mask || ldo >= F),
                "dc_tag_mask_grad: bad sizes");
+    DC_REQUIRE(!bits || (F % kReluBitsGroup == 0 && ldb >= F / 32 && ldb % 4 == 0 && ((uintptr_t)bits & 15) == 0),
+               "dc_tag_mask_grad_bits: the bit image needs F %% 256 == 0, ldb >= F / 32, ldb %% 4 == 0 and a 16-byte "
+               "aligned base (F=%lld ldb=%lld)", (long long)F, (long long)ldb);
     if (N == 0) return DC_OK;
     DC_REQUIRE(g && gm && rowmax_a, "dc_tag_mask_grad: null pointer");
     const bool vec4 = (F % 4 == 0) && (ldg % 4 == 0) && (ldgm % 4 == 0) && (((uintptr_t)g) & 15) == 0 &&
                       (((uintptr_t)gm) & 15) == 0 &&
                       (!out_for_mask || ((ldo % 4 == 0) && (((uintptr_t)out_for_mask) & 15) == 0));
     DC_LAUNCH(k_mask_grad, dim3((unsigned)((N + 3) / 4)), dim3(256), 0, (hipStream_t)stream, g,
-                       ldg, out_for_mask, ldo, gm, ldgm, N, (int)F, rowmax_a, rowmax_b, vec4);
+                       ldg, out_for_mask, ldo, gm, ldgm, N, (int)F, rowmax_a, rowmax_b, vec4, bits, ldb);
     return check_launch("dc_tag_mask_grad");
+}
+
+extern "C" int dc_tag_mask_grad(const float *g, int64_t ldg, const float *out_for_mask, int64_t ldo,
+                                float *gm, int64_t ldgm, int64_t N, int64_t F, float *rowmax_a,
+                                float *rowmax_b, dc_stream_t stream) {
+    return mask_grad_impl(g, ldg, out_for_mask, ldo, nullptr, 0, gm, ldgm, N, F, rowmax_a, rowmax_b, stream);
+}
+
+extern "C" int dc_tag_mask_grad_bits(const float *g, int64_t ldg, const uint32_t *mask_bits, int64_t ldb, float *gm,
+                                     int64_t ldgm, int64_t N, int64_t F, float *rowmax_a, float *rowmax_b,
+                                     dc_stream_t stream) {
+    DC_REQUIRE(mask_bits, "dc_tag_mask_grad_bits: null bit image");
+    return mask_grad_impl(g, ldg, nullptr, 0, mask_bits, ldb, gm, ldgm, N, F, rowmax_a, rowmax_b, stream);
+}
+
+namespace dc {
+__global__ void __launch_bounds__(256)
+k_relu_bits_pack(const float *__restrict__ out, int64_t ldo, uint32_t *__restrict__ bits, int64_t ldb, int64_t N, int F) {
+    const int64_t row = (int64_t)blockIdx.x * 4 + (threadIdx.x >> 6);
+    if (row >= N) return;
+    const int lane = threadIdx.x & 63;
+    for (int c0 = 0; c0 < F; c0 += kReluBitsGroup) {
+        const float4 t = *reinterpret_cast<const float4 *>(out + row * ldo + c0 + 4 * lane);
+        const float v[4] = {t.x, t.y, t.z, t.w};
+        relu_bits_store_group(bits + row * ldb + (c0 >> 5), v);
+    }
+}
+void relu_bits_pack_launch(const float *out, int64_t ldo, uint32_t *bits, int64_t ldb, int64_t N, int64_t F, hipStream_t hs) {
+    DC_LAUNCH(k_relu_bits_pack, dim3((unsigned)((N + 3) / 4)), dim3(256), 0, hs, out, ldo, bits, ldb, N, (int)F);
+}
 }
 
 namespace dc {
diff --git a/deformcontact_amd/csrc/dc_dense_fast.hip b/deformcontact_amd/csrc/dc_dense_fast.hip
--- a/deformcontact_amd/csrc/dc_dense_fast.hip
+++ b/deformcontact_amd/csrc/dc_dense_fast.hip
@@ -280,6 +280,7 @@
     if (p.N % BK != 0 || p.chunk_rows % BK != 0 || p.Fi % 4 != 0 || p.Fo % 4 != 0 || p.Fi < 4 ||
         p.Fo < 4 || !al16(p.g.p) || p.g.ld % 4 != 0)
         return false;
+    if (p.mbits) return false;
     if (p.has_mask && (!al16(p.mask.p) || p.mask.ld != p.g.ld)) return false;
     for (int s = 0; s < p.nseg; ++s)
         if (!al16(p.x[s].p) || p.x[s].ld % 4 != 0) return false;
diff --git a/deformcontact_amd/csrc/dc_dense_h2.hip b/deformcontact_amd/csrc/dc_dense_h2.hip
--- a/deformcontact_amd/csrc/dc_dense_h2.hip
+++ b/deformcontact_amd/csrc/dc_dense_h2.hip
@@ -209,9 +209,9 @@
 
 static inline bool h2_al16(const void *q) { return ((uintptr_t)q & 15) == 0; }
 
-bool fwd_h2_launch(const FwdParams &p, int mb, hipStream_t hs) {
+bool fwd_h2_launch(const FwdParams &p, int mb, hipStream_t hs, bool *wrote_bits) {
     if (!p.h2.a_rowmax || !p.h2.b_rowmax || p.nseg != 1) return false;
-    if (fwd_h2w_launch(p, hs)) return true;
+    if (fwd_h2w_launch(p, hs, wrote_bits)) return true;
     if (p.Fi % BK != 0 || p.Fi < BK) return false;
     if (p.x[0].ld * 128 >= ((int64_t)1 << 30) || p.Fi * 128 >= ((int64_t)1 << 30)) return false;
     for (int s = 0; s < p.nseg; ++s)
diff --git a/deformcontact_amd/csrc/dc_dense_h2d.hip b/deformcontact_amd/csrc/dc_dense_h2d.hip
--- a/deformcontact_amd/csrc/dc_dense_h2d.hip
+++ b/deformcontact_amd/csrc/dc_dense_h2d.hip
@@ -55,6 +55,7 @@
                 v[i] = row >= data_end ? 0.f : t;
             }
             if (FULL || (row < p.N && col < p.Fo)) *reinterpret_cast<hd_f32x4 *>(p.out + row * p.ldo + col) = v;
+            if (p.bits && (FULL || row < p.N)) relu_bits_store_group(p.bits + row * p.ldbits + (col0 >> 5), v);
         }
     };
 
@@ -285,7 +286,7 @@
 
 static inline bool hd_al16(const void *q) { return ((uintptr_t)q & 15) == 0; }
 
-bool fwd_h2d_launch(const FwdParams &p, hipStream_t hs) {
+bool fwd_h2d_launch(const FwdParams &p, hipStream_t hs, bool *wrote_bits) {
     static const int on = [] {
         const char *v = getenv("DC_H2_DMA");
         return (v && *v) ? atoi(v) : 1;
@@ -308,6 +309,7 @@
         DC_LAUNCH((k_fwd_h2d<true>), gd, bd, 0, hs, p);
     else
         DC_LAUNCH((k_fwd_h2d<false>), gd, bd, 0, hs, p);
+    if (wrote_bits) *wrote_bits = p.bits != nullptr;
     return true;
 }
 
diff --git a/deformcontact_amd/csrc/dc_dense_h2w.hip b/deformcontact_amd/csrc/dc_dense_h2w.hip
--- a/deformcontact_amd/csrc/dc_dense_h2w.hip
+++ b/deformcontact_amd/csrc/dc_dense_h2w.hip
@@ -255,7 +255,7 @@
     return (v && *v) ? atoi(v) : dflt;
 }
 
-bool fwd_h2w_launch(const FwdParams &p, hipStream_t hs) {
+bool fwd_h2w_launch(const FwdParams &p, hipStream_t hs, bool *wrote_bits) {
     static const int wide = hw_env_int("DC_H2_WIDE", 1);
     if (!p.h2.a_rowmax || !p.h2.b_rowmax || !p.h2.b_presplit || p.nseg != 1) return false;
     if (!wide && p.grp.n < 1 && !p.x2) return false;
@@ -267,7 +267,7 @@
     const int64_t tiles = ((p.N + kWBM - 1) / kWBM) * ((p.Fo + kWBN - 1) / kWBN);
     static const int min_tiles = hw_env_int("DC_H2_WIDE_MIN_TILES", 128);
     if ((tiles * ks < min_tiles && p.grp.n < 1 && !p.x2) || tiles * ks >= (int64_t)INT32_MAX) return false;
-    if (fwd_h2d_launch(p, hs)) return true;
+    if (fwd_h2d_launch(p, hs, wrote_bits)) return true;
     const dim3 gd((unsigned)(tiles * ks)), bd(512);
     if (p.x2) {
         if (!p.x2_coef || ks > 1 || !hw_al16(p.x2)) return false;
diff --git a/deformcontact_amd/csrc/dc_dense_narrow.hip b/deformcontact_amd/csrc/dc_dense_narrow.hip
--- a/deformcontact_amd/csrc/dc_dense_narrow.hip
+++ b/deformcontact_amd/csrc/dc_dense_narrow.hip
@@ -19,6 +19,8 @@
     float *out;
     int64_t ldo, N;
     int relu, ntiles;
+    uint32_t *bits;
+    int64_t ldbits;
 };
 
 constexpr int kNarrowFo = 256;
@@ -146,10 +148,12 @@
 
     auto store_rows = [&](int64_t row0) {
 #pragma unroll 4
-        for (int r = wid; r < TR; r += 4) {
+        for (int j = 0; j < TR / 4; ++j) {
+            const int r = wid + 4 * j;
             const int64_t row = row0 + r;
             const nb_f32x4 v = *reinterpret_cast<const nb_f32x4 *>(so + r * 256 + 4 * lane);
             if (row < p.N && (!(DC_NARROW_ABL & 4) || v[0] == 12345.678f)) *reinterpret_cast<nb_f32x4 *>(p.out + row * p.ldo + 4 * lane) = v;
+            if (p.bits && row < p.N) relu_bits_store_group(p.bits + row * p.ldbits, v);
         }
     };
     int64_t prev_row0 = -1;
@@ -221,9 +225,9 @@
             (wpad == 96 || wpad == 112 || wpad == 128)) ? 1 : 0;
 }
 
-extern "C" int dc_tag_linear_fwd_narrow(const float *slab, int64_t ld, const float *const *ws, int nseg, int64_t fi,
-                                        const float *bias, int relu, float *out, int64_t ldo, int64_t N, int64_t wpad,
-                                        int64_t Fo, dc_stream_t stream) {
+static int narrow_impl(const float *slab, int64_t ld, const float *const *ws, int nseg, int64_t fi, const float *bias,
+                       int relu, float *out, int64_t ldo, int64_t N, int64_t wpad, int64_t Fo, uint32_t *bits, int64_t ldb,
+                       dc_stream_t stream) {
     DC_REQUIRE(dc_tag_linear_fwd_narrow_ok(fi, nseg, wpad, Fo),
                "dc_tag_linear_fwd_narrow: needs Fo = 256, a padded reduction of 96 / 112 / 128 >= nseg * fi (got Fo=%lld wpad=%lld "
                "nseg=%d fi=%lld)", (long long)Fo, (long long)wpad, nseg, (long long)fi);
@@ -235,6 +239,9 @@
     DC_REQUIRE(N < ((int64_t)1 << 31) - 64, "dc_tag_linear_fwd_narrow: too many rows");
     NarrowParams p{};
     p.x = slab, p.ld = ld, p.nseg = nseg, p.fi = (int)fi, p.bias = bias, p.out = out, p.ldo = ldo, p.N = N, p.relu = relu;
+    DC_REQUIRE(!bits || (ldb >= Fo / 32 && ldb % 4 == 0 && ((uintptr_t)bits & 15) == 0),
+               "dc_tag_linear_fwd_narrow_bits: the bit image needs ldb >= Fo / 32, ldb %% 4 == 0 and a 16-byte aligned base");
+    p.bits = bits, p.ldbits = ldb;
     for (int s = 0; s < nseg; ++s) {
         DC_REQUIRE(ws[s], "dc_tag_linear_fwd_narrow: null weight segment %d", s);
         p.w[s] = ws[s];
@@ -247,3 +254,15 @@
     }
     return check_launch("dc_tag_linear_fwd_narrow");
 }
+
+extern "C" int dc_tag_linear_fwd_narrow(const float *slab, int64_t ld, const float *const *ws, int nseg, int64_t fi,
+                                        const float *bias, int relu, float *out, int64_t ldo, int64_t N, int64_t wpad,
+                                        int64_t Fo, dc_stream_t stream) {
+    return narrow_impl(slab, ld, ws, nseg, fi, bias, relu, out, ldo, N, wpad, Fo, nullptr, 0, stream);
+}
+
+extern "C" int dc_tag_linear_fwd_narrow_bits(const float *slab, int64_t ld, const float *const *ws, int nseg, int64_t fi,
+                                             const float *bias, int relu, float *out, int64_t ldo, int64_t N,
+                                             int64_t wpad, int64_t Fo, uint32_t *bits, int64_t ldb, dc_stream_t stream) {
+    return narrow_impl(slab, ld, ws, nseg, fi, bias, relu, out, ldo, N, wpad, Fo, bits, ldb, stream);
+}
diff --git a/deformcontact_amd/csrc/dc_dense_split.hip b/deformcontact_amd/csrc/dc_dense_split.hip
--- a/deformcontact_amd/csrc/dc_dense_split.hip
+++ b/deformcontact_amd/csrc/dc_dense_split.hip
@@ -316,22 +316,27 @@
     static constexpr int BYTES = Planes<NP>::P * PLANE;
 };
 
-template <int COLS, bool MASK, int NP>
+template <int COLS, bool MASK, int NP, bool BITS = false>
 struct SplitOpRC {
+    static_assert(!BITS || MASK, "a bit image is a mask");
     static constexpr int P = Planes<NP>::P;
     static constexpr int NV = COLS / 64;
     static constexpr int PER = COLS / 4, KPER = 256 / PER;
     using Img = TrImage<COLS, NP>;
     const float *p[NV];
-    const float *pm[MASK ? NV : 1];
+    const float *pm[(MASK && !BITS) ? NV : 1];
+    const uint32_t *pb[BITS ? NV : 1];
     float4 v[NV];
-    float4 m[MASK ? NV : 1];
+    float4 m[(MASK && !BITS) ? NV : 1];
+    uint4 mw[BITS ? NV : 1];
     int off[NV];
     int64_t step, mstep;
+    int bshift;
     float sc;
 
     __device__ __forceinline__ void init(const float *base, const float *mbase, int64_t ld,
-                                         int64_t k0, int64_t col0, int64_t ncols, int64_t mld = 0) {
+                                         int64_t k0, int64_t col0, int64_t ncols, int64_t mld = 0,
+                                         const uint32_t *bbase = nullptr, int64_t ldb = 0) {
         const int c4 = threadIdx.x % PER, kr = threadIdx.x / PER;
         int64_t col = col0 + 4 * c4;
         col = col + 4 <= ncols ? col : ncols - 4;
@@ -340,11 +345,13 @@
         for (int j = 0; j < NV; ++j) {
             const int64_t k = k0 + kr + KPER * j;
             p[j] = base + k * ld + col;
-            if (MASK) pm[j] = mbase + k * mld + col;
+            if (MASK && !BITS) pm[j] = mbase + k * mld + col;
+            if (BITS) pb[j] = bbase + k * ldb + ((col >> 7) << 2);
             off[j] = (kr + KPER * j) * Img::ROWB + 8 * c4;
         }
         step = BK * ld;
-        mstep = BK * mld;
+        mstep = BITS ? BK * ldb : BK * mld;
+        bshift = relu_bits_shift(col);
     }
     __device__ __forceinline__ void load() {
 #pragma unroll
@@ -353,7 +360,10 @@
             else if ((DC_DWS_ABL & 16) && !MASK) v[j] = make_float4(1.f, 2.f, 3.f, (float)j);
             else v[j] = *reinterpret_cast<const float4 *>(p[j]);
             p[j] += step;
-            if (MASK) {
+            if (BITS) {
+                mw[j] = *reinterpret_cast<const uint4 *>(pb[j]);
+                pb[j] += mstep;
+            } else if (MASK) {
                 if (DC_DWS_ABL & 2) m[j] = make_float4(1.f, -1.f, 1.f, 1.f);
                 else m[j] = *reinterpret_cast<const float4 *>(pm[j]);
                 pm[j] += mstep;
@@ -362,6 +372,7 @@
     }
     __device__ __forceinline__ float4 value(int j) const {
         if (!MASK) return v[j];
+        if (BITS) return relu_bits_apply(v[j], relu_bits_pick4(mw[j], bshift));
         return make_float4(m[j].x > 0.f ? v[j].x : 0.f, m[j].y > 0.f ? v[j].y : 0.f,
                            m[j].z > 0.f ? v[j].z : 0.f, m[j].w > 0.f ? v[j].w : 0.f);
     }
@@ -402,7 +413,7 @@
     return u.b;
 }
 
-template <int MB, bool MASK, int NP>
+template <int MB, bool MASK, int NP, bool BITS = false>
 __global__ void __launch_bounds__(256)
 k_dw_split(DwParams p) {
     constexpr int BM = 64 * MB, P = Planes<NP>::P;
@@ -424,10 +435,10 @@
     f32x16 acc[MB][2];
     zero_acc<MB>(acc);
     float4 bsum4 = make_float4(0.f, 0.f, 0.f, 0.f);
-    using OA = SplitOpRC<BM, MASK, NP>;
+    using OA = SplitOpRC<BM, MASK, NP, BITS>;
     OA A;
     SplitOpRC<BN, false, NP> B;
-    A.init(p.g.p, p.mask.p, p.g.ld, n_beg, o0, p.Fo, p.mask.ld);
+    A.init(p.g.p, p.mask.p, p.g.ld, n_beg, o0, p.Fo, p.mask.ld, p.mbits, p.ldmb);
     B.init(p.x[s].p, nullptr, p.x[s].ld, n_beg, f0, p.Fi);
     float inva = 1.f, invb = 1.f;
     if (Planes<NP>::F16) {
@@ -809,7 +820,8 @@
     if (p.N % BK != 0 || p.chunk_rows % BK != 0 || p.Fi % 4 != 0 || p.Fo % 4 != 0 || p.Fi < 4 ||
         p.Fo < 4 || !al16(p.g.p) || p.g.ld % 4 != 0)
         return false;
-    if (p.has_mask && (!al16(p.mask.p) || p.mask.ld % 4 != 0)) return false;
+    if (p.has_mask && !p.mbits && (!al16(p.mask.p) || p.mask.ld % 4 != 0)) return false;
+    if (p.mbits && np != 6) return false;
     for (int s = 0; s < p.nseg; ++s)
         if (!al16(p.x[s].p) || p.x[s].ld % 4 != 0) return false;
     if (np == 2 && dw_h2w_launch(p, hs)) return true;
@@ -822,6 +834,10 @@
         else if (np == 2) DC_LAUNCH((k_dw_split<MB_, M_, 2>), gd, bd, 0, hs, p);  \
         else DC_LAUNCH((k_dw_split<MB_, M_, 1>), gd, bd, 0, hs, p);               \
     } while (0)
+    if (p.mbits) {
+        if (mb == 2) DC_LAUNCH((k_dw_split<2, true, 6, true>), gd, bd, 0, hs, p);
+        else DC_LAUNCH((k_dw_split<1, true, 6, true>), gd, bd, 0, hs, p);
+    } else
     if (mb == 2) { if (p.has_mask) DC_L(2, true); else DC_L(2, false); }
     else { if (p.has_mask) DC_L(1, true); else DC_L(1, false); }
 #undef DC_L
diff --git a/deformcontact_amd/ops.py b/deformcontact_amd/ops.py
--- a/deformcontact_amd/ops.py
+++ b/deformcontact_amd/ops.py
@@ -149,6 +149,9 @@
 
 
 NARROW_FWD = os.environ.get("DC_NARROW_FWD", "1") != "0"
+
+RELU_BITS = os.environ.get("DC_RELU_BITS", "1") != "0"
+RELU_BITS_GROUP = 256
 
 DENSE_F16X2 = os.environ.get("DC_DENSE_F16X2", "1") != "0"
 
@@ -436,7 +439,7 @@
     return nxt[:, :fo]
 
 
-def _tag_weight_gradients(ctx, slab, g: torch.Tensor, mask_ptr, ldm: int, g_rowmax=None, xrowmax=None):
+def _tag_weight_gradients(ctx, slab, g: torch.Tensor, mask_ptr, ldm: int, g_rowmax=None, xrowmax=None, bits=None):
     k, fi, fo = ctx.k, ctx.fi, ctx.fo
     need_ws, need_b = ctx.needs_input_grad[5:], ctx.has_bias and ctx.needs_input_grad[2]
     gws: List[Optional[torch.Tensor]] = [None] * (k + 1)
@@ -461,6 +464,8 @@
             n, fi_eff, fo)
     if g_rowmax is not None and n % 16 == 0:
         rc = L.dc_tag_linear_bwd_dw_h2(*args, g_rowmax.data_ptr(), xrowmax.data_ptr(), st)
+    elif ctx.path != "fp32" and bits is not None and mask_ptr is not None and DENSE_PRODUCTS == 6:
+        rc = L.dc_tag_linear_bwd_dw_split_bits(*args[:2], bits.data_ptr(), bits.stride(0), *args[4:], DENSE_PRODUCTS, st)
     elif ctx.path != "fp32":
         rc = L.dc_tag_linear_bwd_dw_split(*args, DENSE_PRODUCTS, st)
     else:
@@ -484,7 +489,7 @@
 
 
 def _tag_backward_h2(ctx, gout: torch.Tensor):
-    slab, out, xrowmax, wt, wt_rowmax, *ws = ctx.saved_tensors
+    slab, out, bits, xrowmax, wt, wt_rowmax, *ws = ctx.saved_tensors
     g, k, fi, fo = ctx.g, ctx.k, ctx.fi, ctx.fo
     L = _lib.lib()
     n, dev = slab.size(0), slab.device
@@ -496,8 +501,13 @@
     gld = gslab.stride(0)
     g_rowmax = torch.empty(n, dtype=torch.float32, device=dev)
     hop_rowmax = torch.empty(n, dtype=torch.float32, device=dev) if need_x else None
-    _lib.check(L.dc_tag_mask_grad(gout.data_ptr(), gout.stride(0), _ptr(out), ldm, gslab.data_ptr(), gld, n, fo,
-                                  g_rowmax.data_ptr(), _ptr(hop_rowmax), st), "dc_tag_mask_grad")
+    if bits is not None and out is not None:
+        _lib.check(L.dc_tag_mask_grad_bits(gout.data_ptr(), gout.stride(0), bits.data_ptr(), bits.stride(0),
+                                           gslab.data_ptr(), gld, n, fo, g_rowmax.data_ptr(), _ptr(hop_rowmax), st),
+                   "dc_tag_mask_grad_bits")
+    else:
+        _lib.check(L.dc_tag_mask_grad(gout.data_ptr(), gout.stride(0), _ptr(out), ldm, gslab.data_ptr(), gld, n, fo,
+                                      g_rowmax.data_ptr(), _ptr(hop_rowmax), st), "dc_tag_mask_grad")
 
     def weight_gradients():
         return _tag_weight_gradients(ctx, slab, gslab, None, ldm, g_rowmax, xrowmax)
@@ -526,13 +536,13 @@
 
 
 def _tag_backward_generic(ctx, gout: torch.Tensor):
-    slab, out, _, _, _, *ws = ctx.saved_tensors
+    slab, out, bits, _, _, _, *ws = ctx.saved_tensors
     k, fi, fo = ctx.k, ctx.fi, ctx.fo
     L = _lib.lib()
     n, dev = slab.size(0), slab.device
     st = current_stream_ptr(dev)
     mask_ptr, ldm = _ptr(out), (out.stride(0) if out is not None else fo)
-    gws, gb = _tag_weight_gradients(ctx, slab, gout, mask_ptr, ldm)
+    gws, gb = _tag_weight_gradients(ctx, slab, gout, mask_ptr, ldm, bits=bits)
     if not ctx.needs_input_grad[1]:
         return None, gws, gb
     wpad = slab.size(1)
@@ -586,16 +596,27 @@
         ldo = out.stride(0)
         b = bias.contiguous() if bias is not None else None
         wt = wt_rowmax = None
+        bits = None
+        if (RELU_BITS and relu and path in ("h2", "narrow") and fo % RELU_BITS_GROUP == 0 and ldo % 4 == 0
+                and out.data_ptr() % 16 == 0):
+            bits = torch.empty((n, fo // 32), dtype=torch.int32, device=dev)
         if path == "h2":
             if prepped is None:
                 prepped = _h2_weight_prep(L, ws, k, fo, fi, need_x and fo % 16 == 0, dev, st)
             wmax, wimg, wt, wt_rowmax = prepped
-            rc = L.dc_tag_linear_fwd_h2p(slab.data_ptr(), slab.stride(0), wimg.data_ptr(), _ptr(b), int(relu),
-                                         out.data_ptr(), ldo, n, width, fo, rowmax.data_ptr(), wmax.data_ptr(),
-                                         None, 0, st)
+            args = (slab.data_ptr(), slab.stride(0), wimg.data_ptr(), _ptr(b), int(relu), out.data_ptr(), ldo, n, width,
+                    fo, rowmax.data_ptr(), wmax.data_ptr(), None, 0)
+            if bits is not None:
+                rc = L.dc_tag_linear_fwd_h2p_bits(*args, bits.data_ptr(), bits.stride(0), st)
+            else:
+                rc = L.dc_tag_linear_fwd_h2p(*args, st)
         elif path == "narrow":
-            rc = L.dc_tag_linear_fwd_narrow(slab.data_ptr(), slab.stride(0), _ptr_array(ws), k + 1, fi, _ptr(b),
-                                            int(relu), out.data_ptr(), ldo, n, wpad, fo, st)
+            args = (slab.data_ptr(), slab.stride(0), _ptr_array(ws), k + 1, fi, _ptr(b), int(relu), out.data_ptr(), ldo,
+                    n, wpad, fo)
+            if bits is not None:
+                rc = L.dc_tag_linear_fwd_narrow_bits(*args, bits.data_ptr(), bits.stride(0), st)
+            else:
+                rc = L.dc_tag_linear_fwd_narrow(*args, st)
         else:
             xs, ldxs, fi_eff, nseg = _dense_operands(slab, fi, k, concat)
             args = (_ptr_array(xs), _i64_array(ldxs), _ptr_array(ws), nseg, _ptr(b), int(relu), out.data_ptr(), ldo,
@@ -605,7 +626,7 @@
         ctx.g, ctx.k, ctx.fi, ctx.fo, ctx.has_bias, ctx.relu, ctx.concat, ctx.path = \
             g, k, fi, fo, bias is not None, relu, concat, path
         ctx.params, ctx.bias_param = weights, bias
-        ctx.save_for_backward(slab, out if relu else None, rowmax, wt, wt_rowmax, *ws)
+        ctx.save_for_backward(slab, out if relu else None, bits, rowmax, wt, wt_rowmax, *ws)
         return out
 
     @staticmethod
diff --git a/include/deformcontact.h b/include/deformcontact.h
--- a/include/deformcontact.h
+++ b/include/deformcontact.h
@@ -149,6 +149,9 @@
 int dc_tag_linear_fwd_narrow(const float *slab, int64_t ld, const float *const *ws, int nseg, int64_t fi,
                              const float *bias, int relu, float *out, int64_t ldo, int64_t N, int64_t wpad,
                              int64_t Fo, dc_stream_t stream);
+int dc_tag_linear_fwd_narrow_bits(const float *slab, int64_t ld, const float *const *ws, int nseg, int64_t fi,
+                                  const float *bias, int relu, float *out, int64_t ldo, int64_t N, int64_t wpad,
+                                  int64_t Fo, uint32_t *bits, int64_t ldb, dc_stream_t stream);
 int64_t dc_tag_linear_bwd_dx_split_workspace_bytes(int64_t Fi, int64_t Fo, int nseg);
 int dc_tag_linear_bwd_dx_split(const float *g, int64_t ldg, const float *out_for_mask,
                                int64_t ldo, const float *const *ws, int nseg, float *const *gxs,
@@ -166,6 +169,18 @@
                                float *const *gws, int ngw, int64_t gw_cols, float *gbias,
                                int accumulate, void *partials, int64_t partials_bytes, int64_t N,
                                int64_t Fi, int64_t Fo, int products, dc_stream_t stream);
+
+int dc_tag_linear_bwd_dw_split_bits(const float *g, int64_t ldg, const uint32_t *mask_bits, int64_t ldb,
+                                    const float *const *xs, const int64_t *ldxs, int nseg, float *const *gws,
+                                    int ngw, int64_t gw_cols, float *gbias, int accumulate, void *partials,
+                                    int64_t partials_bytes, int64_t N, int64_t Fi, int64_t Fo, int products,
+                                    dc_stream_t stream);
+int dc_tag_mask_grad_bits(const float *g, int64_t ldg, const uint32_t *mask_bits, int64_t ldb, float *gm,
+                          int64_t ldgm, int64_t N, int64_t F, float *rowmax_a, float *rowmax_b, dc_stream_t stream);
+int dc_tag_linear_fwd_h2p_bits(const float *x, int64_t ldx, const void *w_image, const float *bias, int relu,
+                               float *out, int64_t ldo, int64_t N, int64_t K, int64_t Fo, const float *x_rowmax,
+                               const float *w_rowmax, void *workspace, int64_t workspace_bytes, uint32_t *bits,
+                               int64_t ldb, dc_stream_t stream);
 
 int dc_tag_linear_fwd_h2(const float *const *xs, const int64_t *ldxs, const float *const *ws,
                          int nseg, const float *bias, int relu, float *out, int64_t ldo, int64_t N,
```

Measured after the change: 530.0 M edges/s. 0.979x the previous value.
